# xds0112/5G_based_System_level_Integrated_Sensing_and_Communication_Simulator

Measured on AMD Instinct MI355X. Metric: sensing slots/sec (CDL echo->2D-FFT->2D-CFAR), higher is better.
Workload: dtype f64

## Files before the change

5g_based_system_level_integrated_sensing_and_communication_simulator_amd/_build.py:

```python
from __future__ import annotations

import os
import subprocess
import sys
from concurrent.futures import ThreadPoolExecutor

HERE = os.path.dirname(os.path.abspath(__file__))
CSRC = os.path.join(HERE, "csrc")
OBJ = os.path.join(CSRC, "build")
LIB = os.path.join(HERE, "libisac_hip.so")
SOURCES = ["capi.hip", "fft2d.hip", "tables.hip", "echo.hip", "rdm.hip", "cov.hip", "eigh.hip", "music.hip", "cdl.hip", "cdl_os.hip", "cqi.hip", "los.hip", "doa2d.hip", "doa.hip", "rxfe.hip", "targets.hip", "cfar.hip"]
HEADERS = ["isac_common.hpp", "isac_internal.hpp", "cut_window.hpp", "ofdm_symbol.hpp", "beam_window.hpp", "fft_lds.hpp", "echo_dev.hpp", "eigh_dev.hpp", "eigh_layout.hpp", os.path.join("..", "..", "include", "isac.h"), os.path.join("..", "..", "include", "isac_targets.h"), os.path.join("..", "..", "include", "isac_cfar.h"), os.path.join("..", "..", "include", "isac_cfar_mc.h")]
HIPCC = os.environ.get("HIPCC", "/opt/rocm/bin/hipcc")
FLAGS = ["--offload-arch=gfx950", "-O3", "-std=c++17", "-fPIC", "-fno-gpu-rdc", "-Wall", "-Wno-unused-function",
         "-Wno-unused-variable", "-Wno-unused-value", "-Wno-unused-result", "-ffp-contract=on"]


def _newer(target: str, deps: list[str]) -> bool:
    if not os.path.exists(target):
        return False
    t = os.path.getmtime(target)
    return all(os.path.getmtime(d) <= t for d in deps if os.path.exists(d))


def _compile(src: str, force: bool) -> str:
    obj = os.path.join(OBJ, os.path.splitext(src)[0] + ".o")
    deps = [os.path.join(CSRC, src)] + [os.path.join(CSRC, h) for h in HEADERS] + [os.path.abspath(__file__)]
    if not force and _newer(obj, deps):
        return obj
    cmd = [HIPCC, *FLAGS, "-c", os.path.join(CSRC, src), "-o", obj]
    r = subprocess.run(cmd, capture_output=True, text=True)
    if r.returncode != 0:
        raise RuntimeError(f"hipcc failed for {src}:\n{r.stdout}\n{r.stderr}")
    if r.stderr.strip():
        sys.stderr.write(r.stderr)
    return obj


def build(force: bool = False, verbose: bool = False) -> str:
    os.makedirs(OBJ, exist_ok=True)
    srcs = [s for s in SOURCES if os.path.exists(os.path.join(CSRC, s))]
    with ThreadPoolExecutor(max_workers=min(len(srcs), os.cpu_count() or 4)) as ex:
        objs = list(ex.map(lambda s: _compile(s, force), srcs))
    if force or not _newer(LIB, objs):
        cmd = [HIPCC, "--offload-arch=gfx950", "-shared", "-fPIC", "-o", LIB, *objs,
               "-Wl,-soname,libisac_hip.so", "-Wl,--no-undefined"]
        r = subprocess.run(cmd, capture_output=True, text=True)
        if r.returncode != 0:
            raise RuntimeError(f"link failed:\n{r.stdout}\n{r.stderr}")
    if verbose:
        print(f"built {LIB}")
    return LIB


if __name__ == "__main__":
    build(force="--force" in sys.argv, verbose=True)
```

5g_based_system_level_integrated_sensing_and_communication_simulator_amd/_lib.py:

```python
from __future__ import annotations

import ctypes as C
import os
import sys
import threading

import numpy as np

_HERE = os.path.dirname(os.path.abspath(__file__))
_LIB_PATH = os.path.join(_HERE, "libisac_hip.so")
_lib = None
_lock = threading.Lock()

ISAC_ABI_VERSION = 8
ISAC_MAX_EST = 4096
ISAC_MAX_TARGETS = 1024
NOISE_NONE, NOISE_INJECTED, NOISE_PHILOX, NOISE_PHILOX_SPECTRAL, NOISE_INJECTED_SPECTRAL = 0, 1, 2, 3, 4
CFAR_CA, CFAR_GOCA, CFAR_SOCA, CFAR_OS = 0, 1, 2, 3
CFAR_METHODS = {"CA": CFAR_CA, "GOCA": CFAR_GOCA, "SOCA": CFAR_SOCA, "OS": CFAR_OS}
ISAC_CFAR_MAX_TRAIN = 1024
TARGET_SW0, TARGET_SW1 = 0, 1
TARGET_MODELS = {"swerling0": TARGET_SW0, "swerling1": TARGET_SW1}
ISAC_CFAR_MC_MAX_TRAIN = 128
OPT_MUSIC_ROUTE, OPT_TAIL_FUSION, OPT_WIDE_ORDER, OPT_CDL_SHARE_SPECTRA, OPT_UPA_DOA = 0, 1, 2, 3, 4

STATUS_NAMES = {0: "OK", 1: "INVALID_ARG", 2: "HIP", 3: "NO_LOS", 4: "NO_DETECTION", 5: "CFAR_WINDOW",
                6: "CAPACITY", 7: "UNSUPPORTED", 8: "SHORT_WAVEFORM"}


class IsacError(RuntimeError):

    def __init__(self, code: int, message: str):
        self.code = int(code)
        self.name = STATUS_NAMES.get(int(code), str(code))
        super().__init__(f"isac[{self.name}]: {message}")


class c64(C.Structure):
    _fields_ = [("re", C.c_double), ("im", C.c_double)]


class Carrier(C.Structure):
    _fields_ = [("n_sc", C.c_int32), ("nfft", C.c_int32), ("scs_khz", C.c_int32), ("reserved", C.c_int32)]


class RadarChannelParams(C.Structure):
    _fields_ = [("fc", C.c_double), ("fs", C.c_double), ("n0", C.c_double), ("n_ants", C.c_int32),
                ("n_targets", C.c_int32), ("range", C.POINTER(C.c_double)), ("velocity", C.POINTER(C.c_double)),
                ("large_scale_fading", C.POINTER(C.c_double)), ("rx_steering", C.c_void_p)]


class CfarConfig(C.Structure):
    _fields_ = [("pfa", C.c_double), ("guard", C.c_int32 * 2), ("train", C.c_int32 * 2),
                ("row0", C.c_int32), ("row1", C.c_int32), ("col0", C.c_int32), ("col1", C.c_int32)]


class EstParams(C.Structure):
    _fields_ = [("n_ifft", C.c_int32), ("n_fft", C.c_int32), ("r_res", C.c_double), ("v_res", C.c_double),
                ("array_is_upa", C.c_int32), ("n_ants_x", C.c_int32), ("n_ants_y", C.c_int32),
                ("azimuth_scan_scale", C.c_double), ("azimuth_scan_granularity", C.c_double),
                ("elevation_scan_scale", C.c_double), ("elevation_scan_granularity", C.c_double)]


class Music2dParams(C.Structure):
    _fields_ = [("fc", C.c_double), ("t_sri", C.c_double), ("scs_hz", C.c_double), ("r_max", C.c_double), ("v_max", C.c_double)]


ISAC_MAX_SUBBANDS = 70


class CsiReport(C.Structure):
    _fields_ = [("n_subbands_pmi", C.c_int32), ("n_subbands_cqi", C.c_int32), ("n_cqi", C.c_int32), ("reserved", C.c_int32),
                ("i1", C.c_double * 3), ("i2", C.c_double * ISAC_MAX_SUBBANDS), ("cqi", C.c_double * (ISAC_MAX_SUBBANDS + 1)),
                ("subband_cqi", C.c_double * (ISAC_MAX_SUBBANDS + 1)), ("sinr_per_subband_cw", C.c_double * (ISAC_MAX_SUBBANDS + 1)), ("ri_total_sinr", C.c_double)]


ISAC_MAX_RBS = 275


class SrsReport(C.Structure):
    _fields_ = [("n_subbands", C.c_int32), ("n_tpmi", C.c_int32), ("n_rb", C.c_int32), ("reserved", C.c_int32),
                ("pmi", C.c_double * (ISAC_MAX_SUBBANDS + 1)), ("sinr_subband_pmi", C.c_double * (ISAC_MAX_SUBBANDS + 1)), ("cqi_rb", C.c_double * ISAC_MAX_RBS)]


class CdlJob(C.Structure):
    _fields_ = [("d_x", C.c_void_p), ("d_y", C.c_void_p), ("d_H", C.c_void_p), ("block_start", C.c_void_p), ("n_blocks", C.c_int32), ("reserved", C.c_int32)]


class SensingJob(C.Structure):
    _fields_ = [("d_tx_wave", C.c_void_p), ("d_tx_grid", C.c_void_p), ("d_echo_grid", C.c_void_p), ("rp", C.c_void_p), ("los", C.c_void_p),
                ("d_noise_unit", C.c_void_p), ("seed", C.c_uint64), ("noise_mode", C.c_int32), ("reserved", C.c_int32)]


class RxFrontendJob(C.Structure):
    _fields_ = [("d_y", C.c_void_p), ("d_noise_unit", C.c_void_p), ("path_scale", C.c_double), ("gain_scale", C.c_double), ("noise_power", C.c_double), ("seed", C.c_uint64)]


class PathLossConfig(C.Structure):
    _fields_ = [("building_height", C.c_double), ("street_width", C.c_double), ("environment_height", C.c_double), ("optional_model", C.c_int32), ("reserved", C.c_int32)]


class EstResult(C.Structure):
    _fields_ = [("n_rng", C.c_int32), ("n_vel", C.c_int32), ("n_azi", C.c_int32), ("num_dets", C.c_int32),
                ("total_detections", C.c_int32), ("reserved", C.c_int32),
                ("rng_est", C.c_double * ISAC_MAX_EST), ("vel_est", C.c_double * ISAC_MAX_EST),
                ("azi_est", C.c_double * ISAC_MAX_EST), ("ele_est", C.c_double * ISAC_MAX_EST)]
# ... 29 lines not shown
    "isac_sync": (_INT, (_P,)),
    "isac_dev_alloc": (_INT, (_P, _SZ, _P)),
    "isac_dev_free": (_INT, (_P, _P)),
    "isac_memcpy_h2d": (_INT, (_P, _P, _P, _SZ)),
    "isac_memcpy_d2h": (_INT, (_P, _P, _P, _SZ)),
    "isac_memcpy_d2d": (_INT, (_P, _P, _P, _SZ)),
    "isac_memset_dev": (_INT, (_P, _P, _I32, _SZ)),
    "isac_timer_start": (_INT, (_P,)),
    "isac_timer_stop_ms": (_INT, (_P, _P)),
    "isac_profile_enable": (_INT, (_P, _I32)),
    "isac_profile_last_kernel_ms": (_INT, (_P, _P)),
    "isac_basic_radar_channel_dev": (_INT, (_P, _P, _I64, _ptr(RadarChannelParams), _P, _I32, _P, _U64, _P)),
    "isac_basic_radar_channel": (_INT, (_P, _P, _I64, _ptr(RadarChannelParams), _P, _I32, _P, _U64, _P)),
    "isac_mono_static_sensing_dev": (_INT, (_P, _P, _I64, _I32, _ptr(Carrier), _ptr(RadarChannelParams), _P, _I32, _P, _U64, _P, _P)),
    "isac_mono_static_sensing": (_INT, (_P, _P, _I64, _I32, _ptr(Carrier), _ptr(RadarChannelParams), _P, _I32, _P, _U64, _P, _P)),
    "isac_mono_static_sensing_fused_dev": (_INT, (_P, _P, _I64, _I32, _ptr(Carrier), _ptr(RadarChannelParams), _P, _I32, _P, _U64, _P, _P, _ptr(EstParams), _ptr(CfarConfig), _P)),
    "isac_echo_grid_materialize_dev": (_INT, (_P, _P, _P)),
    "isac_ofdm_symbol_count": (_INT, (_ptr(Carrier), _I64, _P)),
    "isac_ofdm_demodulate_dev": (_INT, (_P, _P, _I64, _I32, _ptr(Carrier), _P, _I32)),
    "isac_ofdm_modulate_dev": (_INT, (_P, _P, _I32, _I32, _ptr(Carrier), _F64, _P, _I64)),
    "isac_ofdm_waveform_length": (_INT, (_ptr(Carrier), _I32, _P)),
    "isac_ofdm_modulate_windowed_dev": (_INT, (_P, _P, _I32, _I32, _ptr(Carrier), _F64, _I32, _I32, _P, _I64)),
    "isac_sentx_append_dev": (_INT, (_P, _ptr(Carrier), _I32, _I32, _I32, _P, _F64, _I32, _P, _I32, _I32, _P, _I64, _I64, _P)),
    "isac_cfar2d_ca": (_INT, (_P, _P, _I32, _I32, _P, _I32, _P, _P, _F64, _P, _I32, _P)),
    "isac_fft2d_dev": (_INT, (_P, _ptr(EstParams), _ptr(CfarConfig), _P, _P, _I32, _I32, _I32, _ptr(EstResult))),
    "isac_fft2d": (_INT, (_P, _ptr(EstParams), _ptr(CfarConfig), _P, _P, _I32, _I32, _I32, _ptr(EstResult))),
    "isac_fft2d_submit_dev": (_INT, (_P, _ptr(EstParams), _ptr(CfarConfig), _P, _P, _I32, _I32, _I32)),
    "isac_fft2d_collect": (_INT, (_P, _ptr(EstResult))),
    "isac_fft2d_submit_cached_dev": (_INT, (_P, _ptr(EstParams), _ptr(CfarConfig), _P, _P, _I32, _I32, _I32)),
    "isac_sensing_submit_n": (_INT, (_P, _I32, _ptr(SensingJob), _I64, _I32, _ptr(Carrier), _ptr(EstParams), _ptr(CfarConfig), _F64, _P)),
    "isac_sensing_collect_n": (_INT, (_P, _I32, _ptr(EstResult), _P)),
    "isac_fft2d_range_stage_dev": (_INT, (_P, _ptr(EstParams), _ptr(CfarConfig), _P, _P, _I32, _I32, _I32)),
    "isac_fft2d_get_detections": (_INT, (_P, _P, _P, _I32, _P, _P)),
    "isac_fft2d_get_power_window": (_INT, (_P, _P, _I64, _P, _P, _P)),
    "isac_fft2d_get_covariance": (_INT, (_P, _P, _I32)),
    "isac_fft2d_get_music_spectrum": (_INT, (_P, _P, _I32, _P)),
    "isac_rdm_plane_dev": (_INT, (_P, _ptr(EstParams), _P, _P, _I32, _I32, _I32, _I32, _P)),
    "isac_covariance_dev": (_INT, (_P, _P, _I64, _I32, _P)),
    "isac_eigh_top": (_INT, (_P, _P, _I32, _I32, _P, _P)),
    "isac_ctx_set_option": (_INT, (_P, _I32, _I32)),
    "isac_ctx_share_streams": (_INT, (_P, _P)),
    "isac_ctx_reserve": (_INT, (_P, _I64, _I32, _ptr(Carrier), _ptr(RadarChannelParams), _ptr(EstParams), _ptr(CfarConfig), _F64, _P)),
    "isac_music_doa": (_INT, (_P, _I32, _ptr(EstParams), _P, _I32, _P, _P, _P, _I32, _P)),
    "isac_beamscan_doa": (_INT, (_P, _I32, _I32, _ptr(EstParams), _P, _I32, _P, _P, _I32, _P)),
    "isac_get_angular_spectrum2d": (_INT, (_P, _P, _I64, _P)),
    "isac_find2d_peaks": (_INT, (_P, _P, _I32, _I32, _I32, _P, _P, _P)),
    "isac_music2d_dev": (_INT, (_P, _ptr(EstParams), _ptr(Music2dParams), _P, _P, _I32, _I32, _I32, _ptr(EstResult))),
    "isac_music2d_get_spectra": (_INT, (_P, _P, _I32, _P, _I32, _P)),
    "isac_eigh": (_INT, (_P, _P, _I32, _P, _P)),
    "isac_cdl_apply_dev": (_INT, (_P, _P, _I64, _I32, _I32, _I32, _P, _I32, _P, _P, _I32, _P, _F64, _P)),
    "isac_cdl_apply_batch_dev": (_INT, (_P, _ptr(CdlJob), _I32, _I64, _I32, _I32, _I32, _P, _I32, _P, _F64)),
    "isac_cdl_path_gains_dev": (_INT, (_P, _P, _P, _I32, _I32, _I32, _I32, _P, _F64, _P, _I32, _P)),
    "isac_prg_precode_dev": (_INT, (_P, _P, _I32, _I32, _I32, _P, _I32, _I32, _I32, _P)),
    "isac_cdl_freq_response_dev": (_INT, (_P, _P, _I32, _I32, _I32, _I32, _P, _P, _I64, _P)),
    "isac_cdl_csi_estimate_batch_dev": (_INT, (_P, _I32, _P, _P, _P, _P, _P, _I32, _I32, _I32, _I32, _I32, _P, _P, _I64, _P)),
    "isac_path_loss_38901": (_INT, (_I32, _F64, _I32, _P, _P, _ptr(PathLossConfig), _P)),
    "isac_path_loss_fspl": (_INT, (_F64, _P, _P, _P)),
    "isac_thermal_noise_power": (_INT, (_F64, _F64, _F64, _P)),
    "isac_dft_channel_matrix": (_INT, (_I32, _I32, _P)),
    "isac_rx_frontend_batch_dev": (_INT, (_P, _ptr(RxFrontendJob), _I32, _I64, _I32, _I32)),
    "isac_rx_frontend_dev": (_INT, (_P, _P, _I64, _I32, _F64, _F64, _F64, _I32, _P, _U64)),
    "isac_precoded_sinr_cqi_dev": (_INT, (_P, _P, _I64, _I32, _I32, _P, _I32, _F64, _P, _I32, _P, _P, _P)),
    "isac_type1sp_codebook": (_INT, (_I32, _I32, _I32, _I32, _I32, _P, _I64, _P)),
    "isac_csi_report_dev": (_INT, (_P, _P, _I64, _I32, _I32, _P, _P, _I32, _I32, _I32, _I32, _I32, _P, _I32, _P, _F64, _P, _I32, _ptr(CsiReport), _P, _P)),
    "isac_csi_report_batch_dev": (_INT, (_P, _I32, _P, _I64, _I32, _I32, _P, _P, _I32, _I32, _I32, _I32, _I32, _P, _I32, _P, _P, _P, _I32, _ptr(CsiReport), _P)),
    "isac_pusch_codebook": (_INT, (_I32, _I32, _P, _I64, _P)),
    "isac_srs_pmi_select_batch_dev": (_INT, (_P, _I32, _P, _I64, _I32, _I32, _P, _I32, _I32, _I32, _P, _P, _I32, _ptr(SrsReport))),
    "isac_los_check_dev": (_INT, (_P, _P, _P, _I64, _P, _P, _P, _P, _I32, _P, _P)),
    "isac_winding_number_dev": (_INT, (_P, _P, _I64, _P, _P, _P, _I32, _P)),
    "isac_synth_qpsk_grid_dev": (_INT, (_P, _P, _I32, _I32, _I32, _U64, _I32)),
}
EXPORTS = list(PROTOTYPES)
PROTOTYPES_ADDED = {
    "isac_fft2d_get_targets": (_INT, (_P, _P, _P, _I32)),
}
PROTOTYPES_CFAR = {
    "isac_cfar_threshold_factor": (_INT, (_I32, _I32, _I32, _F64, _P)),
    "isac_cfar2d": (_INT, (_P, _P, _I32, _I32, _P, _I32, _P, _P, _F64, _ptr(CfarMethod), _P, _I32, _P)),
    "isac_fft2d_redetect": (_INT, (_P, _ptr(CfarMethod), _ptr(EstResult), _P, _P, _I32, _P, _P)),
}
PROTOTYPES_CFAR_MC = {
    "isac_cfar_monte_carlo": (_INT, (_P, _ptr(CfarMethod), _I32, _F64, _I32, _P, _I32, _U64, _U64, _P, _P)),
}


def library_path() -> str:
    return _LIB_PATH


def load():
    global _lib
    with _lock:
        if _lib is not None:
            return _lib
        if not os.path.exists(_LIB_PATH):
            raise RuntimeError(
                f"{_LIB_PATH} is missing: build it with `python -c 'import __graft_entry__ as g; g.build()'` "
                "(hipcc --offload-arch=gfx950).  There is no CPU fallback for the sensing hot path.")
        if "torch" not in sys.modules and os.environ.get("ISAC_NO_TORCH_PRELOAD") != "1":
            try:
                import torch
            except Exception:
                pass
        lib = C.CDLL(_LIB_PATH, mode=C.RTLD_GLOBAL)
        for name, (restype, argtypes) in {**PROTOTYPES, **PROTOTYPES_ADDED, **PROTOTYPES_CFAR, **PROTOTYPES_CFAR_MC}.items():
            fn = getattr(lib, name)
            fn.restype, fn.argtypes = restype, argtypes
        if lib.isac_abi_version() != ISAC_ABI_VERSION:
            raise RuntimeError(f"{_LIB_PATH}: ABI version {lib.isac_abi_version()} but this binding was written for {ISAC_ABI_VERSION}; rebuild the library")
        for which, name, cls in [(i, n, c) for i, (n, c) in enumerate(ABI_STRUCTS)] + list(ABI_STRUCTS_ADDED) + list(ABI_STRUCTS_CFAR):
            if lib.isac_abi_sizeof(which) != C.sizeof(cls):
                raise RuntimeError(f"{_LIB_PATH}: sizeof({name}) = {lib.isac_abi_sizeof(which)} in the library, {C.sizeof(cls)} in the binding")
        _lib = lib
        return lib


def _np_ptr(a: np.ndarray):
    return a.ctypes.data_as(C.c_void_p)


class DeviceArray:

    def __init__(self, ctx: "Context", ptr: int, shape, dtype, owner: bool = True):
        self.ctx, self.ptr, self.shape, self.dtype, self._owner = ctx, int(ptr), tuple(int(s) for s in shape), np.dtype(dtype), owner

    @property
    def _as_parameter_(self):
        return C.c_void_p(self.ptr)

    @property
    def nbytes(self) -> int:
        return int(np.prod(self.shape, dtype=np.int64)) * self.dtype.itemsize

    def numpy(self) -> np.ndarray:
        out = np.empty(self.shape, dtype=self.dtype, order="F")
        self.ctx.check(self.ctx.lib.isac_memcpy_d2h(self.ctx.handle, _np_ptr(out), self, self.nbytes))
        return out

    def free(self):
        if self._owner and self.ptr:
            self.ctx.lib.isac_dev_free(self.ctx.handle, self)
            self.ptr = 0

    def __del__(self):
        try:
            if self.ctx.handle:
                self.free()
        except Exception:
            pass


class Context:

    def __init__(self, device: int | None = None):
        self.lib = load()
        if device is None:
            device = int(os.environ.get("ISAC_DEVICE", os.environ.get("LOCAL_RANK", "0")))
        n = C.c_int(0)
        st = self.lib.isac_device_count(C.byref(n))
        if st != 0 or n.value <= 0:
            raise IsacError(2, "no HIP device visible: the sensing hot path needs an MI355X (no CPU fallback)")
        h = C.c_void_p()
        st = self.lib.isac_ctx_create(device % n.value, C.byref(h))
        if st != 0:
            raise IsacError(st, f"isac_ctx_create(device={device}) failed")
        self.handle = h
        self.device = device % n.value
        self.device_cache = {}

    def close(self):
        if getattr(self, "handle", None):
            for ent in list(self.device_cache.values()):
                for d in (ent if isinstance(ent, tuple) else (ent,)):
                    for dd in (d if isinstance(d, tuple) else (d,)):
                        if isinstance(dd, DeviceArray):
                            dd.free()
            self.device_cache.clear()
            self.lib.isac_ctx_destroy(self.handle)
            self.handle = None

    def __del__(self):
        try:
            self.close()
        except Exception:
            pass

    def check(self, status: int):
        if status != 0:
            raise IsacError(status, (self.lib.isac_last_error(self.handle) or b"").decode())

    def sync(self):
        self.check(self.lib.isac_sync(self.handle))

    def stream(self) -> int:
        s = C.c_void_p()
        self.check(self.lib.isac_ctx_get_stream(self.handle, C.byref(s)))
        return int(s.value or 0)

    def empty(self, shape, dtype=np.complex128) -> DeviceArray:
        dt = np.dtype(dtype)
        nbytes = int(np.prod(shape, dtype=np.int64)) * dt.itemsize
        p = C.c_void_p()
        self.check(self.lib.isac_dev_alloc(self.handle, nbytes, C.byref(p)))
        return DeviceArray(self, p.value, shape, dt)

    def to_device(self, a: np.ndarray) -> DeviceArray:
        a = np.asfortranarray(a)
        d = self.empty(a.shape, a.dtype)
        self.check(self.lib.isac_memcpy_h2d(self.handle, d, _np_ptr(a), a.nbytes))
        return d

    def set_music_route(self, route: int):
        self.check(self.lib.isac_ctx_set_option(self.handle, OPT_MUSIC_ROUTE, int(route)))

    def set_tail_fusion(self, on: bool):
        self.check(self.lib.isac_ctx_set_option(self.handle, OPT_TAIL_FUSION, 1 if on else 0))

    def set_cdl_share_spectra(self, on: bool):
        self.check(self.lib.isac_ctx_set_option(self.handle, OPT_CDL_SHARE_SPECTRA, 1 if on else 0))

    def set_wide_order(self, on: bool):
        self.check(self.lib.isac_ctx_set_option(self.handle, OPT_WIDE_ORDER, 1 if on else 0))

    def set_upa_doa(self, on: bool):
        self.check(self.lib.isac_ctx_set_option(self.handle, OPT_UPA_DOA, 1 if on else 0))

    def angular_spectrum2d(self) -> np.ndarray:
        dims = (C.c_int32 * 2)()
        self.check(self.lib.isac_get_angular_spectrum2d(self.handle, None, 0, dims))
        out = np.zeros((dims[0], dims[1]), dtype=np.float64, order="F")
        self.check(self.lib.isac_get_angular_spectrum2d(self.handle, _np_ptr(out), out.size, dims))
        return out

    def angular_spectrum(self) -> np.ndarray:
        n = C.c_int32(0)
        self.check(self.lib.isac_fft2d_get_music_spectrum(self.handle, None, 0, C.byref(n)))
        out = np.zeros(n.value, dtype=np.float64)
        self.check(self.lib.isac_fft2d_get_music_spectrum(self.handle, _np_ptr(out), out.size, C.byref(n)))
        return out

    def music2d_spectra(self):
        n = (C.c_int32 * 2)()
        self.check(self.lib.isac_music2d_get_spectra(self.handle, None, 0, None, 0, n))
        pr, pv = np.zeros(n[0], dtype=np.float64), np.zeros(n[1], dtype=np.float64)
        self.check(self.lib.isac_music2d_get_spectra(self.handle, _np_ptr(pr), pr.size, _np_ptr(pv), pv.size, n))
        return pr, pv

    def share_streams(self, owner: "Context | None"):
        self.check(self.lib.isac_ctx_share_streams(self.handle, owner.handle if owner is not None else None))
        self._stream_owner = owner

    def eigh_top(self, h, n_top: int):
        h = as_c128_f(h)
        a = h.shape[0]
        w = np.zeros(a)
        u = np.zeros((a, max(int(n_top), 1)), dtype=np.complex128, order="F")
        self.check(self.lib.isac_eigh_top(self.handle, _np_ptr(h), a, int(n_top), _np_ptr(w), _np_ptr(u)))
        return w, u[:, : int(n_top)]

    def timer_start(self):
        self.check(self.lib.isac_timer_start(self.handle))

    def timer_stop_ms(self) -> float:
        ms = C.c_double(0)
        self.check(self.lib.isac_timer_stop_ms(self.handle, C.byref(ms)))
        return ms.value


_default_ctx = None


def default_context() -> Context:
    global _default_ctx
    if _default_ctx is None:
        _default_ctx = Context()
    return _default_ctx


def as_f64(x) -> np.ndarray:
    return np.ascontiguousarray(np.asarray(x, dtype=np.float64).reshape(-1))


def as_c128_f(x) -> np.ndarray:
    return np.asfortranarray(np.asarray(x, dtype=np.complex128))
```

5g_based_system_level_integrated_sensing_and_communication_simulator_amd/csrc/capi.hip:

```cpp
#include <algorithm>
#include <chrono>
#include <map>
#include <mutex>

#include "isac_internal.hpp"

using namespace isac;

extern "C" int isac_abi_version(void) { return ISAC_ABI_VERSION; }
extern "C" int isac_abi_sizeof(int32_t which) {
  switch (which) {
    case ISAC_SIZEOF_EST_RESULT: return (int)sizeof(isac_est_result);
    case ISAC_SIZEOF_EST_PARAMS: return (int)sizeof(isac_est_params);
    case ISAC_SIZEOF_CFAR_CONFIG: return (int)sizeof(isac_cfar_config);
    case ISAC_SIZEOF_RADAR_CHANNEL_PARAMS: return (int)sizeof(isac_radar_channel_params);
    case ISAC_SIZEOF_CARRIER: return (int)sizeof(isac_carrier);
    case ISAC_SIZEOF_MUSIC2D_PARAMS: return (int)sizeof(isac_music2d_params);
    case ISAC_SIZEOF_CSI_REPORT: return (int)sizeof(isac_csi_report);
    case ISAC_SIZEOF_SENSING_JOB: return (int)sizeof(isac_sensing_job);
    case ISAC_SIZEOF_SRS_REPORT: return (int)sizeof(isac_srs_report);
    case ISAC_SIZEOF_RX_FRONTEND_JOB: return (int)sizeof(isac_rx_frontend_job);
    case ISAC_SIZEOF_PATH_LOSS_CONFIG: return (int)sizeof(isac_path_loss_config);
    case ISAC_SIZEOF_TARGET_LIST: return (int)sizeof(isac_target_list);
    case ISAC_SIZEOF_CFAR_METHOD: return (int)sizeof(isac_cfar_method);
// ... 195 lines not shown
extern "C" int isac_profile_enable(isac_ctx* ctx, int on) {
  ISAC_ENTER(ctx);
  ctx->profile = on != 0;
  ctx->profile_cov = on == 2;
  ctx->profile_recorded = false;
  return ISAC_OK;
}
extern "C" int isac_profile_last_kernel_ms(isac_ctx* ctx, double* ms) {
  ISAC_ENTER(ctx);
  if (!ms) return fail(ctx, ISAC_ERR_INVALID_ARG, "NULL argument");
  if (!ctx->profile || !ctx->profile_recorded) return fail(ctx, ISAC_ERR_INVALID_ARG, "no profiled kernel launch on this context");
  ISAC_HIP(hipEventSynchronize(ctx->ev_k1));
  float f = 0.f;
  ISAC_HIP(hipEventElapsedTime(&f, ctx->ev_k0, ctx->ev_k1));
  *ms = (double)f;
  return ISAC_OK;
}

extern "C" int isac_ctx_reserve(isac_ctx* ctx, int64_t T, int32_t tx_dim_l, const isac_carrier* carrier, const isac_radar_channel_params* rp,
                                const isac_est_params* ep, const isac_cfar_config* cfar, double warm_ms, double* elapsed_ms) {
  ISAC_ENTER(ctx);
  if (!carrier || !rp || !ep || !cfar || T <= 0 || tx_dim_l < 0 || rp->n_ants <= 0 || rp->n_targets <= 0) return fail(ctx, ISAC_ERR_INVALID_ARG, "isac_ctx_reserve: NULL / empty argument");
  if (!std::isfinite(warm_ms) || warm_ms < 0.0) return fail(ctx, ISAC_ERR_INVALID_ARG, "isac_ctx_reserve: warm_ms must be finite and >= 0");
  if (warm_ms > 5000.0) warm_ms = 5000.0;
  if (ctx->pending.active) return fail(ctx, ISAC_ERR_INVALID_ARG, "isac_ctx_reserve: a submitted fft2D is pending on this context (the dry run would discard it): collect it first");
  const auto t0 = std::chrono::steady_clock::now();
  auto ms_since = [&]() { return std::chrono::duration<double, std::milli>(std::chrono::steady_clock::now() - t0).count(); };
  int32_t l_whole = 0;
  ISAC_TRY(isac_ofdm_symbol_count(carrier, T, &l_whole));
  const int K = carrier->n_sc, A = rp->n_ants, L = std::max<int>(l_whole, tx_dim_l);
  if (L <= 0) return fail(ctx, ISAC_ERR_SHORT_WAVEFORM, "isac_ctx_reserve: waveform shorter than one OFDM symbol");
  const size_t g_bytes = sizeof(c64) * (size_t)K * L * A, w_bytes = sizeof(c64) * (size_t)T * A;
  DevBuf grid, wave, echo;
  if (ensure(ctx, grid, g_bytes) != ISAC_OK || ensure(ctx, wave, w_bytes) != ISAC_OK || ensure(ctx, echo, g_bytes) != ISAC_OK)
    return fail(ctx, ISAC_ERR_HIP, "isac_ctx_reserve: no device memory for the dry run's grids (T A + 2 K L A elements)");
  void *d_grid = grid.p, *d_wave = wave.p, *d_echo = echo.p;
  std::vector<uint8_t> los((size_t)rp->n_targets, 1);
  int st = isac_synth_qpsk_grid_dev(ctx, (isac_c64*)d_grid, K, L, A, 0x5EEDull, 0);
  if (st == ISAC_OK) st = isac_memset_dev(ctx, d_wave, 0, w_bytes);
  if (st == ISAC_OK && l_whole > 0) st = isac_ofdm_modulate_dev(ctx, (const isac_c64*)d_grid, std::min<int>(l_whole, L), A, carrier, 1.0, (isac_c64*)d_wave, T);
  int n_dry = 0;
  while (st == ISAC_OK) {
    int32_t lo = 0;
    st = isac_mono_static_sensing_fused_dev(ctx, (const isac_c64*)d_wave, T, tx_dim_l, carrier, rp, los.data(), ISAC_NOISE_PHILOX_SPECTRAL, nullptr, 0x5EED0000ull + (uint64_t)n_dry,
                                            (isac_c64*)d_echo, &lo, ep, cfar, (const isac_c64*)d_grid);
    if (st != ISAC_OK) break;
    st = isac_fft2d_submit_cached_dev(ctx, ep, cfar, (const isac_c64*)d_echo, (const isac_c64*)d_grid, K, L, A);
    if (st == ISAC_ERR_INVALID_ARG) st = isac_fft2d_submit_dev(ctx, ep, cfar, (const isac_c64*)d_echo, (const isac_c64*)d_grid, K, L, A);
    if (st != ISAC_OK) break;
    static thread_local isac_est_result res;
    st = isac_fft2d_collect(ctx, &res);
    if (st == ISAC_ERR_NO_DETECTION || st == ISAC_ERR_CFAR_WINDOW) st = ISAC_OK;
    ++n_dry;
    if (ms_since() >= warm_ms) break;
  }
  const std::string keep = ctx->err;
  (void)hipStreamSynchronize(ctx->stream);
  (void)hipStreamSynchronize(ctx->stream2);
  ctx->range_cache.valid = false;
  ctx->last.valid = false;
  ctx->last.spectrum_db.clear();
  ctx->last.range_db.clear(); ctx->last.velocity_db.clear();
  ctx->tgt.drop();
  ctx->profile_recorded = false;
  (void)grid.reset(); (void)wave.reset(); (void)echo.reset();
  if (elapsed_ms) *elapsed_ms = ms_since();
  if (st != ISAC_OK) { ctx->err = keep; return st; }
  return ISAC_OK;
}

extern "C" int isac_ctx_set_option(isac_ctx* ctx, int32_t option, int32_t value) {
  ISAC_ENTER(ctx);
  if (value != 0 && value != 1) return fail(ctx, ISAC_ERR_INVALID_ARG, "option values are 0 or 1");
  switch (option) {
    case ISAC_OPT_MUSIC_ROUTE: ctx->music_route = value; return ISAC_OK;
    case ISAC_OPT_TAIL_FUSION: ctx->tail_fusion = value; return ISAC_OK;
    case ISAC_OPT_WIDE_ORDER: ctx->wide_order = value; return ISAC_OK;
    case ISAC_OPT_CDL_SHARE_SPECTRA: ctx->cdl_share_spectra = value; ctx->os_valid = false; return ISAC_OK;
    case ISAC_OPT_UPA_DOA: ctx->upa_doa = value; return ISAC_OK;
    default: return fail(ctx, ISAC_ERR_INVALID_ARG, "unknown option");
  }
}

extern "C" int isac_ctx_share_streams(isac_ctx* ctx, isac_ctx* owner) {
  ISAC_ENTER(ctx);
  if (owner && owner->device != ctx->device) return fail(ctx, ISAC_ERR_INVALID_ARG, "contexts of different devices cannot share streams");
  ISAC_HIP(hipStreamSynchronize(ctx->stream));
  ISAC_HIP(hipStreamSynchronize(ctx->stream2));
  if (ctx->pending.active) return fail(ctx, ISAC_ERR_INVALID_ARG, "a submitted fft2D is pending on this context: collect it first");
  ctx->stream = (owner && owner != ctx) ? owner->stream : ctx->own_stream;
  ctx->stream2 = (owner && owner != ctx) ? owner->stream2 : ctx->own_stream2;
  return ISAC_OK;
}

extern "C" int isac_basic_radar_channel(isac_ctx* ctx, const isac_c64* tx_wave, int64_t T,
                                        const isac_radar_channel_params* rp, const uint8_t* los, int noise_mode,
                                        const isac_c64* noise_unit, uint64_t seed, isac_c64* rx_wave) {
  ISAC_ENTER(ctx);
  if (!tx_wave || !rp || !rx_wave || T <= 0) return fail(ctx, ISAC_ERR_INVALID_ARG, "bad arguments");
  const size_t bytes = sizeof(c64) * (size_t)T * rp->n_ants;
  DevBuf d_tx, d_nz, d_rx;
  ISAC_TRY(ensure(ctx, d_tx, bytes));
  ISAC_TRY(ensure(ctx, d_rx, bytes));
  if (noise_mode == ISAC_NOISE_INJECTED && noise_unit) {
    if (ensure(ctx, d_nz, bytes) != ISAC_OK || copy_h2d(ctx, d_nz.p, noise_unit, bytes) != ISAC_OK)
      return fail(ctx, ISAC_ERR_HIP, "noise upload failed");
  }
  if (copy_h2d(ctx, d_tx.p, tx_wave, bytes) != ISAC_OK) return fail(ctx, ISAC_ERR_HIP, "upload failed");
  ISAC_TRY(isac_basic_radar_channel_dev(ctx, (const isac_c64*)d_tx.p, T, rp, los, noise_mode, (const isac_c64*)d_nz.p, seed, (isac_c64*)d_rx.p));
  if (copy_d2h(ctx, rx_wave, d_rx.p, bytes) != ISAC_OK) return fail(ctx, ISAC_ERR_HIP, "download failed");
  return ISAC_OK;
}

extern "C" int isac_mono_static_sensing(isac_ctx* ctx, const isac_c64* tx_wave, int64_t T, int32_t tx_dim_l,
                                        const isac_carrier* carrier, const isac_radar_channel_params* rp, const uint8_t* los,
                                        int noise_mode, const isac_c64* noise_unit, uint64_t seed, isac_c64* echo_grid,
                                        int32_t* l_out) {
  ISAC_ENTER(ctx);
  if (!tx_wave || !rp || !carrier || !echo_grid || T <= 0) return fail(ctx, ISAC_ERR_INVALID_ARG, "bad arguments");
  int32_t lw = 0;
  ISAC_TRY(isac_ofdm_symbol_count(carrier, T, &lw));
  const int L_out = lw < tx_dim_l ? tx_dim_l : lw;
  const size_t wbytes = sizeof(c64) * (size_t)T * rp->n_ants;
  const size_t gbytes = sizeof(c64) * (size_t)carrier->n_sc * (size_t)(L_out > 0 ? L_out : 1) * rp->n_ants;
  DevBuf d_tx, d_nz, d_g;
  ISAC_TRY(ensure(ctx, d_tx, wbytes));
  ISAC_TRY(ensure(ctx, d_g, gbytes));
  if ((noise_mode == ISAC_NOISE_INJECTED || noise_mode == ISAC_NOISE_INJECTED_SPECTRAL) && noise_unit) {
    const size_t nbytes = noise_mode == ISAC_NOISE_INJECTED ? wbytes : gbytes;
    if (ensure(ctx, d_nz, nbytes) != ISAC_OK || copy_h2d(ctx, d_nz.p, noise_unit, nbytes) != ISAC_OK)
      return fail(ctx, ISAC_ERR_HIP, "noise upload failed");
  }
  if (copy_h2d(ctx, d_tx.p, tx_wave, wbytes) != ISAC_OK) return fail(ctx, ISAC_ERR_HIP, "upload failed");
  ISAC_TRY(isac_mono_static_sensing_dev(ctx, (const isac_c64*)d_tx.p, T, tx_dim_l, carrier, rp, los, noise_mode,
                                        (const isac_c64*)d_nz.p, seed, (isac_c64*)d_g.p, l_out));
  if (copy_d2h(ctx, echo_grid, d_g.p, gbytes) != ISAC_OK) return fail(ctx, ISAC_ERR_HIP, "download failed");
  return ISAC_OK;
}
```

5g_based_system_level_integrated_sensing_and_communication_simulator_amd/csrc/cov.hip:

```cpp
#include <algorithm>
#include <type_traits>
#include "isac_internal.hpp"
#include "echo_dev.hpp"

namespace isac {

typedef double v4f64 __attribute__((ext_vector_type(4)));


constexpr int kCovSyncSlabs = 8;
template <int NB>
struct CovPlan {
  static constexpr int kTiles = NB * (NB + 1) / 2;
  static constexpr int kGroups = (kTiles + 4) / 5;
  static constexpr int kPerGroup = (kTiles + kGroups - 1) / kGroups;
  static constexpr int kPhases = 4 / kGroups;
  static constexpr int kSamplesPerLane = 4 / kPhases;
  static constexpr int first_tile(int grp) { return grp * kPerGroup; }
  static constexpr int tiles_of(int grp) { return first_tile(grp) + kPerGroup <= kTiles ? kPerGroup : kTiles - first_tile(grp); }
};

constexpr int cov_tile_i(int nb, int t) {
  int i = 0;
  while (t >= nb - i) { t -= nb - i; ++i; }
  return i;
}
constexpr int cov_tile_j(int nb, int t) {
  int i = 0;
  while (t >= nb - i) { t -= nb - i; ++i; }
  return i + t;
}
template <int U, int NT, class F>
__device__ __forceinline__ void static_for(F&& f) {
  if constexpr (U < NT) {
    f(std::integral_constant<int, U>{});
    static_for<U + 1, NT>(f);
  }
}

template <int NB, int T0, int NT, int E, int SPL, class F>
__device__ __forceinline__ void cov_3m_kstep(const c64 (&cur)[NB][SPL], const double (&dm)[NB], const double (&sp)[NB], v4f64 (&re)[NT], v4f64 (&im)[NT],
                                             v4f64 (&s3)[NT], F&& filler) {
  static_for<0, NT>([&](auto uc) {
    constexpr int u = decltype(uc)::value;
    constexpr int I = cov_tile_i(NB, T0 + u), J = cov_tile_j(NB, T0 + u);
    re[u] = __builtin_amdgcn_mfma_f64_16x16x4f64(cur[I][E].re, cur[J][E].re, re[u], 0, 0, 0);
    filler(std::integral_constant<int, u>{});
  });
  static_for<0, NT>([&](auto uc) {
    constexpr int u = decltype(uc)::value;
    constexpr int I = cov_tile_i(NB, T0 + u), J = cov_tile_j(NB, T0 + u);
    if constexpr (I == J) im[u] = __builtin_amdgcn_mfma_f64_16x16x4f64(cur[I][E].re, cur[J][E].im, im[u], 0, 0, 0);
    else                  im[u] = __builtin_amdgcn_mfma_f64_16x16x4f64(cur[I][E].im, cur[J][E].im, im[u], 0, 0, 0);
    filler(std::integral_constant<int, NT + u>{});
  });
  static_for<0, NT>([&](auto uc) {
    constexpr int u = decltype(uc)::value;
    constexpr int I = cov_tile_i(NB, T0 + u), J = cov_tile_j(NB, T0 + u);
    if constexpr (I == J) re[u] = __builtin_amdgcn_mfma_f64_16x16x4f64(cur[I][E].im, cur[J][E].im, re[u], 0, 0, 0);
    else                  s3[u] = __builtin_amdgcn_mfma_f64_16x16x4f64(dm[I], sp[J], s3[u], 0, 0, 0);
    filler(std::integral_constant<int, 2 * NT + u>{});
  });
}

template <bool DIAG>
__device__ __forceinline__ void cov_3m_out(double re, double im, double s3, double& o0, double& o1) {
  if constexpr (!DIAG) {
    o0 = re + im;
    o1 = (s3 - re) + im;
  } else {
    o0 = re;
    o1 = im;
  }
}

template <int NB, int GRP, int NBUF = 3>
__device__ __forceinline__ void cov_group_body(const c64* __restrict__ G, long long N, int A, int n_tiles, int phase, int lane,
                                               long long s0, long long s_step, long long s_cnt, long long s_lim, int part_index,
                                               double* __restrict__ part) {
  using P = CovPlan<NB>;
  constexpr int T0 = P::first_tile(GRP), NT = P::tiles_of(GRP);
  constexpr int SPL = P::kSamplesPerLane;
  const int li = lane & 15, kq = lane >> 4;
  v4f64 re[NT], im[NT], s3[NT];
#pragma unroll
  for (int u = 0; u < NT; ++u) re[u] = im[u] = s3[u] = v4f64{0.0, 0.0, 0.0, 0.0};
// ... 599 lines not shown
    v_half[1] = in && k0 + 512 < K;
    const uint32_t slot = (uint32_t)(((c.sc >> 6) << 9) + ((c.sc & 63) << 3));
    const uint64_t slab = (uint64_t)slot + (uint64_t)kSpectralSlotsPerColumn * (uint64_t)c.l;
#pragma unroll
    for (int j = 0; j < 2; ++j) {
      const uint64_t ctr = slab + colbase[j];
      pc[j][0] = (uint32_t)ctr; pc[j][1] = (uint32_t)(ctr >> 32); pc[j][2] = kSpectralStream; pc[j][3] = 0u;
    }
  }
  template <int R>
  __device__ __forceinline__ void round() {
#pragma unroll
    for (int j = 0; j < 2; ++j) philox4x32_round(pc[j], key0 + (uint32_t)R * 0x9E3779B9u, key1 + (uint32_t)R * 0xBB67AE85u);
  }
  template <int I>
  __device__ __forceinline__ void bm() {
    constexpr int j = I / 2, h = I % 2;
    box_muller32_hw_f32(pc[j][2 * h], pc[j][2 * h + 1], wf[j][h][0], wf[j][h][1]);
  }
  template <int I>
  __device__ __forceinline__ void emit(const c64 (&dv)[QT][2], c64* img) {
    constexpr int j = I / 2, h = I % 2;
    c64 d[QT];
#pragma unroll
    for (int q = 0; q < QT; ++q) d[q] = dv[q][h];
    c64 v = spectral_echo_value<QT, true>(d, st[j], mk((double)wf[j][h][0], (double)wf[j][h][1]), sig);
    const bool ok = v_half[h] && ant_ok[j];
    v = mk(ok ? v.re : 0.0, ok ? v.im : 0.0);
    img[g_lds0 + 2 * j * kCovSlabBlk + 8 * h * kCovPitch] = v;
  }
  __device__ __forceinline__ void loads(c64 (&dv)[QT][2], const Cur& c) {
    const int k0 = k0_of(c);
    const bool in = c.g < s_end;
    const unsigned base = (unsigned)(((long long)K * c.l + k0) * (long long)sizeof(c64));
    const unsigned o0 = (in && k0 < K) ? base : kCovOobOffset, o1 = (in && k0 + 512 < K) ? base + 512u * (unsigned)sizeof(c64) : kCovOobOffset;
#pragma unroll
    for (int q = 0; q < QT; ++q) { dv[q][0] = buffer_load_c64(rsD[q], o0); dv[q][1] = buffer_load_c64(rsD[q], o1); }
  }
  __device__ __forceinline__ void whole(c64 (&dv)[QT][2], c64* img) {
    loads(dv, cg);
    init(cg);
    static_for<0, 10>([&](auto rc) { round<decltype(rc)::value>(); });
    static_for<0, 4>([&](auto ic) { bm<decltype(ic)::value>(); });
    static_for<0, 4>([&](auto ic) { emit<decltype(ic)::value>(dv, img); });
    advance(cg);
  }
  __device__ __forceinline__ void prologue(c64* __restrict__ lds) {
    whole(dl[0], lds);
    whole(dl[1], lds + NB * kCovSlabBlk);
    cd = cg;
    loads(dl[0], cd); advance(cd);
    loads(dl[1], cd); advance(cd);
  }
  __device__ __forceinline__ void begin_step(long long) {}
  template <int PAR, int I>
  __device__ __forceinline__ void piece(c64* dst) {
    if constexpr (I == 0) { init(cg); round<0>(); }
    else if constexpr (I < 10) round<I>();
    else if constexpr (I < 14) bm<I - 10>();
    else if constexpr (I < 18) emit<I - 14>(dl[PAR], dst);
    else { loads(dl[PAR], cd); advance(cg); advance(cd); }
  }
  template <int PAR, int K_>
  __device__ __forceinline__ void gap(c64* dst, long long) {
    static_for<0, kLazyPieces>([&](auto ic) {
      if constexpr (lazy_piece_gap(decltype(ic)::value) == K_) piece<PAR, decltype(ic)::value>(dst);
    });
  }
};

template <int QT>
__global__ __launch_bounds__(256, 2) void cov_lazy_kernel(LazyCovArgs a, long long n_slabs, long long slabs_per_wg, double* __restrict__ part ) {
  extern __shared__ __attribute__((aligned(16))) char smem_raw[];
  c64* lds = reinterpret_cast<c64*>(smem_raw);
  const int wid = __builtin_amdgcn_readfirstlane(threadIdx.x >> 6);
  const int grp = wid >> 1, phase = wid & 1;
  const long long s_begin = (long long)blockIdx.x * slabs_per_wg;
  long long s_end = s_begin + slabs_per_wg;
  if (s_end > n_slabs) s_end = n_slabs;
  if (grp == 0) cov_staged_body<4, 0>(CovLazyGenerator<QT>(a, s_begin, s_end), phase, s_begin, s_end, blockIdx.x, part, lds);
  else cov_staged_body<4, 1>(CovLazyGenerator<QT>(a, s_begin, s_end), phase, s_begin, s_end, blockIdx.x, part, lds);
}

__global__ __launch_bounds__(256, 2) void cov_mfma_block_kernel(const c64* __restrict__ G, long long N, int A, int n_blk,
                                                                int n_pairs, long long slabs_per_wg,
                                                                double* __restrict__ part ) {
  extern __shared__ __attribute__((aligned(16))) char smem_raw[];
  c64* lds = reinterpret_cast<c64*>(smem_raw);
  const int pair = blockIdx.x % n_pairs, chunk = blockIdx.x / n_pairs;
  int BI, BJ;
  cov_pair_blocks(n_blk, pair, BI, BJ);
  if (BI == BJ) cov_block_pair<true>(G, N, A, BI, BJ, pair, chunk, n_pairs, slabs_per_wg, part, lds);
  else cov_block_pair<false>(G, N, A, BI, BJ, pair, chunk, n_pairs, slabs_per_wg, part, lds);
}

__global__ __launch_bounds__(1024) void cov_block_reduce_kernel(const double* __restrict__ part, int n_chunks, int n_blk, int n_pairs,
                                                                int A, double inv_n, c64* __restrict__ Ra) {
  __shared__ double s_sum[2][4][256];
  const int tile = blockIdx.x, pair = blockIdx.y;
  int BI, BJ;
  cov_pair_blocks(n_blk, pair, BI, BJ);
  const int I = tile >> 2, J = tile & 3;
  if (BI == BJ && J < I) return;
  const int e = threadIdx.x, g = threadIdx.y;
  const int per = (n_chunks + 3) / 4;
  const int c0 = g * per, c1 = min(n_chunks, c0 + per);
  double sr = 0.0, si = 0.0;
  for (int c = c0; c < c1; ++c) {
    const double* o = part + ((((long long)c * n_pairs + pair) * 16 + tile) * 2) * 256;
    sr += o[e];
    si += o[256 + e];
  }
  s_sum[0][g][e] = sr; s_sum[1][g][e] = si;
  __syncthreads();
  if (g != 0) return;
  sr = ((s_sum[0][0][e] + s_sum[0][1][e]) + s_sum[0][2][e]) + s_sum[0][3][e];
  si = ((s_sum[1][0][e] + s_sum[1][1][e]) + s_sum[1][2][e]) + s_sum[1][3][e];
  const int r = e >> 6, lane = e & 63;
  if (BI == BJ && I == J) {
    const int row = (lane >> 4) + 4 * r, col = lane & 15;
    const int et = (col >> 2) * 64 + ((col & 3) << 4) + row;
    si -= ((s_sum[1][0][et] + s_sum[1][1][et]) + s_sum[1][2][et]) + s_sum[1][3][et];
  }
  const int a = 64 * BI + 16 * I + (lane >> 4) + 4 * r;
  const int b = 64 * BJ + 16 * J + (lane & 15);
  if (a >= A || b >= A) return;
  c64 v = mk(sr * inv_n, si * inv_n);
  if (a == b) v.im = 0.0;
  if (BI == BJ && I == J && a > b) return;
  Ra[a + (long long)A * b] = v;
  if (a != b) Ra[b + (long long)A * a] = conj(v);
}

__global__ __launch_bounds__(256) void cov_reduce_slice_kernel(const double* __restrict__ part, int n_wg, int n_tiles, int S,
                                                               double* __restrict__ part2 ) {
  const int t = blockIdx.x, sl = blockIdx.y, e = threadIdx.x;
  const int per = (n_wg + S - 1) / S;
  const int w0 = sl * per, w1 = min(n_wg, w0 + per);
  double sr = 0.0, si = 0.0;
#pragma unroll 8
  for (int w = w0; w < w1; ++w) {
    const double* o = part + (((long long)w * n_tiles + t) * 2) * 256;
    sr += o[e];
    si += o[256 + e];
  }
  double* d = part2 + (((long long)sl * n_tiles + t) * 2) * 256;
  d[e] = sr; d[256 + e] = si;
}

__global__ __launch_bounds__(1024) void cov_reduce_kernel(const double* __restrict__ part, int n_wg, int n_tiles, int A,
                                                          double inv_n, c64* __restrict__ Ra ) {
  __shared__ double s_sum[2][4][256];
  const int t = blockIdx.x;
  const int nb = (A + 15) / 16;
  const int I = cov_tile_i(nb, t), J = cov_tile_j(nb, t);
  const int e = threadIdx.x;
  const int g = threadIdx.y;
  const int r = e >> 6, lane = e & 63;
  const int row = (lane >> 4) + 4 * r;
  const int col = lane & 15;
  const int per = (n_wg + 3) / 4;
  const int w0 = g * per, w1 = min(n_wg, w0 + per);
  double sr = 0.0, si = 0.0;
#pragma unroll 8
  for (int w = w0; w < w1; ++w) {
    const double* o = part + (((long long)w * n_tiles + t) * 2) * 256;
// ... 23 lines not shown
      Ra[b + (long long)A * a] = conj(v);
    }
  }
}

}

using namespace isac;

extern "C" int isac_covariance_dev(isac_ctx* ctx, const isac_c64* d_grid, int64_t N, int32_t A, isac_c64* d_Ra) {
  ISAC_ENTER(ctx);
  return isac_covariance_on(ctx, ctx->stream, d_grid, N, A, d_Ra);
}
#define ISAC_PROF_COV0(st) do { if (ctx->profile_cov) ISAC_HIP(hipEventRecord(ctx->ev_k0, st)); } while (0)
#define ISAC_PROF_COV1(st) do { if (ctx->profile_cov) { ISAC_HIP(hipEventRecord(ctx->ev_k1, st)); ctx->profile_recorded = true; } } while (0)
static void cov_staged_grid(long long slabs, long long& gx, long long& per) {
  gx = 512 < slabs ? 512 : slabs;
  per = (slabs + gx - 1) / gx;
  per = (per + 1) & ~1ll;
  gx = (slabs + per - 1) / per;
}

template <class Launch>
static int cov_partials_to_ra(isac_ctx* ctx, hipStream_t st, int n_part, int n_tiles, int A, double inv_n, c64* Ra, Launch&& launch) {
  const int S = 32;
  ISAC_TRY(ensure(ctx, ctx->cov_part, sizeof(double) * ((size_t)n_part + S) * n_tiles * 2 * 256));
  double* part = (double*)ctx->cov_part.p;
  double* part2 = part + (size_t)n_part * n_tiles * 2 * 256;
  ISAC_TRY(launch(part));
  hipLaunchKernelGGL(cov_reduce_slice_kernel, dim3(n_tiles, S), dim3(256), 0, st, (const double*)part, n_part, n_tiles, S, part2);
  ISAC_HIP(hipGetLastError());
  hipLaunchKernelGGL(cov_reduce_kernel, dim3(n_tiles), dim3(256, 4), 0, st, (const double*)part2, S, n_tiles, A, inv_n, Ra);
  ISAC_HIP(hipGetLastError());
  return ISAC_OK;
}

template <int NB>
static int launch_cov_small(isac_ctx* ctx, hipStream_t st, const c64* G, long long N, int A, c64* Ra) {
  using P = CovPlan<NB>;
  const long long total = (N + 15) / 16;
  if (N * 256 >= (1ll << 32)) return fail(ctx, ISAC_ERR_UNSUPPORTED, "covariance: at most 2^24 - 1 samples per antenna");
  const bool staged = (NB >= 3) && N * 256 < (1ll << 31);
  long long gx, per;
  if (staged) {
    cov_staged_grid(total, gx, per);
  } else {
    gx = NB == 4 ? 512 : 768;
    if (gx > total) gx = total;
    per = (total + gx - 1) / gx;
    gx = (total + per - 1) / per;
  }
  const int n_part = (int)gx * (staged ? 1 : P::kPhases);
  return cov_partials_to_ra(ctx, st, n_part, P::kTiles, A, 1.0 / (double)N, Ra, [&](double* part) -> int {
    if constexpr (NB >= 3) {
      if (staged) {
        const size_t lds = sizeof(c64) * kCovLdsBufs * NB * kCovSlabBlk;
        ISAC_TRY(allow_lds(ctx, reinterpret_cast<const void*>(cov_mfma_lds_kernel<NB>), lds));
        ISAC_PROF_COV0(st);
        hipLaunchKernelGGL((cov_mfma_lds_kernel<NB>), dim3((unsigned)gx), dim3(256), lds, st, G, N, A, per, part);
        ISAC_HIP(hipGetLastError());
        ISAC_PROF_COV1(st);
        return ISAC_OK;
      }
    }
    ISAC_PROF_COV0(st);
    hipLaunchKernelGGL((cov_mfma_small_kernel<NB>), dim3((unsigned)gx), dim3(256), 0, st, G, N, A, per, part);
    ISAC_HIP(hipGetLastError());
    ISAC_PROF_COV1(st);
    return ISAC_OK;
  });
}

template <int QT>
static int launch_cov_lazy(isac_ctx* ctx, hipStream_t st, const LazyCovArgs& a, long long n_slabs, long long per, long long gx, double* part) {
  const size_t lds = sizeof(c64) * kCovLdsBufs * 4 * kCovSlabBlk;
  ISAC_TRY(allow_lds(ctx, reinterpret_cast<const void*>(cov_lazy_kernel<QT>), lds));
  ISAC_PROF_COV0(st);
  hipLaunchKernelGGL((cov_lazy_kernel<QT>), dim3((unsigned)gx), dim3(256), lds, st, a, n_slabs, per, part);
  ISAC_HIP(hipGetLastError());
  ISAC_PROF_COV1(st);
  return ISAC_OK;
}

int isac_covariance_lazy_on(isac_ctx* ctx, hipStream_t st, isac_c64* d_Ra) {
  const LazyEcho& lz = ctx->lazy;
  if (!lz.valid || !lz.native || !d_Ra) return fail(ctx, ISAC_ERR_INVALID_ARG, "no native lazy echo grid on this context");
  if (lz.A <= 48 || lz.A > 64 || lz.Q < 1 || lz.Q > 2) return fail(ctx, ISAC_ERR_UNSUPPORTED, "lazy covariance: 49..64 antennas, one or two LoS targets");
  if ((long long)lz.K * lz.L_whole * 16 >= (1ll << 31)) return fail(ctx, ISAC_ERR_UNSUPPORTED, "lazy covariance: per-target grid of 2 GB or more");
  int s_col = 0;
  for (int k0 = 0; k0 < lz.K; k0 += 1024) s_col += (std::min(512, lz.K - k0) + 7) / 8;
  const long long n_slabs = (long long)lz.L_whole * s_col;
  if (n_slabs <= 0 || n_slabs >= (1ll << 31) - 4) return fail(ctx, ISAC_ERR_UNSUPPORTED, "lazy covariance: slab count out of range");
  long long gx, per;
  cov_staged_grid(n_slabs, gx, per);
  LazyCovArgs a{(const c64*)ctx->dgrid.p, (const c64*)ctx->steer.p + (size_t)lz.A * lz.Q, lz.sig, lz.seed, lz.K, lz.L_whole, lz.L_out, lz.A, s_col};
  return cov_partials_to_ra(ctx, st, (int)gx, CovPlan<4>::kTiles, lz.A, 1.0 / ((double)lz.K * (double)lz.L_out), (c64*)d_Ra, [&](double* part) -> int {
    return lz.Q == 1 ? launch_cov_lazy<1>(ctx, st, a, n_slabs, per, gx, part) : launch_cov_lazy<2>(ctx, st, a, n_slabs, per, gx, part);
  });
}

int isac_covariance_on(isac_ctx* ctx, hipStream_t st, const isac_c64* d_grid, int64_t N, int32_t A, isac_c64* d_Ra) {
  if (!d_grid || !d_Ra || N <= 0 || A <= 0) return fail(ctx, ISAC_ERR_INVALID_ARG, "bad arguments");
  const int nb = (A + 15) / 16;
  if (nb <= 4) {
    switch (nb) {
      case 1: return launch_cov_small<1>(ctx, st, (const c64*)d_grid, N, A, (c64*)d_Ra);
      case 2: return launch_cov_small<2>(ctx, st, (const c64*)d_grid, N, A, (c64*)d_Ra);
      case 3: return launch_cov_small<3>(ctx, st, (const c64*)d_grid, N, A, (c64*)d_Ra);
      default: return launch_cov_small<4>(ctx, st, (const c64*)d_grid, N, A, (c64*)d_Ra);
    }
  }
  {
    const int n_blk = (A + 63) / 64;
    const int n_pairs = n_blk * (n_blk + 1) / 2;
    const long long total = (N + 15) / 16;
    long long n_chunks = 1024 / n_pairs;
    if (n_chunks < 1) n_chunks = 1;
    if (n_chunks > total) n_chunks = total;
    if (N * 256 >= (1ll << 31)) return fail(ctx, ISAC_ERR_UNSUPPORTED, "covariance of more than 64 antennas: at most 2^23 - 1 samples per antenna");
    long long per = (total + n_chunks - 1) / n_chunks;
    per = (per + 1) & ~1ll;
    n_chunks = (total + per - 1) / per;
    ISAC_TRY(ensure(ctx, ctx->cov_part, sizeof(double) * (size_t)n_chunks * n_pairs * 16 * 2 * 256));
    ISAC_PROF_COV0(st);
    if (N * 512 < (1ll << 31)) {
      const size_t lds = sizeof(c64) * kCovUImgs * kCovUImg;
      ISAC_TRY(allow_lds(ctx, reinterpret_cast<const void*>(cov_mfma_block_pl_kernel), (size_t)(lds)));
      hipLaunchKernelGGL(cov_mfma_block_pl_kernel, dim3((unsigned)(n_chunks * n_pairs)), dim3(256), lds, st, (const c64*)d_grid, (long long)N, A,
                         n_blk, n_pairs, 2 * per, (double*)ctx->cov_part.p);
    } else {
      const size_t lds = sizeof(c64) * 2 * kCovBufElems;
      ISAC_TRY(allow_lds(ctx, reinterpret_cast<const void*>(cov_mfma_block_kernel), (size_t)(lds)));
      hipLaunchKernelGGL(cov_mfma_block_kernel, dim3((unsigned)(n_chunks * n_pairs)), dim3(256), lds, st, (const c64*)d_grid, (long long)N, A,
                         n_blk, n_pairs, per, (double*)ctx->cov_part.p);
    }
    ISAC_HIP(hipGetLastError());
    ISAC_PROF_COV1(st);
    hipLaunchKernelGGL(cov_block_reduce_kernel, dim3(16, n_pairs), dim3(256, 4), 0, st, (const double*)ctx->cov_part.p, (int)n_chunks,
                       n_blk, n_pairs, A, 1.0 / (double)N, (c64*)d_Ra);
    ISAC_HIP(hipGetLastError());
    return ISAC_OK;
  }
}
```

5g_based_system_level_integrated_sensing_and_communication_simulator_amd/csrc/echo.hip:

```cpp
#include <cstring>
#include <type_traits>

#include "isac_internal.hpp"
#include "fft_lds.hpp"
#include "echo_dev.hpp"
#include "beam_window.hpp"

namespace isac {

template <int QT, int UNROLL>
__device__ __forceinline__ void beam_sample(const c64* __restrict__ p , long long T, int A, const c64* __restrict__ s_steer , c64 (&acc)[QT]) {
#pragma unroll
  for (int q = 0; q < QT; ++q) acc[q] = mk(0.0, 0.0);
  int a = 0;
  for (; a + UNROLL <= A; a += UNROLL) {
    c64 v[UNROLL];
#pragma unroll
    for (int u = 0; u < UNROLL; ++u) v[u] = p[(long long)(a + u) * T];
#pragma unroll
    for (int u = 0; u < UNROLL; ++u)
#pragma unroll
      for (int q = 0; q < QT; ++q) acc[q] = fma(v[u], s_steer[q * A + a + u], acc[q]);
  }
  for (; a < A; ++a) {
    c64 v = p[(long long)a * T];
#pragma unroll
    for (int q = 0; q < QT; ++q) acc[q] = fma(v, s_steer[q * A + a], acc[q]);
  }
}

template <int QT, int UNROLL>
__global__ __launch_bounds__(256) void beamsum_kernel(const c64* __restrict__ tx, long long T, int A,
                                                      const c64* __restrict__ steer ,
                                                      c64* __restrict__ beam ) {
  extern __shared__ __attribute__((aligned(16))) char smem_raw[];
  c64* s_steer = reinterpret_cast<c64*>(smem_raw);
  for (int i = threadIdx.x; i < A * QT; i += blockDim.x) s_steer[i] = steer[i];
  __syncthreads();
  for (long long t0 = (long long)blockIdx.x * 256; t0 < T; t0 += (long long)gridDim.x * 256) {
    const long long t = t0 + threadIdx.x;
    const long long tc = t < T ? t : T - 1;
    c64 acc[QT];
    beam_sample<QT, UNROLL>(tx + tc, T, A, s_steer, acc);
    if (t < T) {
#pragma unroll
      for (int q = 0; q < QT; ++q) beam[(long long)q * T + t] = acc[q];
    }
  }
}

struct TargetDesc {
  double wd;
  double lsf;
  long long shift;
};
constexpr int kMaxTargets = 64;
struct TargetTable {
  TargetDesc t[kMaxTargets];
};

__device__ __forceinline__ c64 rx_phase(double w , double tt) {
  double s, c;
  sincos(w * tt, &s, &c);
  return mk(c, -s);
}

__device__ __forceinline__ c64 coef_value(c64 b, long long t, const TargetDesc& td, double w, double Ts, double tt, c64 prx) {
  double sd, cd, st, ct;
  sincos(td.wd * tt, &sd, &cd);
  sincos(w * ((double)(t - td.shift) * Ts), &st, &ct);
  c64 v = b * mk(ct, st);
  v = v * mk(cd, sd);
  v = v * td.lsf;
  return v * prx;
}

__global__ __launch_bounds__(256) void coef_kernel(const c64* __restrict__ beam, long long T, int Q,
                                                   TargetTable tab, double w , double Ts,
                                                   c64* __restrict__ coef ,
                                                   c64* __restrict__ phase_rx ) {
  long long t = (long long)blockIdx.x * blockDim.x + threadIdx.x;
  if (t >= T) return;
  double tt = (double)t * Ts;
  c64 prx = rx_phase(w, tt);
  phase_rx[t] = prx;
  for (int q = 0; q < Q; ++q) {
    long long d = tab.t[q].shift;
    c64 out = mk(0.0, 0.0);
    if (t >= d) out = coef_value(beam[(long long)q * T + (t - d)], t, tab.t[q], w, Ts, tt, prx);
    coef[(long long)q * T + t] = out;
  }
}

template <int QT>
struct CoefTargets {
  TargetDesc t[QT];
};
constexpr int kSteerArgMax = 128;
struct SteerArg {
  c64 v[kSteerArgMax];
};
template <int QT, int UNROLL>
__global__ __launch_bounds__(256) void beamsum_coef_kernel(const c64* __restrict__ tx, long long T, int A,
                                                           const c64* __restrict__ steer ,
                                                           const SteerArg steer_arg, c64* __restrict__ steer_out ,
                                                           BeamWindow bw, CoefTargets<QT> tab, double w , double Ts,
                                                           c64* __restrict__ coef ) {
  extern __shared__ __attribute__((aligned(16))) char smem_raw[];
  c64* s_steer = reinterpret_cast<c64*>(smem_raw);
  if (steer) {
    for (int i = threadIdx.x; i < A * QT; i += blockDim.x) s_steer[i] = steer[i];
  } else {
    for (int i = threadIdx.x; i < A * QT; i += blockDim.x) {
      const c64 v = steer_arg.v[i];
      s_steer[i] = v;
      if (blockIdx.x == 0) {
        const int q = i / A, a = i - q * A;
        steer_out[i] = v;
        steer_out[A * QT + a * QT + q] = v;
      }
    }
  }
  __syncthreads();
  const int n_units = (int)bw_units(bw);
  for (int k = blockIdx.x; k < n_units; k += gridDim.x) {
    const int l = k / bw.units_per_symbol, j = k - l * bw.units_per_symbol;
    const long long lo = bw_first(bw, l), hi = bw_range_end(bw, l);
    const long long u = bw_sample(bw, l, j, threadIdx.x);
    const bool mine = u >= lo && u < hi;
    if (!__any(mine)) continue;
    long long uc = u < lo ? lo : u < hi ? u : hi - 1;
    uc = uc < 0 ? 0 : uc < T ? uc : T - 1;
    c64 acc[QT];
    beam_sample<QT, UNROLL>(tx + uc, T, A, s_steer, acc);
    if (!mine) continue;
#pragma unroll
    for (int q = 0; q < QT; ++q) {
      const long long t = u + tab.t[q].shift;
      c64* cq = coef + (long long)q * T;
      if (t >= 0 && t < T) {
        const double tt = (double)t * Ts;
        cq[t] = u < 0 ? mk(0.0, 0.0) : coef_value(acc[q], t, tab.t[q], w, Ts, tt, rx_phase(w, tt));
      }
    }
  }
}

__global__ __launch_bounds__(256) void radar_waveform_kernel(long long T, int A, int Q, const c64* __restrict__ coef,
                                                             const c64* __restrict__ steer_rq ,
                                                             const c64* __restrict__ phase_rx, int noise_mode,
                                                             const c64* __restrict__ noise, double n0s, uint64_t seed,
                                                             c64* __restrict__ rx) {
  long long t = (long long)blockIdx.x * blockDim.x + threadIdx.x;
  int r = blockIdx.y;
  if (t >= T) return;
  rx[t + T * r] = rx_sample(t, r, T, Q, coef, steer_rq + (long long)r * Q, phase_rx, noise_mode, noise, n0s, seed);
}

struct OfdmGeom {
  int nfft, n_sc, cp_base, cp_long, sym_per_half;
};

template <class FFT, bool SYNTH, int QT = 0>
__global__ __launch_bounds__(256, 2) void demod_kernel(OfdmGeom g, long long T, int A, int L_whole, int L_out,
                                                       const c64* __restrict__ tw,
                                                       int Q_rt, const c64* __restrict__ coef,
                                                       const c64* __restrict__ steer_rq, const c64* __restrict__ phase_rx,
                                                       int noise_mode, const c64* __restrict__ noise, double n0s,
                                                       uint64_t seed,
                                                       const c64* __restrict__ wave,
                                                       c64* __restrict__ grid, const c64* __restrict__ logtab_g) {
  extern __shared__ __attribute__((aligned(16))) char smem_raw[];
  c64* lds = reinterpret_cast<c64*>(smem_raw);
  const int tid = threadIdx.x;
  FFT fft;
  constexpr bool kTables = SYNTH && QT > 0 && std::is_same<FFT, Fft4096>::value;
  const int Q = QT ? QT : Q_rt;
  {
    const int col = blockIdx.x;
    const int l = col % L_whole, r = col / L_whole;
    const int cp = cp_of_symbol(l, g.cp_base, g.cp_long, g.sym_per_half);
    const int off = cp / 2;
    const long long w0 = symbol_start(l, g.nfft, g.cp_base, g.cp_long, g.sym_per_half) + off;
    const int dshift = cp - off;
    if constexpr (SYNTH) {
      const c64* sr = steer_rq + (long long)r * Q;
      if (noise_mode == ISAC_NOISE_PHILOX) {
        if constexpr (kTables) {
          c64* lt = lds + FFT::LDS_ELEMS;
          if (tid < kLogTabSize) lt[tid] = logtab_g[tid];
          fft.init_table(lds, tw, tid);
          const c64* w256 = lds + FFT::IMG;
          fft.template fill<4>([&](int n) { return rx_sample(w0 + n, r, T, Q, coef, sr, phase_rx, ISAC_NOISE_PHILOX, noise, n0s, seed, w256, lt); }, tid);
          fft.init_twiddles(tw, tid);
        } else {
          fft.template fill<4>([&](int n) { return rx_sample(w0 + n, r, T, Q, coef, sr, phase_rx, ISAC_NOISE_PHILOX, noise, n0s, seed); }, tid);
        }
      } else {
        const int nm = (noise_mode == ISAC_NOISE_INJECTED) ? ISAC_NOISE_INJECTED : ISAC_NOISE_NONE;
        fft.template fill<8>([&](int n) { return rx_sample(w0 + n, r, T, Q, coef, sr, phase_rx, nm, noise, n0s, seed); }, tid);
      }
    } else {
      const c64* src = wave + w0 + T * (long long)r;
      fft.fill([&](int n) { return src[n]; }, tid);
    }
    if (!(kTables && noise_mode == ISAC_NOISE_PHILOX)) fft.init(lds, tw, tid);
    fft.template transform<-1>(lds, tw, tid);
    c64* dst = grid + (long long)g.n_sc * ((long long)l + (long long)L_out * r);
    const int half = g.n_sc / 2;
    fft.drain(
        [&](int k, c64 v) {
          const int kb = (k < g.nfft / 2) ? k : k - g.nfft;
          const int row = kb + half;
          const c64 ph = fft.phase_ramp(lds, tw, kb, dshift);
          if (row >= 0 && row < g.n_sc) {
            const c64 o = v * ph;
            __builtin_nontemporal_store(o.re, &dst[row].re);
            __builtin_nontemporal_store(o.im, &dst[row].im);
          }
        },
        tid);
  }
}

template <int QT, int NZ>
__global__ __launch_bounds__(256) void echo_spectral_kernel(int K, int L_whole, int L_out, int A, int Q_rt, const c64* __restrict__ D,
// ... 3 lines not shown
  const int tid = threadIdx.x;
  int l, r;
  if (!spectral_tile_map(blockIdx.x, L_whole, A, l, r)) return;
  const int Q = QT ? QT : Q_rt;
  const long long colg = (long long)l + (long long)L_out * r;
  c64* dst = grid + (long long)K * colg;
  struct None_ {};
  c64 acc[16];
  spectral_echo_column<QT, NZ, 4, 256>(tid, K, Q, D + (long long)K * l, (long long)K * L_whole, steer_rq + (long long)r * Q, sig, seed, colg,
                                  NZ == 2 ? noise + (long long)K * colg : nullptr, acc, [](int) { return None_{}; },
                                  [&](int, int k, c64 v, None_) {
                                    if (k < K) {
                                      __builtin_nontemporal_store(v.re, &dst[k].re);
                                      __builtin_nontemporal_store(v.im, &dst[k].im);
                                    }
                                    return v;
                                  });
}

constexpr int kEchoRangeWavesPerSimd = 4;
template <int QT, int NZ, int GROUP = (QT <= 1 ? 4 : 2)>
__global__ __launch_bounds__(Fft4096W::NT, kEchoRangeWavesPerSimd) void echo_range_kernel(int K, int L_whole, int L_out, int A, int Q_rt, const c64* __restrict__ D,
                                                            const c64* __restrict__ steer_rq, double sig, uint64_t seed,
                                                            const c64* __restrict__ noise, const c64* __restrict__ tw,
                                                            c64* __restrict__ grid,
                                                            const c64* __restrict__ txg, const double* __restrict__ win_k,
                                                            const double* __restrict__ win_r, double inv_n, double sqrt_n,
                                                            int row_lo, int n_rows, c64* __restrict__ ymid) {
  extern __shared__ __attribute__((aligned(16))) char smem_raw[];
  c64* lds = reinterpret_cast<c64*>(smem_raw);
  using FFT = Fft4096W;
  const int tid = threadIdx.x;
  FFT fft;
  const int Q = QT ? QT : Q_rt;
  int l, r;
  if (!spectral_tile_map(blockIdx.x, L_whole, A, l, r)) return;
  const long long colg = (long long)l + (long long)L_out * r;
  fft.init_table(lds, tw, tid);
  c64* dst = grid + (long long)K * colg;
  const c64* ptx = txg + (long long)K * colg;
#pragma unroll
  for (int j = 0; j < FFT::PER; ++j) fft.x[j] = mk(0.0, 0.0);
  struct TxWin { c64 tx; double w; };
  bool live = false;
  spectral_echo_column<QT, NZ, GROUP, FFT::NT>(
      tid, K, Q, D + (long long)K * l, (long long)K * L_whole, steer_rq + (long long)r * Q, sig, seed, colg,
      NZ == 2 ? noise + (long long)K * colg : nullptr, fft.x,
      [&](int kc) { return TxWin{ptx[kc], win_k[kc]}; },
      [&](int, int k, c64 v, TxWin t) {
        if (k < K) {
          __builtin_nontemporal_store(v.re, &dst[k].re);
          __builtin_nontemporal_store(v.im, &dst[k].im);
        }
        c64 y = mul_conj(v, t.tx) * t.w;
        y = k < K ? y : mk(0.0, 0.0);
        live |= (y.re != 0.0) | (y.im != 0.0);
        return y;
      });
  c64* yd = ymid + (long long)n_rows * colg;
  if (!__syncthreads_or(live)) {
    for (int rr = tid; rr < n_rows; rr += FFT::NT) yd[rr] = mk(0.0, 0.0);
    return;
  }
  fft.init_twiddles_lds(lds, tid);
  const int blk = FFT::block_of_rows(row_lo, n_rows);
  fft.template transform<+1>(lds, tw, tid, blk);
  auto put = [&](int n, c64 v) {
    const int rr = n - row_lo;
    const double wr = win_r[n];
    if (rr >= 0 && rr < n_rows) yd[rr] = ((v * inv_n) * sqrt_n) * wr;
  };
  if (blk >= 0) fft.drain_block(put, tid, blk);
  else fft.drain(put, tid);
}

template <int QT, int NZ, bool STORE = true, int GROUP = (QT <= 1 ? 4 : 2)>
__global__ __launch_bounds__(Fft4096W::NT, kEchoRangeWavesPerSimd) void echo_range_sl_kernel(int K, int L_whole, int L_out, int A, const c64* D,
                                                            const c64* __restrict__ steer_rq, double sig, uint64_t seed,
                                                            const c64* noise, const c64* __restrict__ tw,
                                                            c64* grid,
                                                            const c64* txg, const double* win_k,
                                                            const double* __restrict__ win_r, double inv_n, double sqrt_n,
                                                            int row_lo, int n_rows, c64* __restrict__ ymid) {
  static_assert(QT >= 1 && QT <= 2, "compile-time target count");
  extern __shared__ __attribute__((aligned(16))) char smem_raw[];
  c64* lds = reinterpret_cast<c64*>(smem_raw);
  using FFT = Fft4096W;
  constexpr int NT = FFT::NT, PER = FFT::PER, NG = PER / GROUP;
  const int tid = threadIdx.x;
  FFT fft;
  int l, r;
  if (!spectral_tile_map(blockIdx.x, L_whole, A, l, r)) return;
  const long long colg = (long long)l + (long long)L_out * r;
  const c64* Dl = D + (long long)K * l;
  const long long d_stride = (long long)K * L_whole;
  const c64* ptx = txg + (long long)K * colg;
  const c64* nzc = NZ == 2 ? noise + (long long)K * colg : nullptr;
  const __amdgpu_buffer_rsrc_t rs_dst = buffer_of(grid + (long long)K * colg, (unsigned)K * (unsigned)sizeof(c64));
  c64 s[QT];
#pragma unroll
  for (int q = 0; q < QT; ++q) s[q] = steer_rq[(long long)r * QT + q];
  struct Ld { c64 tx; double w; c64 d[QT]; c64 nz; };
  Ld ld[2][GROUP];
  auto load_group = [&](int g, int b) {
#pragma unroll
    for (int u = 0; u < GROUP; ++u) {
      const int k = tid + NT * (g * GROUP + u);
      const int kc = k < K ? k : K - 1;
      const unsigned o16 = (unsigned)kc * (unsigned)sizeof(c64);
      auto at = [](const auto* base, unsigned off) { return *reinterpret_cast<decltype(base)>(reinterpret_cast<const char*>(base) + off); };
      Ld& e = ld[b][u];
      e.tx = at(ptx, o16);
      e.w = at(win_k, (unsigned)k * (unsigned)sizeof(double));
      if constexpr (NZ == 2) e.nz = at(nzc, o16);
#pragma unroll
      for (int q = 0; q < QT; ++q) e.d[q] = at(Dl + (long long)q * d_stride, o16);
    }
    asm volatile("" ::: "memory");
  };
  fft.init_table(lds, tw, tid);
  load_group(0, 0);
  __builtin_amdgcn_sched_barrier(0);
#pragma unroll
  for (int j = 0; j < PER; ++j) fft.x[j] = mk(0.0, 0.0);
  const int wave_k0 = __builtin_amdgcn_readfirstlane(tid & ~63);
  auto draw = [&](int c) {
    if constexpr (NZ == 1) {
      const int j0 = 2 * c, j1 = j0 + 1;
      if (wave_k0 + NT * j0 < K) {
        const uint64_t ctr = (uint64_t)(tid + NT * c) + (uint64_t)kSpectralSlotsPerColumn * (uint64_t)colg;
        uint32_t o[4];
        philox4x32_10((uint32_t)ctr, (uint32_t)(ctr >> 32), kSpectralStream, 0u, (uint32_t)seed, (uint32_t)(seed >> 32), o);
        fft.x[j0] = box_muller32_hw(o[0], o[1]);
        if (wave_k0 + NT * j1 < K) fft.x[j1] = box_muller32_hw(o[2], o[3]);
      }
    }
  };
  bool live = false;
  auto consume = [&](int g, int b) {
#pragma unroll
    for (int u = 0; u < GROUP; ++u) {
      const int j = g * GROUP + u, k = tid + NT * j;
      const Ld& e = ld[b][u];
      const c64 v = spectral_echo_value<QT, NZ != 0>(e.d, s, NZ == 2 ? e.nz : fft.x[j], sig);
      if constexpr (STORE) buffer_store_c64_nt(rs_dst, (unsigned)k * (unsigned)sizeof(c64), v);
      else asm volatile("" ::"v"(v.re), "v"(v.im) : "memory");
      const c64 y = mul_conj(v, e.tx) * e.w;
      live |= (y.re != 0.0) | (y.im != 0.0);
      fft.x[j] = y;
    }
  };
#pragma unroll
  for (int g = 0; g < NG; ++g) {
#pragma unroll
    for (int c = g * GROUP / 2; c < (g + 1) * GROUP / 2; ++c) draw(c);
    __builtin_amdgcn_sched_barrier(0);
    if (g + 1 < NG) load_group(g + 1, (g + 1) & 1);
    consume(g, g & 1);
    __builtin_amdgcn_sched_barrier(0);
  }
  c64* yd = ymid + (long long)n_rows * colg;
  if (!__syncthreads_or(live)) {
    for (int rr = tid; rr < n_rows; rr += NT) yd[rr] = mk(0.0, 0.0);
    return;
  }
  fft.init_twiddles_lds(lds, tid);
  const int blk = FFT::block_of_rows(row_lo, n_rows);
  fft.template transform<+1>(lds, tw, tid, blk);
  auto put = [&](int n, c64 v) {
    const int rr = n - row_lo;
    const double wr = win_r[n];
    if (rr >= 0 && rr < n_rows) yd[rr] = ((v * inv_n) * sqrt_n) * wr;
  };
  if (blk >= 0) fft.drain_block(put, tid, blk);
  else fft.drain(put, tid);
}

struct ModIo {
  long long wave_rows, t_off;
  int grid_cols, l_off, sym0, n_win;
};

template <class FFT>
__global__ __launch_bounds__(256, 2) void mod_kernel(OfdmGeom g, ModIo io, int A, int L, const c64* __restrict__ tw,
                                                     const c64* __restrict__ grid, double scale ,
                                                     c64* __restrict__ wave, c64* __restrict__ head ,
                                                     const double* __restrict__ rise ) {
  extern __shared__ __attribute__((aligned(16))) char smem_raw[];
  c64* lds = reinterpret_cast<c64*>(smem_raw);
  const int tid = threadIdx.x;
  FFT fft;
  {
    const int col = blockIdx.x;
    const int l = col % L, a = col / L;
    const int cp = cp_of_symbol(io.sym0 + l, g.cp_base, g.cp_long, g.sym_per_half);
    const long long s0 = symbol_start(io.sym0 + l, g.nfft, g.cp_base, g.cp_long, g.sym_per_half) -
                         symbol_start(io.sym0, g.nfft, g.cp_base, g.cp_long, g.sym_per_half);
    const c64* src = grid + (long long)g.n_sc * ((long long)(io.l_off + l) + (long long)io.grid_cols * a);
    const int half = g.n_sc / 2;
    fft.fill(
        [&](int n) {
          int kb = (n < g.nfft / 2) ? n : n - g.nfft;
          int row = kb + half;
          const bool ok = (row >= 0 && row < g.n_sc);
          c64 v = src[ok ? row : 0];
          return ok ? v : mk(0.0, 0.0);
        },
        tid);
    fft.init(lds, tw, tid);
    fft.template transform<+1>(lds, tw, tid);
    c64* dst = wave + io.t_off + s0 + io.wave_rows * (long long)a;
    c64* hd = head ? head + (long long)io.n_win * ((long long)l + (long long)L * a) : nullptr;
    const int h0 = g.nfft - cp - io.n_win;
    fft.drain(
        [&](int m, c64 v) {
          v = v * scale;
          dst[cp + m] = v;
          if (m >= g.nfft - cp) dst[m - (g.nfft - cp)] = v;
          if (hd && m >= h0 && m < h0 + io.n_win) hd[m - h0] = v * rise[m - h0];
        },
        tid);
  }
}

__global__ __launch_bounds__(256) void mod_window_kernel(OfdmGeom g, ModIo io, int A, int L, const c64* __restrict__ head,
                                                         const double* __restrict__ rise, c64* __restrict__ wave) {
  const long long i = (long long)blockIdx.x * blockDim.x + threadIdx.x;
  const long long n = (long long)io.n_win * L * A;
  if (i >= n) return;
  const int w = (int)(i % io.n_win), l = (int)((i / io.n_win) % L), a = (int)(i / ((long long)io.n_win * L));
  const long long e = symbol_start(io.sym0 + l + 1, g.nfft, g.cp_base, g.cp_long, g.sym_per_half) -
                      symbol_start(io.sym0, g.nfft, g.cp_base, g.cp_long, g.sym_per_half);
  c64* p = wave + io.t_off + io.wave_rows * (long long)a + e - io.n_win + w;
  const c64 hv = head[(long long)io.n_win * ((long long)((l + 1) % L) + (long long)L * a) + w];
  *p = *p * rise[io.n_win - 1 - w] + hv;
}

__global__ __launch_bounds__(256) void copy_slot_kernel(const c64* __restrict__ src , c64* __restrict__ dst, int K, int L, int A,
                                                        int grid_cols, int l_off) {
  const long long i = (long long)blockIdx.x * blockDim.x + threadIdx.x;
  const long long n = (long long)K * L * A;
  if (i >= n) return;
  const long long k = i % K, l = (i / K) % L, a = i / ((long long)K * L);
  dst[k + (long long)K * ((l_off + l) + (long long)grid_cols * a)] = src ? src[i] : mk(0.0, 0.0);
}

__global__ __launch_bounds__(256) void synth_qpsk_kernel(c64* __restrict__ grid, int K, int L, int A, uint64_t seed,
                                                         int zero_s_slots) {
  long long i = (long long)blockIdx.x * blockDim.x + threadIdx.x;
  long long n = (long long)K * L * A;
  if (i >= n) return;
  int l = (int)((i / K) % L);
  int slot = l / 14;
  c64 v = mk(0.0, 0.0);
  if (!(zero_s_slots && (slot % 4) == 3)) {
    uint32_t o[4];
    philox4x32_10((uint32_t)i, (uint32_t)((uint64_t)i >> 32), 1u, 0u, (uint32_t)seed, (uint32_t)(seed >> 32), o);
    v = mk((o[0] & 1u) ? kR2 : -kR2, (o[1] & 1u) ? kR2 : -kR2);
  }
  grid[i] = v;
}

}

using namespace isac;

static int check_carrier(isac_ctx* ctx, const isac_carrier* c) {
  if (!c) return fail(ctx, ISAC_ERR_INVALID_ARG, "carrier is NULL");
  if (c->nfft < 128 || c->nfft > 4096 || (c->nfft & (c->nfft - 1)))
    return fail(ctx, ISAC_ERR_UNSUPPORTED, "carrier.nfft must be a power of two in 128..4096: no integral normal cyclic prefix (144 Nfft / 2048 samples) exists below 128");
  if (c->n_sc <= 0 || c->n_sc > c->nfft || (c->n_sc & 1)) return fail(ctx, ISAC_ERR_INVALID_ARG, "carrier.n_sc invalid");
  if (c->scs_khz != 15 && c->scs_khz != 30 && c->scs_khz != 60 && c->scs_khz != 120)
    return fail(ctx, ISAC_ERR_INVALID_ARG, "carrier.scs_khz must be 15/30/60/120");
  return ISAC_OK;
}

static OfdmGeom geom_of(const isac_carrier* c) {
  Numerology n = numerology(c->nfft, c->scs_khz);
  return OfdmGeom{c->nfft, c->n_sc, n.cp_base, n.cp_long, n.sym_per_half};
}

static int whole_symbols(const OfdmGeom& g, long long T) {
  long long lo = 0, hi = T / g.nfft + 1;
  while (lo < hi) {
    long long mid = (lo + hi + 1) / 2;
    if (symbol_start((int)mid, g.nfft, g.cp_base, g.cp_long, g.sym_per_half) <= T) lo = mid; else hi = mid - 1;
  }
  return (int)lo;
}

extern "C" int isac_ofdm_symbol_count(const isac_carrier* carrier, int64_t T, int32_t* n_symbols) {
  if (!carrier || !n_symbols || T < 0) return ISAC_ERR_INVALID_ARG;
  *n_symbols = whole_symbols(geom_of(carrier), T);
  return ISAC_OK;
}

extern "C" int isac_ofdm_waveform_length(const isac_carrier* carrier, int32_t L, int64_t* T) {
  if (!carrier || !T || L < 0) return ISAC_ERR_INVALID_ARG;
  OfdmGeom g = geom_of(carrier);
  *T = symbol_start(L, g.nfft, g.cp_base, g.cp_long, g.sym_per_half);
  return ISAC_OK;
}

static int prepare_echo(isac_ctx* ctx, const c64* d_tx, long long T, const isac_radar_channel_params* rp,
                        const uint8_t* los, int* q_out, const OfdmGeom* coef_only = nullptr) {
  if (!d_tx || !rp || !los) return fail(ctx, ISAC_ERR_INVALID_ARG, "NULL argument");
  if (T <= 0 || rp->n_ants <= 0 || rp->n_targets < 0) return fail(ctx, ISAC_ERR_INVALID_ARG, "bad T / n_ants / n_targets");
  ctx->lazy.valid = false;
  if (!(rp->fs > 0)) return fail(ctx, ISAC_ERR_INVALID_ARG, "fs must be positive");
  const int A = rp->n_ants;
  const double c0 = 299792458.0;
  const double lambda = c0 / rp->fc;
  const double Ts = 1.0 / rp->fs;
  const double two_pi = 2.0 * M_PI;
  TargetTable tab{};
  std::vector<c64> steer_aq;
  int Q = 0;
  for (int i = 0; i < rp->n_targets; ++i) {
    if (los[i] != 1) continue;
    if (Q >= kMaxTargets) return fail(ctx, ISAC_ERR_CAPACITY, "more than 64 LoS targets");
    for (int a = 0; a < A; ++a) {
      const isac_c64 sv = rp->rx_steering[(size_t)a + (size_t)A * i];
      steer_aq.push_back(mk(sv.re, sv.im));
    }
    double path_delay = 2.0 * rp->range[i] / c0;
    tab.t[Q].shift = (long long)std::ceil(path_delay / Ts);
    double fd = 2.0 * rp->velocity[i] / lambda;
    tab.t[Q].wd = two_pi * fd;
    tab.t[Q].lsf = rp->large_scale_fading[i];
    ++Q;
  }
  if (Q == 0) return fail(ctx, ISAC_ERR_NO_LOS, "no LoS target: rxWaveform is empty (basicRadarChannel.m:59,64)");
  std::vector<c64> steer_rq((size_t)A * Q);
  for (int q = 0; q < Q; ++q)
    for (int a = 0; a < A; ++a) steer_rq[(size_t)a * Q + q] = steer_aq[(size_t)q * A + a];
  ISAC_TRY(ensure(ctx, ctx->steer, sizeof(c64) * (size_t)A * Q * 2));
  ISAC_TRY(ensure(ctx, ctx->beam, sizeof(c64) * (size_t)Q * T));
  ISAC_TRY(ensure(ctx, ctx->coef, sizeof(c64) * (size_t)Q * T));
  ISAC_TRY(ensure(ctx, ctx->phase_rx, sizeof(c64) * (size_t)T));
  c64* d_steer_aq = (c64*)ctx->steer.p;
  const bool one_launch = coef_only && Q <= 2;
  const bool steer_by_arg = one_launch && A * Q <= kSteerArgMax;
  if (!steer_by_arg) {
    const size_t bytes = sizeof(c64) * (size_t)A * Q * 2;
    void* hst = nullptr;
    ISAC_TRY(stage_acquire(ctx, bytes, &hst));
    std::memcpy(hst, steer_aq.data(), bytes / 2);
    std::memcpy((char*)hst + bytes / 2, steer_rq.data(), bytes / 2);
    ISAC_TRY(stage_commit(ctx, d_steer_aq, bytes));
  }
  const unsigned gb = cdiv(T, 256);
  const unsigned gbs = (unsigned)std::min<long long>(gb, 1024);
  timeline_mark(ctx, 0, ctx->stream);
  const double w = two_pi * rp->fc;
  if (one_launch) {
    long long d_min = tab.t[0].shift, d_max = d_min;
    for (int q = 1; q < Q; ++q) { d_min = std::min(d_min, tab.t[q].shift); d_max = std::max(d_max, tab.t[q].shift); }
    const OfdmGeom& g = *coef_only;
    constexpr long long kSpan = 1LL << 38;
    if (T >= kSpan || d_max >= kSpan || d_min <= -kSpan) return fail(ctx, ISAC_ERR_CAPACITY, "waveform or target delay beyond the beam-sum's unit count");
    const BeamWindow bw = beam_window(g.nfft, g.cp_base, g.cp_long, g.sym_per_half, whole_symbols(g, T), T, d_min, d_max);
    const unsigned gbu = (unsigned)std::max<long long>(1, std::min<long long>(bw_units(bw), 1024));
    SteerArg sa{};
    if (steer_by_arg) std::memcpy(sa.v, steer_aq.data(), sizeof(c64) * (size_t)A * Q);
    auto launch = [&](auto qc) {
      constexpr int QT = decltype(qc)::value;
      CoefTargets<QT> ct;
      for (int q = 0; q < QT; ++q) ct.t[q] = tab.t[q];
      hipLaunchKernelGGL((beamsum_coef_kernel<QT, 32>), dim3(gbu), dim3(256), sizeof(c64) * A * QT, ctx->stream, d_tx, T, A, steer_by_arg ? nullptr : (const c64*)d_steer_aq, sa,
                         d_steer_aq, bw, ct, w, Ts, (c64*)ctx->coef.p);
    };
    if (Q == 1) launch(std::integral_constant<int, 1>{});
    else launch(std::integral_constant<int, 2>{});
    ISAC_HIP(hipGetLastError());
    timeline_mark(ctx, 1, ctx->stream);
    *q_out = Q;
    return ISAC_OK;
  }
#define ISAC_BEAMSUM(QT) \
  hipLaunchKernelGGL((beamsum_kernel<QT, (QT <= 2 ? 32 : 8)>), dim3(gbs), dim3(256), sizeof(c64) * A * QT, ctx->stream, d_tx, T, A, st, bm)
  for (int q0 = 0; q0 < Q;) {
    int rem = Q - q0;
    const c64* st = d_steer_aq + (size_t)q0 * A;
    c64* bm = (c64*)ctx->beam.p + (size_t)q0 * T;
    if (rem >= 8) { ISAC_BEAMSUM(8); q0 += 8; }
    else if (rem >= 4) { ISAC_BEAMSUM(4); q0 += 4; }
    else if (rem >= 2) { ISAC_BEAMSUM(2); q0 += 2; }
    else { ISAC_BEAMSUM(1); q0 += 1; }
  }
#undef ISAC_BEAMSUM
  timeline_mark(ctx, 1, ctx->stream);
  hipLaunchKernelGGL(coef_kernel, dim3(gb), dim3(256), 0, ctx->stream, (const c64*)ctx->beam.p, T, Q, tab, w, Ts,
                     (c64*)ctx->coef.p, (c64*)ctx->phase_rx.p);
  ISAC_HIP(hipGetLastError());
  *q_out = Q;
  return ISAC_OK;
}

extern "C" int isac_basic_radar_channel_dev(isac_ctx* ctx, const isac_c64* d_tx_wave, int64_t T,
                                            const isac_radar_channel_params* rp, const uint8_t* los, int noise_mode,
                                            const isac_c64* d_noise_unit, uint64_t seed, isac_c64* d_rx_wave) {
  ISAC_ENTER(ctx);
  if (!d_rx_wave) return fail(ctx, ISAC_ERR_INVALID_ARG, "rx_wave is NULL");
  if (noise_mode == ISAC_NOISE_INJECTED && !d_noise_unit) return fail(ctx, ISAC_ERR_INVALID_ARG, "noise buffer missing");
  if (noise_mode < ISAC_NOISE_NONE || noise_mode > ISAC_NOISE_PHILOX)
    return fail(ctx, ISAC_ERR_INVALID_ARG, "basicRadarChannel returns a time-domain waveform: noise modes NONE / INJECTED / PHILOX only");
  int Q = 0;
  ISAC_TRY(prepare_echo(ctx, (const c64*)d_tx_wave, T, rp, los, &Q));
  const int A = rp->n_ants;
  const double n0s = std::sqrt(rp->n0 / 2.0);
  hipLaunchKernelGGL(radar_waveform_kernel, dim3(cdiv(T, 256), A), dim3(256), 0, ctx->stream, (long long)T, A, Q,
                     (const c64*)ctx->coef.p, (const c64*)ctx->steer.p + (size_t)A * Q, (const c64*)ctx->phase_rx.p,
                     noise_mode, (const c64*)d_noise_unit, n0s, seed, (c64*)d_rx_wave);
  ISAC_HIP(hipGetLastError());
  return ISAC_OK;
}

template <int MAXQ, class F>
static int echo_dispatch(int Q, F&& f) {
  if constexpr (MAXQ > 0)
    if (Q != MAXQ) return echo_dispatch<MAXQ - 1>(Q, f);
  return f(std::integral_constant<int, MAXQ>{});
}

static int padded_symbols(int L_whole, int tx_dim_l, int32_t* l_out) {
  const int L_out = L_whole < tx_dim_l ? tx_dim_l : L_whole;
  if (l_out) *l_out = L_out;
  return L_out;
}

template <class FFT, bool SYNTH, int QT = 0>
static int launch_demod(isac_ctx* ctx, const OfdmGeom& g, long long T, int A, int L_whole, int L_out, const c64* tw, int Q,
                        int noise_mode, const c64* noise, double n0s, uint64_t seed, const c64* wave, c64* grid) {
  size_t lds = sizeof(c64) * (FFT::LDS_ELEMS + kLogTabSize);
  const c64* logtab = nullptr;
  ISAC_TRY(isac_get_logtab(ctx, &logtab));
  auto kern = demod_kernel<FFT, SYNTH, QT>;
  ISAC_TRY(allow_lds(ctx, reinterpret_cast<const void*>(kern), lds));
  hipLaunchKernelGGL(kern, dim3((unsigned)(L_whole * A)) , dim3(256), lds, ctx->stream, g, T, A, L_whole, L_out, tw, Q,
                     (const c64*)ctx->coef.p, SYNTH ? (const c64*)ctx->steer.p + (size_t)A * Q : nullptr,
                     (const c64*)ctx->phase_rx.p, noise_mode, noise, n0s, seed, wave, grid, logtab);
  ISAC_HIP(hipGetLastError());
  return ISAC_OK;
}

static int spectral_prepare(isac_ctx* ctx, const c64* d_tx, long long T, const isac_radar_channel_params* rp, const uint8_t* los,
                            const OfdmGeom& g, int* q_out, int* l_whole_out, bool coef_only = false) {
  int Q = 0;
  ISAC_TRY(prepare_echo(ctx, d_tx, T, rp, los, &Q, coef_only ? &g : nullptr));
  const int L_whole = whole_symbols(g, T);
  if (L_whole <= 0) return fail(ctx, ISAC_ERR_SHORT_WAVEFORM, "waveform shorter than one OFDM symbol");
  ISAC_TRY(ensure(ctx, ctx->dgrid, sizeof(c64) * (size_t)g.n_sc * L_whole * Q));
  const c64* tw = nullptr;
  ISAC_TRY(isac_get_twiddles(ctx, g.nfft, &tw));
  ISAC_FFT_DISPATCH(g.nfft, ISAC_TRY((launch_demod<FFT, false>(ctx, g, T, Q, L_whole, L_whole, tw, 0, 0, nullptr, 0.0, 0,
                                                               (const c64*)ctx->coef.p, (c64*)ctx->dgrid.p))));
  *q_out = Q;
  *l_whole_out = L_whole;
  return ISAC_OK;
}

static bool spectral_mode(int noise_mode) { return noise_mode == ISAC_NOISE_PHILOX_SPECTRAL || noise_mode == ISAC_NOISE_INJECTED_SPECTRAL; }

template <int QT>
static int launch_echo_spectral(isac_ctx* ctx, const OfdmGeom& g, int A, int L_whole, int L_out, int Q, int noise_mode,
                                const c64* noise, double sig, uint64_t seed, c64* grid) {
  const dim3 gr((unsigned)spectral_grid_size(L_whole, A)), bl(256);
  const c64* D = (const c64*)ctx->dgrid.p;
  const c64* srq = (const c64*)ctx->steer.p + (size_t)A * Q;
  auto kern = noise_mode == ISAC_NOISE_PHILOX_SPECTRAL ? echo_spectral_kernel<QT, 1> : noise_mode == ISAC_NOISE_INJECTED_SPECTRAL ? echo_spectral_kernel<QT, 2> : echo_spectral_kernel<QT, 0>;
  hipLaunchKernelGGL(kern, gr, bl, 0, ctx->stream, g.n_sc, L_whole, L_out, A, Q, D, srq, sig, seed, noise, grid);
  ISAC_HIP(hipGetLastError());
  return ISAC_OK;
}

template <class Kern, class... Args>
static int launch_echo_range(isac_ctx* ctx, Kern kern, int L_whole, int A, Args... args) {
  const size_t lds = sizeof(c64) * Fft4096W::LDS_ELEMS;
  ISAC_TRY(allow_lds(ctx, reinterpret_cast<const void*>(kern), lds));
  hipLaunchKernelGGL(kern, dim3((unsigned)spectral_grid_size(L_whole, A)), dim3(Fft4096W::NT), lds, ctx->stream, args...);
  ISAC_HIP(hipGetLastError());
  return ISAC_OK;
}

static int mono_static_spectral(isac_ctx* ctx, const c64* d_tx, long long T, int tx_dim_l, const OfdmGeom& g,
                                const isac_radar_channel_params* rp, const uint8_t* los, int noise_mode, const c64* d_noise,
                                uint64_t seed, c64* d_grid, int32_t* l_out) {
  int Q = 0, L_whole = 0;
  ISAC_TRY(spectral_prepare(ctx, d_tx, T, rp, los, g, &Q, &L_whole));
  const int A = rp->n_ants;
  const int L_out = padded_symbols(L_whole, tx_dim_l, l_out);
  if (L_out > L_whole) ISAC_HIP(hipMemsetAsync(d_grid, 0, sizeof(c64) * (size_t)g.n_sc * L_out * A, ctx->stream));
  const double sig = std::sqrt(rp->n0 / 2.0) * std::sqrt((double)g.nfft);
  return echo_dispatch<4>(Q, [&](auto qc) { return launch_echo_spectral<decltype(qc)::value>(ctx, g, A, L_whole, L_out, Q, noise_mode, d_noise, sig, seed, d_grid); });
}

extern "C" int isac_mono_static_sensing_dev(isac_ctx* ctx, const isac_c64* d_tx_wave, int64_t T, int32_t tx_dim_l,
                                            const isac_carrier* carrier, const isac_radar_channel_params* rp,
                                            const uint8_t* los, int noise_mode, const isac_c64* d_noise_unit,
                                            uint64_t seed, isac_c64* d_echo_grid, int32_t* l_out) {
  ISAC_ENTER(ctx);
  ctx->range_cache.valid = false;
  ISAC_TRY(check_carrier(ctx, carrier));
  if (!d_echo_grid) return fail(ctx, ISAC_ERR_INVALID_ARG, "echo_grid is NULL");
  if ((noise_mode == ISAC_NOISE_INJECTED || noise_mode == ISAC_NOISE_INJECTED_SPECTRAL) && !d_noise_unit)
    return fail(ctx, ISAC_ERR_INVALID_ARG, "noise buffer missing");
  if (noise_mode < ISAC_NOISE_NONE || noise_mode > ISAC_NOISE_INJECTED_SPECTRAL) return fail(ctx, ISAC_ERR_INVALID_ARG, "unknown noise mode");
  if (spectral_mode(noise_mode))
    return mono_static_spectral(ctx, (const c64*)d_tx_wave, T, tx_dim_l, geom_of(carrier), rp, los, noise_mode, (const c64*)d_noise_unit,
                                seed, (c64*)d_echo_grid, l_out);
  int Q = 0;
  ISAC_TRY(prepare_echo(ctx, (const c64*)d_tx_wave, T, rp, los, &Q));
  OfdmGeom g = geom_of(carrier);
  const int A = rp->n_ants;
  const int L_whole = whole_symbols(g, T);
  if (L_whole <= 0) return fail(ctx, ISAC_ERR_SHORT_WAVEFORM, "waveform shorter than one OFDM symbol");
  const int L_out = padded_symbols(L_whole, tx_dim_l, l_out);
  if (L_out > L_whole) ISAC_HIP(hipMemsetAsync(d_echo_grid, 0, sizeof(c64) * (size_t)g.n_sc * L_out * A, ctx->stream));
  const c64* tw = nullptr;
  ISAC_TRY(isac_get_twiddles(ctx, g.nfft, &tw));
  const double n0s = std::sqrt(rp->n0 / 2.0);
  if (g.nfft == 4096)
    return echo_dispatch<4>(Q, [&](auto qc) {
      return launch_demod<Fft4096, true, decltype(qc)::value>(ctx, g, T, A, L_whole, L_out, tw, Q, noise_mode, (const c64*)d_noise_unit, n0s, seed, nullptr, (c64*)d_echo_grid);
    });
  ISAC_FFT_DISPATCH(g.nfft, ISAC_TRY((launch_demod<FFT, true>(ctx, g, T, A, L_whole, L_out, tw, Q, noise_mode,
                                                              (const c64*)d_noise_unit, n0s, seed, nullptr,
                                                              (c64*)d_echo_grid))));
  return ISAC_OK;
}

extern "C" int isac_mono_static_sensing_fused_dev(isac_ctx* ctx, const isac_c64* d_tx_wave, int64_t T, int32_t tx_dim_l,
                                                  const isac_carrier* carrier, const isac_radar_channel_params* rp,
                                                  const uint8_t* los, int noise_mode, const isac_c64* d_noise_unit,
                                                  uint64_t seed, isac_c64* d_echo_grid, int32_t* l_out,
                                                  const isac_est_params* ep, const isac_cfar_config* cf,
                                                  const isac_c64* d_tx_grid) {
  ISAC_ENTER(ctx);
  ctx->range_cache.valid = false;
  ctx->lazy.valid = false;
  ISAC_TRY(check_carrier(ctx, carrier));
  if (!ep || !cf || !d_tx_grid || !rp) return fail(ctx, ISAC_ERR_INVALID_ARG, "NULL argument");
  if (noise_mode == ISAC_NOISE_INJECTED && !d_noise_unit) return fail(ctx, ISAC_ERR_INVALID_ARG, "noise buffer missing");
  OfdmGeom g = geom_of(carrier);
  CutRows cr;
  const bool rows_ok = cut_rows_ok(ep, cf, &cr) && cf->row1 >= cf->row0;
  const bool fusable = g.nfft == 4096 && ep->n_ifft == g.nfft && rows_ok;
  const bool lazy = d_echo_grid == nullptr;
  bool lazy_native = false;
  if (lazy) {
    int n_los = 0;
    if (!los) return fail(ctx, ISAC_ERR_INVALID_ARG, "NULL argument");
    for (int i = 0; i < rp->n_targets; ++i) n_los += los[i] == 1;
    lazy_native = fusable && noise_mode == ISAC_NOISE_PHILOX_SPECTRAL && rp->n_ants > 48 && rp->n_ants <= 64 && n_los >= 1 && n_los <= 2;
    if (!lazy_native) {
      int32_t lw = 0;
      ISAC_TRY(isac_ofdm_symbol_count(carrier, T, &lw));
      const int lo_ = padded_symbols(lw, tx_dim_l, nullptr);
      if (lo_ <= 0) return fail(ctx, ISAC_ERR_SHORT_WAVEFORM, "waveform shorter than one OFDM symbol");
      ISAC_TRY(ensure(ctx, ctx->echo_own, sizeof(c64) * (size_t)g.n_sc * lo_ * rp->n_ants));
      d_echo_grid = (isac_c64*)ctx->echo_own.p;
    }
  }
  auto plain_then_range = [&](bool cache_rows) -> int {
    int32_t lo = 0;
    ISAC_TRY(isac_mono_static_sensing_dev(ctx, d_tx_wave, T, tx_dim_l, carrier, rp, los, noise_mode, d_noise_unit, seed, d_echo_grid, &lo));
    if (l_out) *l_out = lo;
    if (lazy) ctx->lazy.set_owned(g.n_sc, lo, rp->n_ants);
    if (!cache_rows) return ISAC_OK;
    return isac_range_stage_into_cache(ctx, ep, cf, (const c64*)d_echo_grid, (const c64*)d_tx_grid, g.n_sc, lo, rp->n_ants);
  };
  if (!fusable) return plain_then_range(rows_ok && ep->n_ifft >= g.n_sc && (ep->n_ifft & (ep->n_ifft - 1)) == 0);
  if (noise_mode < ISAC_NOISE_NONE || noise_mode > ISAC_NOISE_INJECTED_SPECTRAL) return fail(ctx, ISAC_ERR_INVALID_ARG, "unknown noise mode");
  if (noise_mode == ISAC_NOISE_INJECTED_SPECTRAL && !d_noise_unit) return fail(ctx, ISAC_ERR_INVALID_ARG, "noise buffer missing");
  if (!spectral_mode(noise_mode)) return plain_then_range(true);
  int Q = 0, L_whole = 0;
  ISAC_TRY(spectral_prepare(ctx, (const c64*)d_tx_wave, T, rp, los, g, &Q, &L_whole, true));
  const int A = rp->n_ants, row_lo = cr.row_lo, nr = cr.nr;
  const int L_out = padded_symbols(L_whole, tx_dim_l, l_out);
  ctx->tgt.drop();
  ISAC_TRY(ensure(ctx, ctx->ymid, sizeof(c64) * (size_t)nr * L_out * A));
  if (L_out > L_whole) {
    if (!lazy_native) ISAC_HIP(hipMemsetAsync(d_echo_grid, 0, sizeof(c64) * (size_t)g.n_sc * L_out * A, ctx->stream));
    ISAC_HIP(hipMemsetAsync(ctx->ymid.p, 0, sizeof(c64) * (size_t)nr * L_out * A, ctx->stream));
  }
  const c64* tw = nullptr;
  const double *wk = nullptr, *wr = nullptr;
  ISAC_TRY(isac_get_w512_pack(ctx, &tw));
  ISAC_TRY(isac_get_windows(ctx, g.n_sc, ep->n_ifft, &wk, &wr));
  const double sig = std::sqrt(rp->n0 / 2.0) * std::sqrt((double)g.nfft);
  if (!ctx->profile_cov) ISAC_TRY(profile_begin(ctx));
  timeline_mark(ctx, 2, ctx->stream);
  auto launch = [&](auto kern, auto... q_rt) {
    return launch_echo_range(ctx, kern, L_whole, A, g.n_sc, L_whole, L_out, A, q_rt..., (const c64*)ctx->dgrid.p, (const c64*)ctx->steer.p + (size_t)A * Q, sig, seed,
                             (const c64*)d_noise_unit, tw, (c64*)d_echo_grid, (const c64*)d_tx_grid, wk, wr, 1.0 / ep->n_ifft, std::sqrt((double)ep->n_ifft), row_lo, nr,
                             (c64*)ctx->ymid.p);
  };
  const bool philox = noise_mode == ISAC_NOISE_PHILOX_SPECTRAL;
  ISAC_TRY(echo_dispatch<4>(Q, [&](auto qc) {
    constexpr int QT = decltype(qc)::value;
    if constexpr (QT == 1 || QT == 2)
      return launch(lazy_native ? echo_range_sl_kernel<QT, 1, false> : philox ? echo_range_sl_kernel<QT, 1> : echo_range_sl_kernel<QT, 2>);
    else
      return launch(philox ? echo_range_kernel<QT, 1> : echo_range_kernel<QT, 2>, Q);
  }));
  if (!ctx->profile_cov) ISAC_TRY(profile_end(ctx));
  timeline_mark(ctx, 3, ctx->stream);
  ctx->range_cache.set(d_echo_grid, d_tx_grid, g.n_sc, L_out, A, ep->n_ifft, row_lo, nr);
  if (lazy_native) ctx->lazy.set_native(g.n_sc, L_whole, L_out, A, Q, sig, seed);
  else if (lazy) ctx->lazy.set_owned(g.n_sc, L_out, A);
  return ISAC_OK;
}

extern "C" int isac_echo_grid_materialize_dev(isac_ctx* ctx, isac_c64* d_echo_grid, int32_t* dims3) {
  ISAC_ENTER(ctx);
  const LazyEcho& lz = ctx->lazy;
  if (!lz.valid) return fail(ctx, ISAC_ERR_INVALID_ARG, "no lazy echo grid on this context (isac_mono_static_sensing_fused_dev with d_echo_grid == NULL comes first)");
  if (dims3) { dims3[0] = lz.K; dims3[1] = lz.L_out; dims3[2] = lz.A; }
  if (!d_echo_grid) return ISAC_OK;
  const size_t bytes = sizeof(c64) * (size_t)lz.K * lz.L_out * lz.A;
  if (!lz.native) {
    ISAC_HIP(hipMemcpyAsync(d_echo_grid, ctx->echo_own.p, bytes, hipMemcpyDeviceToDevice, ctx->stream));
    return ISAC_OK;
  }
  if (lz.L_out > lz.L_whole) ISAC_HIP(hipMemsetAsync(d_echo_grid, 0, bytes, ctx->stream));
  OfdmGeom g{4096, lz.K, 0, 0, 0};
  return echo_dispatch<1>(lz.Q, [&](auto qc) {
    return launch_echo_spectral<(decltype(qc)::value == 1 ? 1 : 2)>(ctx, g, lz.A, lz.L_whole, lz.L_out, lz.Q, ISAC_NOISE_PHILOX_SPECTRAL, nullptr, lz.sig, lz.seed, (c64*)d_echo_grid);
  });
}

extern "C" int isac_ofdm_demodulate_dev(isac_ctx* ctx, const isac_c64* d_wave, int64_t T, int32_t A,
                                        const isac_carrier* carrier, isac_c64* d_grid, int32_t L) {
  ISAC_ENTER(ctx);
  ISAC_TRY(check_carrier(ctx, carrier));
  if (!d_wave || !d_grid || A <= 0) return fail(ctx, ISAC_ERR_INVALID_ARG, "bad arguments");
  OfdmGeom g = geom_of(carrier);
  const int L_whole = whole_symbols(g, T);
  if (L_whole <= 0) return fail(ctx, ISAC_ERR_SHORT_WAVEFORM, "waveform shorter than one OFDM symbol");
  if (L < L_whole) return fail(ctx, ISAC_ERR_CAPACITY, "grid has fewer symbol columns than the waveform holds");
  ctx->range_cache.touch(d_grid, sizeof(c64) * (size_t)g.n_sc * L * A);
  if (L > L_whole) ISAC_HIP(hipMemsetAsync(d_grid, 0, sizeof(c64) * (size_t)g.n_sc * L * A, ctx->stream));
  const c64* tw = nullptr;
  ISAC_TRY(isac_get_twiddles(ctx, g.nfft, &tw));
  ISAC_FFT_DISPATCH(g.nfft, ISAC_TRY((launch_demod<FFT, false>(ctx, g, T, A, L_whole, L, tw, 0, 0, nullptr, 0.0, 0,
                                                               (const c64*)d_wave, (c64*)d_grid))));
  return ISAC_OK;
}

template <class FFT>
static int launch_mod(isac_ctx* ctx, const OfdmGeom& g, const ModIo& io, int A, int L, const c64* tw, const c64* grid,
                      double scale, c64* wave, c64* head, const double* rise) {
  size_t lds = sizeof(c64) * FFT::LDS_ELEMS;
  auto kern = mod_kernel<FFT>;
  ISAC_TRY(allow_lds(ctx, reinterpret_cast<const void*>(kern), lds));
  hipLaunchKernelGGL(kern, dim3((unsigned)(L * A)) , dim3(256), lds, ctx->stream, g, io, A, L, tw, grid, scale, wave, head, rise);
  ISAC_HIP(hipGetLastError());
  return ISAC_OK;
}

static int modulate_into(isac_ctx* ctx, const isac_carrier* carrier, const c64* d_grid, int grid_cols, int l_off, int L, int A, int sym0,
                         double amplitude, int n_win, c64* d_wave, long long wave_rows, long long t_off) {
  OfdmGeom g = geom_of(carrier);
  if (n_win < 0 || n_win > g.cp_base) return fail(ctx, ISAC_ERR_INVALID_ARG, "windowing must lie in 0..(short cyclic prefix length)");
  const c64* tw = nullptr;
  ISAC_TRY(isac_get_twiddles(ctx, g.nfft, &tw));
  ModIo io{wave_rows, t_off, grid_cols, l_off, sym0, n_win};
  c64* head = nullptr;
  const double* rise = nullptr;
  if (n_win > 0) {
    ISAC_TRY(ensure(ctx, ctx->stage_c, sizeof(c64) * (size_t)n_win * L * A));
    head = (c64*)ctx->stage_c.p;
    ISAC_TRY(isac_get_rise_window(ctx, n_win, &rise));
  }
  ISAC_FFT_DISPATCH(g.nfft, ISAC_TRY((launch_mod<FFT>(ctx, g, io, A, L, tw, d_grid, amplitude / g.nfft, d_wave, head, rise))));
  if (n_win > 0) {
    hipLaunchKernelGGL(mod_window_kernel, dim3(cdiv((long long)n_win * L * A, 256)), dim3(256), 0, ctx->stream, g, io, A, L, (const c64*)head, rise, d_wave);
    ISAC_HIP(hipGetLastError());
  }
  return ISAC_OK;
}

extern "C" int isac_ofdm_modulate_dev(isac_ctx* ctx, const isac_c64* d_grid, int32_t L, int32_t A,
                                      const isac_carrier* carrier, double amplitude, isac_c64* d_wave, int64_t T) {
  return isac_ofdm_modulate_windowed_dev(ctx, d_grid, L, A, carrier, amplitude, 0, 0, d_wave, T);
}

extern "C" int isac_ofdm_modulate_windowed_dev(isac_ctx* ctx, const isac_c64* d_grid, int32_t L, int32_t A, const isac_carrier* carrier,
                                               double amplitude, int32_t n_slot, int32_t windowing, isac_c64* d_wave, int64_t T) {
  ISAC_ENTER(ctx);
  ISAC_TRY(check_carrier(ctx, carrier));
  if (!d_wave || !d_grid || A <= 0 || L <= 0 || n_slot < 0) return fail(ctx, ISAC_ERR_INVALID_ARG, "bad arguments");
// ... 46 lines not shown
```

5g_based_system_level_integrated_sensing_and_communication_simulator_amd/csrc/echo_dev.hpp:

```cpp
#pragma once
#include "isac_common.hpp"

namespace isac {

__device__ __forceinline__ uint32_t xor3(uint32_t a, uint32_t b, uint32_t c) {
#if defined(__HIP_DEVICE_COMPILE__) && __has_builtin(__builtin_amdgcn_bitop3_b32)
  return __builtin_amdgcn_bitop3_b32(a, b, c, 0x96);
#else
  return a ^ b ^ c;
#endif
}

__device__ __forceinline__ void philox4x32_10(uint32_t c0, uint32_t c1, uint32_t c2, uint32_t c3,
                                              uint32_t k0, uint32_t k1, uint32_t (&out)[4]) {
#pragma unroll
  for (int r = 0; r < 10; ++r) {
    uint64_t p0 = (uint64_t)0xD2511F53u * c0;
    uint64_t p1 = (uint64_t)0xCD9E8D57u * c2;
    uint32_t hi0 = (uint32_t)(p0 >> 32), lo0 = (uint32_t)p0;
    uint32_t hi1 = (uint32_t)(p1 >> 32), lo1 = (uint32_t)p1;
    uint32_t n0 = xor3(hi1, c1, k0), n2 = xor3(hi0, c3, k1);
    c0 = n0; c1 = lo1; c2 = n2; c3 = lo0;
    k0 += 0x9E3779B9u;
    k1 += 0xBB67AE85u;
// ... 127 lines not shown
  const int x = wg & 7, s = wg >> 3;
  const int tile = (s / (kTileSyms * kTileAnts)) * 8 + x, within = s % (kTileSyms * kTileAnts);
  const int n_ag = (A + kTileAnts - 1) / kTileAnts;
  const int ag = tile % n_ag, lb = tile / n_ag;
  r = kTileAnts * ag + within / kTileSyms;
  l = kTileSyms * lb + within % kTileSyms;
  return r < A && l < L_whole;
}

template <int QT, int NZ, int GROUP, int NT, class PRE, class E>
__device__ __forceinline__ void spectral_echo_column(int tid, int K, int Q_rt, const c64* __restrict__ Dl ,
                                                     long long d_stride , const c64* __restrict__ sr ,
                                                     double sig, uint64_t seed, long long column, const c64* __restrict__ nz,
                                                     c64 (&acc)[4096 / NT],
                                                     PRE&& pre, E&& emit) {
  constexpr int QM = QT ? QT : 1;
  constexpr int PER = 4096 / NT;
  constexpr int NG = PER / GROUP;
  constexpr int NCALL = PER / 2;
  constexpr int JSTEP = 512 / NT;
  const int Q = QT ? QT : Q_rt;
  const int n_el = (K + NT - 1) / NT;
  const int wave_k0 = __builtin_amdgcn_readfirstlane(tid & ~63);
  using Aux = decltype(pre(0));
  Aux aux[2][GROUP];
  c64 dv[2][GROUP][QM];
  c64 nzv[2][GROUP];
  auto kc_of = [&](int j) { const int k = tid + NT * j; return k < K ? k : K - 1; };
  auto load_group = [&](int g, int b) {
#pragma unroll
    for (int u = 0; u < GROUP; ++u) {
      const int j = g * GROUP + u;
      if (j < n_el) {
        const int kc = kc_of(j);
        aux[b][u] = pre(kc);
        if constexpr (NZ == 2) nzv[b][u] = nz[kc];
        if constexpr (QT > 0) {
#pragma unroll
          for (int q = 0; q < QT; ++q) dv[b][u][q] = Dl[(long long)q * d_stride + kc];
        }
      }
    }
  };
  load_group(0, 0);
  __builtin_amdgcn_sched_barrier(0);
  if constexpr (NZ == 1) {
#pragma unroll
    for (int c = 0; c < NCALL; ++c) {
      const int j0 = (NT == 512) ? 2 * c : 4 * (c / 2) + (c % 2), j1 = j0 + JSTEP;
      if (wave_k0 + NT * j0 < K) {
        const uint64_t ctr = (uint64_t)(tid + NT * c) + (uint64_t)kSpectralSlotsPerColumn * (uint64_t)column;
        uint32_t o[4];
        philox4x32_10((uint32_t)ctr, (uint32_t)(ctr >> 32), kSpectralStream, 0u, (uint32_t)seed, (uint32_t)(seed >> 32), o);
        acc[j0] = box_muller32_hw(o[0], o[1]);
        if (wave_k0 + NT * j1 < K) acc[j1] = box_muller32_hw(o[2], o[3]);
      }
    }
  }
  __builtin_amdgcn_sched_barrier(0);
#pragma unroll
  for (int g = 0; g < NG; ++g) {
    const int b = g & 1;
    if (g + 1 < NG) load_group(g + 1, b ^ 1);
#pragma unroll
    for (int u = 0; u < GROUP; ++u) {
      const int j = g * GROUP + u;
      if (j < n_el) {
        c64 v = mk(0.0, 0.0);
        if constexpr (QT > 0) {
#pragma unroll
          for (int q = 0; q < QT; ++q) v = fma(dv[b][u][q], sr[q], v);
        } else {
          for (int q = 0; q < Q; ++q) v = fma(Dl[(long long)q * d_stride + kc_of(j)], sr[q], v);
        }
        if constexpr (NZ == 1) v = v + acc[j] * sig;
        if constexpr (NZ == 2) v = v + nzv[b][u] * sig;
        acc[j] = emit(j, tid + NT * j, v, aux[b][u]);
      }
    }
    __builtin_amdgcn_sched_barrier(0);
  }
}

__device__ __forceinline__ c64 rx_sample(long long t, int r, long long T, int Q, const c64* __restrict__ coef,
                                         const c64* __restrict__ s_steer_r ,
                                         const c64* __restrict__ phase_rx, int noise_mode,
                                         const c64* __restrict__ noise, double n0s, uint64_t seed,
                                         const c64* __restrict__ w256 = nullptr ,
                                         const c64* __restrict__ logtab = nullptr) {
  c64 v = mk(0.0, 0.0);
  for (int q = 0; q < Q; ++q) v = fma(coef[(long long)q * T + t], s_steer_r[q], v);
  if (noise_mode != ISAC_NOISE_NONE) {
    uint64_t e = (uint64_t)t + (uint64_t)T * (uint64_t)r;
    c64 nz = (noise_mode == ISAC_NOISE_INJECTED) ? noise[e]
             : (w256 ? philox_normal_pair_tab(e, seed, 0u, w256, logtab) : philox_normal_pair(e, seed, 0u));
    v = v + (nz * n0s) * phase_rx[t];
  }
  return v;
}

}
```

5g_based_system_level_integrated_sensing_and_communication_simulator_amd/csrc/isac_common.hpp:

```cpp
#pragma once

#include <hip/hip_runtime.h>

#include <array>
#include <cmath>
#include <cstdint>
#include <cstdio>
#include <cstdlib>
#include <cstring>
#include <map>
#include <string>
#include <type_traits>
#include <utility>
#include <vector>

#include "../../include/isac.h"
#include "cut_window.hpp"
#include "ofdm_symbol.hpp"

namespace isac {

struct __attribute__((aligned(16))) c64 {
  double re, im;
};
// ... 12 lines not shown
  return {a.re * b.re + a.im * b.im, a.im * b.re - a.re * b.im};
}
__host__ __device__ inline c64 mul_i(c64 a) { return {-a.im, a.re}; }
__host__ __device__ inline c64 mul_mi(c64 a) { return {a.im, -a.re}; }
__host__ __device__ inline c64& operator+=(c64& a, c64 b) { a.re += b.re; a.im += b.im; return a; }
__host__ __device__ inline c64 fma(c64 a, c64 b, c64 c) {
  return {::fma(a.re, b.re, ::fma(-a.im, b.im, c.re)), ::fma(a.re, b.im, ::fma(a.im, b.re, c.im))};
}

typedef unsigned int u32x4_t __attribute__((ext_vector_type(4)));
constexpr int kBufferRsrcFlags = 0x00020000;
__device__ __forceinline__ __amdgpu_buffer_rsrc_t buffer_of(const void* base, unsigned bytes) {
  const unsigned long long b = reinterpret_cast<unsigned long long>(base);
  const unsigned lo = __builtin_amdgcn_readfirstlane((unsigned)b), hi = __builtin_amdgcn_readfirstlane((unsigned)(b >> 32));
  void* ub = reinterpret_cast<void*>(((unsigned long long)hi << 32) | lo);
  return __builtin_amdgcn_make_buffer_rsrc(ub, 0, (int)__builtin_amdgcn_readfirstlane(bytes), kBufferRsrcFlags);
}
__device__ __forceinline__ c64 buffer_load_c64(__amdgpu_buffer_rsrc_t rs, unsigned byte_off) {
  return __builtin_bit_cast(c64, __builtin_amdgcn_raw_buffer_load_b128(rs, (int)byte_off, 0, 0));
}
__device__ __forceinline__ void buffer_store_c64_nt(__amdgpu_buffer_rsrc_t rs, unsigned byte_off, c64 v) {
  __builtin_amdgcn_raw_buffer_store_b128(__builtin_bit_cast(u32x4_t, v), rs, (int)byte_off, 0,  2);
}

template <hipError_t (*Free)(void*)>
struct OwnedBuf {
  void* p = nullptr;
  size_t cap = 0;
  OwnedBuf() = default;
  OwnedBuf(OwnedBuf&& o) noexcept : p(o.p), cap(o.cap) { o.p = nullptr; o.cap = 0; }
  OwnedBuf& operator=(OwnedBuf&& o) noexcept { if (this != &o) { (void)reset(); p = o.p; cap = o.cap; o.p = nullptr; o.cap = 0; } return *this; }
  OwnedBuf(const OwnedBuf&) = delete;
  OwnedBuf& operator=(const OwnedBuf&) = delete;
  ~OwnedBuf() { (void)reset(); }
  hipError_t reset() {
    const hipError_t e = p ? Free(p) : hipSuccess;
    p = nullptr;
    cap = 0;
    return e;
  }
};
using DevBuf = OwnedBuf<hipFree>;
using PinnedBuf = OwnedBuf<hipHostFree>;
static_assert(!std::is_copy_constructible<DevBuf>::value && std::is_nothrow_move_constructible<DevBuf>::value, "one owner per allocation");

enum TableKind { kTwiddle, kW512Pack, kLogTab, kKaiser3, kKaiser3Shifted, kRiseWindow, kSind, kDoa2d };
struct TableKey {
  TableKind kind;
  std::array<long long, 4> par{};
  bool operator<(const TableKey& o) const { return kind != o.kind ? kind < o.kind : par < o.par; }
};

struct Fft2dLast {
  bool valid = false;
  std::vector<int32_t> det_rc;
  std::vector<double> det_pow;
  std::vector<int32_t> ant_off;
  std::vector<double> spectrum_db;
  std::vector<double> range_db, velocity_db;
};

struct RangeCache {
  bool valid = false;
  const void* rx = nullptr;
  const void* tx = nullptr;
  int K = 0, L = 0, A = 0, n_ifft = 0, row_lo = 0, nr = 0;
  void set(const void* rx_, const void* tx_, int K_, int L_, int A_, int n_ifft_, int row_lo_, int nr_) {
    *this = RangeCache{true, rx_, tx_, K_, L_, A_, n_ifft_, row_lo_, nr_};
  }
  void touch(const void* p, size_t bytes) {
    if (!valid) return;
    const size_t g = sizeof(double) * 2 * (size_t)K * (size_t)L * (size_t)A;
    const char *b = (const char*)p, *e = b + (bytes ? bytes : 1);
    auto hits = [&](const void* q) { const char* c = (const char*)q; return c && b < c + g && c < e; };
    if (hits(rx) || hits(tx)) valid = false;
  }
};

struct LazyEcho {
  bool valid = false, native = false;
  int K = 0, L_whole = 0, L_out = 0, A = 0, Q = 0;
  double sig = 0.0;
  unsigned long long seed = 0;
  void set_owned(int K_, int L_, int A_) { *this = LazyEcho{true, false, K_, L_, L_, A_, 0, 0.0, 0}; }
  void set_native(int K_, int L_whole_, int L_out_, int A_, int Q_, double sig_, unsigned long long seed_) { *this = LazyEcho{true, true, K_, L_whole_, L_out_, A_, Q_, sig_, seed_}; }
};

struct StageSlot {
  PinnedBuf mem;
  hipEvent_t ev = nullptr;
  bool busy = false;
};
constexpr int kStageSlots = 128;

struct DoaPlan {
  int A = 0, mode = 0;
  bool upa = false, upa2d = false;
  bool sub = false;
  const double* d_sind = nullptr; int n_steps = 0;
  const double* d_tab2d = nullptr;
  int e_steps = 0, a_steps = 0, cap2d = 0, n_ants_x = 0, n_ants_y = 0;
  bool refused() const { return upa && !upa2d; }
};

struct Fft2dCpi {
  enum { kNone = 0, kSubmitted = 1, kCollected = 2 };
  int state = kNone;
  isac_est_params ep{};
  isac_cfar_config cfar{};
  CutWindow win{};
  int A = 0, L = 0, cap = 0;
  const double* d_sind = nullptr; int n_steps = 0;
  void drop() { state = kNone; }
};

struct PackLayout {
  static constexpr int pack_first = 4096;
  size_t off_spec = 0, off_pow = 0, off_cut = 0, first_bytes = 0;
  static PackLayout of(int A, int n_spec) {
    PackLayout p;
    p.off_spec = ((3 + (size_t)A + 1) * sizeof(int) + 15) & ~(size_t)15;
    p.off_pow = p.off_spec + sizeof(double) * (size_t)(n_spec > 0 ? n_spec : 1);
    p.off_cut = p.off_pow + sizeof(double) * (size_t)pack_first; p.first_bytes = p.off_cut + sizeof(int) * (size_t)pack_first;
    return p;
  }
};
struct Fft2dPending {
  bool active = false;
  PackLayout pack;
  int* d_pcut_full = nullptr; double* d_ppow_full = nullptr;
  DoaPlan doa; int first2d = 0;
};

}

struct isac_ctx {
  int device = 0;
  int n_cus = 0;
  hipStream_t stream = nullptr;
  hipStream_t stream2 = nullptr;
  hipStream_t own_stream = nullptr, own_stream2 = nullptr;
  hipEvent_t ev_done = nullptr;
  hipEvent_t ev_fork = nullptr, ev_join = nullptr, ev_cfar = nullptr, ev_t0 = nullptr, ev_t1 = nullptr;
  hipEvent_t tl[8] = {nullptr, nullptr, nullptr, nullptr, nullptr, nullptr, nullptr, nullptr};
  bool tl_on = false;
  hipEvent_t ev_k0 = nullptr, ev_k1 = nullptr;
  bool profile = false, profile_recorded = false;
  bool profile_cov = false;
  int music_route = 0;
  long long eig_epoch = 0;
  bool tail_unjoined = false;
  int wide_order = 0;
  int tail_fusion = 1;
  std::string err;
  std::map<const void*, size_t> lds_allowed;
  std::map<isac::TableKey, isac::DevBuf> tables;
  isac::DevBuf beam, coef, phase_rx, steer, dgrid, ymid, pwin, flags, det_cut, det_pow, det_cnt, cov_part, cov,
      eig_w, eig_v, eig_scratch, spec, misc, stage_a, stage_b, stage_c, cdl_par, seg, cdl_h, rxfe_tab;
  isac::PinnedBuf pinned;
  isac::PinnedBuf bounce; hipEvent_t ev_bounce[2] = {nullptr, nullptr};
  isac::PinnedBuf pinned_csi;
  isac::Fft2dLast last;
  isac::Fft2dPending pending;
  isac::Fft2dCpi tgt;
  isac::DevBuf tgt_scratch;
  isac::DevBuf redet;
  isac::DevBuf cfar_mc;
  isac::RangeCache range_cache;
  isac::LazyEcho lazy;
  isac::DevBuf os_x;
  std::vector<const void*> os_waves;
  long long os_T = 0; int os_nt = 0, os_mpad = 0, os_tb = 0; bool os_valid = false;
  int cdl_share_spectra = 0;
  isac::DevBuf echo_own;
  int upa_doa = 0;
  isac::DevBuf doa2d_p, doa2d_db, doa2d_cand, doa2d_w, doa2d_user;
  int doa2d_rows = 0, doa2d_cols = 0;
  isac::StageSlot stage_ring[isac::kStageSlots];
  int stage_next = 0;
};

namespace isac {

inline int fail(isac_ctx* ctx, int code, const std::string& msg) {
  if (ctx) ctx->err = msg;
  return code;
}

inline int allow_lds(isac_ctx* ctx, const void* kernel, size_t bytes) {
  size_t& have = ctx->lds_allowed[kernel];
  if (have < bytes) {
    hipError_t e = hipFuncSetAttribute(kernel, hipFuncAttributeMaxDynamicSharedMemorySize, (int)bytes);
    if (e != hipSuccess) return fail(ctx, ISAC_ERR_HIP, std::string("hipFuncSetAttribute(MaxDynamicSharedMemorySize): ") + hipGetErrorString(e));
    have = bytes;
  }
  return ISAC_OK;
}

#define ISAC_HIP(call)                                                                     \
  do {                                                                                     \
    hipError_t e__ = (call);                                                               \
    if (e__ != hipSuccess)                                                                 \
      return isac::fail(ctx, ISAC_ERR_HIP, std::string(#call) + ": " + hipGetErrorString(e__)); \
  } while (0)

#define ISAC_ENTER_NOJOIN(ctx)                                                                     \
  do {                                                                                             \
    if (!(ctx)) return ISAC_ERR_INVALID_ARG;                                                       \
    if (hipSetDevice((ctx)->device) != hipSuccess)                                                 \
      return isac::fail((ctx), ISAC_ERR_HIP, "hipSetDevice failed for the context's device");     \
  } while (0)
#define ISAC_ENTER(ctx)                                                                            \
  do {                                                                                             \
    ISAC_ENTER_NOJOIN(ctx);                                                                        \
    if ((ctx)->tail_unjoined) {                                                                    \
                   \
      (ctx)->tail_unjoined = false;                                                                \
      if (hipStreamWaitEvent((ctx)->stream, (ctx)->ev_done, 0) != hipSuccess)                       \
        return isac::fail((ctx), ISAC_ERR_HIP, "hipStreamWaitEvent failed");                       \
    }                                                                                              \
  } while (0)

#define ISAC_TRY(call)              \
  do {                              \
    int s__ = (call);               \
    if (s__ != ISAC_OK) return s__; \
  } while (0)

inline int ensure(isac_ctx* ctx, DevBuf& b, size_t bytes) {
  if (b.cap >= bytes && b.p) return ISAC_OK;
  if (b.p) {
    ISAC_HIP(hipStreamSynchronize(ctx->stream));
    if (const hipError_t e = b.reset()) return fail(ctx, ISAC_ERR_HIP, std::string("hipFree(b.p): ") + hipGetErrorString(e));
  }
  size_t want = bytes < 256 ? 256 : bytes;
  ISAC_HIP(hipMalloc(&b.p, want));
  b.cap = want;
  return ISAC_OK;
}

// ... 130 lines not shown
```

5g_based_system_level_integrated_sensing_and_communication_simulator_amd/csrc/isac_internal.hpp:

```cpp
#pragma once
#include "isac_common.hpp"
#include "eigh_layout.hpp"

template <typename T, typename Build>
int cached_table(isac_ctx* ctx, const isac::TableKey& key, const T** out, Build build) {
  auto it = ctx->tables.find(key);
  if (it == ctx->tables.end()) {
    std::vector<T> v;
    build(v);
    isac::DevBuf b;
    ISAC_TRY(isac::upload(ctx, b, v.data(), sizeof(T) * v.size()));
    it = ctx->tables.emplace(key, std::move(b)).first;
  }
  *out = (const T*)it->second.p;
  return ISAC_OK;
}
int isac_get_twiddles(isac_ctx* ctx, int n, const isac::c64** out);
int isac_get_w512_pack(isac_ctx* ctx, const isac::c64** out);
int isac_get_logtab(isac_ctx* ctx, const isac::c64** out);
int isac_get_rise_window(isac_ctx* ctx, int n_win, const double** out);
int isac_get_windows(isac_ctx* ctx, int K, int n_ifft, const double** win_k, const double** win_r);
int isac_rdm_power_window(isac_ctx* ctx, const isac_est_params* ep, const isac_cfar_config* cf, const isac::c64* d_rx, const isac::c64* d_tx, int K, int L, int A, bool use_cached_range);
int check_rdm_dims(isac_ctx* ctx, const isac_est_params* ep, int K, int L, int A);
int isac_cfar_window(isac_ctx* ctx, const isac_est_params* ep, const isac_cfar_config* cf, int A, int cap);
double cfar_alpha(int n_train, double pfa);
namespace isac { struct CutRows { int row_lo, nr; }; }
bool cut_rows_ok(const isac_est_params* ep, const isac_cfar_config* cf, isac::CutRows* out);
int cut_rows(isac_ctx* ctx, const isac_est_params* ep, const isac_cfar_config* cf, isac::CutRows* out);
int isac_range_stage_into_cache(isac_ctx* ctx, const isac_est_params* ep, const isac_cfar_config* cf, const isac::c64* d_rx, const isac::c64* d_tx, int K, int L, int A);
int fft2d_estimates(isac_ctx* ctx, const isac_est_params* ep, const isac::CutWindow& win, int A, const int* ant_off, const std::vector<int>& cut, const std::vector<double>& pw, int num_dets_dev, std::vector<int32_t>& det_rc, isac_est_result* out);
int isac_covariance_on(isac_ctx* ctx, hipStream_t st, const isac_c64* d_grid, int64_t N, int32_t A, isac_c64* d_Ra);
int isac_covariance_lazy_on(isac_ctx* ctx, hipStream_t st, isac_c64* d_Ra);
int isac_eigh_dev(isac_ctx* ctx, const isac::c64* d_H, int A, hipStream_t st, bool live_replay = true);
int isac_eigh_replay_recover(isac_ctx* ctx, int n, hipStream_t st);
int isac_eigh_ql_dev(isac_ctx* ctx, int n, hipStream_t st, const int* ctl, bool allow_live = true);
int isac_music_tridiag_bisect_dev(isac_ctx* ctx, const isac::c64* d_H, int A, hipStream_t st);
bool isac_music_subspace_ok(isac_ctx* ctx, int A);
int isac_music_subspace_dev(isac_ctx* ctx, int A, const int* d_num_dets, int num_dets_host, hipStream_t st);
const int* isac_music_ctl(isac_ctx* ctx);
int isac_music_scan_dev(isac_ctx* ctx, int A, const int* d_num_dets, int num_dets_host, const double* d_sind, int n_steps, double d_ratio, double* d_spec, hipStream_t st, int mode = 0, const int* ctl = nullptr);
int isac_music2d_plane(isac_ctx* ctx, const isac::c64* d_rx, const isac::c64* d_tx, long long n, isac::c64* d_h);
int isac_music2d_signal_vectors(isac_ctx* ctx, const isac::c64* d_h, int K, int Ls, const int* d_top, int Lsig, isac::c64* d_U);
int isac_music2d_scan(isac_ctx* ctx, const isac::c64* d_U, int N, int ldU, const int* d_cols, int Lsig, int conj_u, double coef, double den, double x0, double dx, int n_steps, double* d_p);
int isac_doa2d_peak_cap(int rows, int cols);
int isac_doa2d_cand_doubles(int cap);
int isac_doa2d_scan_dev(isac_ctx* ctx, int mode, int nV, int nH, int eS, int aS, const double* d_tab, const int* d_num_dets, int num_dets_host, const int* ctl, hipStream_t st);
int isac_doa2d_norm_peaks_dev(isac_ctx* ctx, bool normalise, const double* d_db, int rows, int cols, double* d_cand, int cap, hipStream_t st);
int isac_doa2d_select(isac_ctx* ctx, const double* cand, int count, int cap, int rows, int L, std::vector<int>& ele, std::vector<int>& azi);
int doa_plan(isac_ctx* ctx, const isac_est_params* ep, int A, int mode, isac::DoaPlan* pl);
constexpr const char* kUpaRefused = "UPA DoA: music.m:69 calls tools.find2DPeaks, which the reference does not define";
int doa_eig_first_half(isac_ctx* ctx, const isac::DoaPlan& pl, const isac::c64* d_H, hipStream_t st, bool live_replay);
int doa_enqueue(isac_ctx* ctx, const isac::DoaPlan& pl, const int* d_num_dets, int num_dets_host, hipStream_t st);
int doa_readout(isac_ctx* ctx, const isac::DoaPlan& pl, const isac_est_params* ep, const double* host, int n_first, int L, const char* none_prefix, std::vector<double>& ele, std::vector<double>& azi);
void doa_store(const std::vector<double>& ele, const std::vector<double>& azi, int n, double* ele_est, double* azi_est);
bool cdl_os_ok(long long T, int Nt, int Nr, int n_paths, int n_taps, int max_shift);
bool cdl_os_ul_ok(long long T, int Nt, int Nr, int n_paths, int n_taps, int max_shift);
int cdl_os_apply(isac_ctx* ctx, const isac_cdl_job* jobs, int n_jobs, long long T, int Nt, int Nr, int n_paths, const double* taps, int n_taps, const int32_t* shift, int max_shift, double out_scale);
constexpr uint32_t kRxFrontEndStream = 3u;
constexpr uint32_t kCfarMcStream = 4u;
int isac_rx_frontend_jobs(isac_ctx* ctx, const isac_rx_frontend_job* jobs, int n_jobs, long long T, int Nr, int noise_mode);

inline isac::EighInfo* eig_info(isac_ctx* ctx, int A) { return reinterpret_cast<isac::EighInfo*>((char*)ctx->eig_w.p + sizeof(double) * (size_t)A); }
inline int ensure_eig_out(isac_ctx* ctx, int A) {
  ISAC_TRY(isac::ensure(ctx, ctx->eig_w, sizeof(double) * (size_t)A + sizeof(isac::EighInfo)));
  return isac::ensure(ctx, ctx->eig_v, sizeof(isac::c64) * (size_t)A * A);
}
namespace isac {
hipEvent_t timeline_base(hipStream_t st);
inline void timeline_mark(isac_ctx* ctx, int i, hipStream_t st) {
  static const bool on = std::getenv("ISAC_TIMELINE") != nullptr;
  if (!on) return;
  if (!ctx->tl_on) {
    for (auto& e : ctx->tl) (void)hipEventCreate(&e);
    ctx->tl_on = true;
    (void)timeline_base(st);
  }
  (void)hipEventRecord(ctx->tl[i], st);
}

struct MusicCtl { enum { kRoute = 0, kLsub = 1 }; };
}
```

include/isac.h:

```cpp
#ifndef ISAC_H
#define ISAC_H

#include <stddef.h>
#include <stdint.h>

#ifdef __cplusplus
extern "C" {
#endif

#define ISAC_ABI_VERSION 8
#define ISAC_MAX_EST 4096

typedef struct isac_ctx isac_ctx;

typedef struct { double re, im; } isac_c64;

typedef enum {
  ISAC_OK = 0,
  ISAC_ERR_INVALID_ARG = 1,
  ISAC_ERR_HIP = 2,
  ISAC_ERR_NO_LOS = 3,
  ISAC_ERR_NO_DETECTION = 4,
  ISAC_ERR_CFAR_WINDOW = 5,
  ISAC_ERR_CAPACITY = 6,
// ... 237 lines not shown
  ISAC_PL_UMA = 0, ISAC_PL_UMI = 1, ISAC_PL_RMA = 2, ISAC_PL_INH = 3,
  ISAC_PL_INF_SL = 4, ISAC_PL_INF_DL = 5, ISAC_PL_INF_SH = 6, ISAC_PL_INF_DH = 7, ISAC_PL_INF_HH = 8
} isac_path_loss_scenario;
typedef struct {
  double building_height;
  double street_width;
  double environment_height;
  int32_t optional_model;
  int32_t reserved;
} isac_path_loss_config;
int isac_path_loss_38901(int32_t scenario, double fc_hz, int32_t los, const double bs_pos[3], const double ue_pos[3],
                         const isac_path_loss_config* cfg, double* pl_db);
int isac_path_loss_fspl(double fc_hz, const double bs_pos[3], const double ue_pos[3], double* pl_db);
int isac_thermal_noise_power(double temperature_k, double noise_figure_db, double sample_rate_hz, double* nt_w);
int isac_dft_channel_matrix(int32_t Nt, int32_t Nr, isac_c64* H);

typedef struct {
  isac_c64* d_y;
  const isac_c64* d_noise_unit;
  double path_scale;
  double gain_scale;
  double noise_power;
  uint64_t seed;
} isac_rx_frontend_job;
int isac_rx_frontend_batch_dev(isac_ctx* ctx, const isac_rx_frontend_job* jobs, int32_t n_jobs, int64_t T, int32_t Nr, int32_t noise_mode);
int isac_rx_frontend_dev(isac_ctx* ctx, isac_c64* d_y, int64_t T, int32_t Nr, double path_scale, double gain_scale, double noise_power, int32_t noise_mode,
                         const isac_c64* d_noise_unit, uint64_t seed);

int isac_precoded_sinr_cqi_dev(isac_ctx* ctx, const isac_c64* d_H, int64_t n_re, int32_t Nr, int32_t P,
                               const isac_c64* W, int32_t n_layers, double sigma, const double* sinr_table_db,
                               int32_t n_table, double* d_sinr_per_re, double* mean_sinr, int32_t* cqi);

int isac_type1sp_codebook(int32_t n_ports, int32_t n1, int32_t n2, int32_t codebook_mode, int32_t n_layers, isac_c64* W,
                          int64_t cap_elems, int32_t dims[4]);

#define ISAC_MAX_SUBBANDS 70
typedef struct {
  int32_t n_subbands_pmi, n_subbands_cqi, n_cqi, reserved;
  double i1[3];
  double i2[ISAC_MAX_SUBBANDS];
  double cqi[ISAC_MAX_SUBBANDS + 1];
  double subband_cqi[ISAC_MAX_SUBBANDS + 1];
  double sinr_per_subband_cw[ISAC_MAX_SUBBANDS + 1];
  double ri_total_sinr;
} isac_csi_report;
int isac_csi_report_dev(isac_ctx* ctx, const isac_c64* d_H, int64_t n_re, int32_t Nr, int32_t P, const int32_t* re_k,
                        const int32_t* re_l, int32_t n_size_bwp, int32_t n_start_bwp, int32_t subband_size, int32_t pmi_subband,
                        int32_t cqi_subband, const isac_c64* W, int32_t n_layers, const int32_t dims[4], double nvar,
                        const double* sinr_table_db, int32_t n_table, isac_csi_report* out, double* total_sinr_out,
                        double* d_sinr_per_re_out);
int isac_csi_report_batch_dev(isac_ctx* ctx, int32_t n_ue, const isac_c64* const* d_H_list, int64_t n_re, int32_t Nr, int32_t P, const int32_t* re_k,
                              const int32_t* re_l, int32_t n_size_bwp, int32_t n_start_bwp, int32_t subband_size, int32_t pmi_subband,
                              int32_t cqi_subband, const isac_c64* W, int32_t n_layers, const int32_t dims[4], const double* nvar,
                              const double* sinr_table_db, int32_t n_table, isac_csi_report* out, double* total_sinr_out);

int isac_pusch_codebook(int32_t n_layers, int32_t n_ports, isac_c64* W, int64_t cap_elems, int32_t* n_tpmi);
#define ISAC_MAX_RBS 275
typedef struct {
  int32_t n_subbands, n_tpmi, n_rb, reserved;
  double pmi[ISAC_MAX_SUBBANDS + 1];
  double sinr_subband_pmi[ISAC_MAX_SUBBANDS + 1];
  double cqi_rb[ISAC_MAX_RBS];
} isac_srs_report;
int isac_srs_pmi_select_batch_dev(isac_ctx* ctx, int32_t n_ue, const isac_c64* const* d_H_list, int64_t n_re, int32_t R, int32_t P, const int32_t* re_k, int32_t n_rb,
                                  int32_t band_size, int32_t n_layers, const double* nvar, const double* sinr_table_db, int32_t n_table, isac_srs_report* out);

int isac_los_check_dev(isac_ctx* ctx, const double* d_ue, const double* d_ant, int64_t n_links,
                       const double* d_corners, const int32_t* d_wall_offsets, const double* d_normals,
                       const double* d_norm_dist, int32_t n_walls, uint8_t* d_los, int32_t* d_n_blocking);
int isac_winding_number_dev(isac_ctx* ctx, const double* d_points, int64_t n_points, const double* d_corners,
                            const int32_t* d_wall_offsets, const double* d_normals, int32_t n_walls,
                            double* d_winding);

int isac_synth_qpsk_grid_dev(isac_ctx* ctx, isac_c64* d_grid, int32_t K, int32_t L, int32_t A,
                             uint64_t seed, int32_t zero_s_slots);

#ifdef __cplusplus
}
#endif

#include "isac_targets.h"
#include "isac_cfar.h"
#include "isac_cfar_mc.h"

#endif
```

Before: 22250.

## Add split lazy-covariance route fusing noise covariance with beamforming stream

```diff
diff --git a/5g_based_system_level_integrated_sensing_and_communication_simulator_amd/_build.py b/5g_based_system_level_integrated_sensing_and_communication_simulator_amd/_build.py
--- a/5g_based_system_level_integrated_sensing_and_communication_simulator_amd/_build.py
+++ b/5g_based_system_level_integrated_sensing_and_communication_simulator_amd/_build.py
@@ -10,7 +10,7 @@
 OBJ = os.path.join(CSRC, "build")
 LIB = os.path.join(HERE, "libisac_hip.so")
 SOURCES = ["capi.hip", "fft2d.hip", "tables.hip", "echo.hip", "rdm.hip", "cov.hip", "eigh.hip", "music.hip", "cdl.hip", "cdl_os.hip", "cqi.hip", "los.hip", "doa2d.hip", "doa.hip", "rxfe.hip", "targets.hip", "cfar.hip"]
-HEADERS = ["isac_common.hpp", "isac_internal.hpp", "cut_window.hpp", "ofdm_symbol.hpp", "beam_window.hpp", "fft_lds.hpp", "echo_dev.hpp", "eigh_dev.hpp", "eigh_layout.hpp", os.path.join("..", "..", "include", "isac.h"), os.path.join("..", "..", "include", "isac_targets.h"), os.path.join("..", "..", "include", "isac_cfar.h"), os.path.join("..", "..", "include", "isac_cfar_mc.h")]
+HEADERS = ["isac_common.hpp", "isac_internal.hpp", "cut_window.hpp", "ofdm_symbol.hpp", "beam_window.hpp", "beam_stream.hpp", "echo_range_sl_body.inc", "fft_lds.hpp", "echo_dev.hpp", "eigh_dev.hpp", "eigh_layout.hpp", os.path.join("..", "..", "include", "isac.h"), os.path.join("..", "..", "include", "isac_targets.h"), os.path.join("..", "..", "include", "isac_cfar.h"), os.path.join("..", "..", "include", "isac_cfar_mc.h"), os.path.join("..", "..", "include", "isac_lazy_cov.h")]
 HIPCC = os.environ.get("HIPCC", "/opt/rocm/bin/hipcc")
 FLAGS = ["--offload-arch=gfx950", "-O3", "-std=c++17", "-fPIC", "-fno-gpu-rdc", "-Wall", "-Wno-unused-function",
          "-Wno-unused-variable", "-Wno-unused-value", "-Wno-unused-result", "-ffp-contract=on"]
diff --git a/5g_based_system_level_integrated_sensing_and_communication_simulator_amd/_lib.py b/5g_based_system_level_integrated_sensing_and_communication_simulator_amd/_lib.py
--- a/5g_based_system_level_integrated_sensing_and_communication_simulator_amd/_lib.py
+++ b/5g_based_system_level_integrated_sensing_and_communication_simulator_amd/_lib.py
@@ -22,6 +22,7 @@
 TARGET_SW0, TARGET_SW1 = 0, 1
 TARGET_MODELS = {"swerling0": TARGET_SW0, "swerling1": TARGET_SW1}
 ISAC_CFAR_MC_MAX_TRAIN = 128
+LAZY_COV_SPLIT, LAZY_COV_REGENERATE = 0, 1
 OPT_MUSIC_ROUTE, OPT_TAIL_FUSION, OPT_WIDE_ORDER, OPT_CDL_SHARE_SPECTRA, OPT_UPA_DOA = 0, 1, 2, 3, 4
 
 STATUS_NAMES = {0: "OK", 1: "INVALID_ARG", 2: "HIP", 3: "NO_LOS", 4: "NO_DETECTION", 5: "CFAR_WINDOW",
@@ -217,6 +218,10 @@
 PROTOTYPES_CFAR_MC = {
     "isac_cfar_monte_carlo": (_INT, (_P, _ptr(CfarMethod), _I32, _F64, _I32, _P, _I32, _U64, _U64, _P, _P)),
 }
+PROTOTYPES_LAZY_COV = {
+    "isac_ctx_set_lazy_cov_route": (_INT, (_P, _I32)),
+    "isac_ctx_get_lazy_cov_route_used": (_INT, (_P, _P)),
+}
 
 
 def library_path() -> str:
@@ -238,7 +243,7 @@
             except Exception:
                 pass
         lib = C.CDLL(_LIB_PATH, mode=C.RTLD_GLOBAL)
-        for name, (restype, argtypes) in {**PROTOTYPES, **PROTOTYPES_ADDED, **PROTOTYPES_CFAR, **PROTOTYPES_CFAR_MC}.items():
+        for name, (restype, argtypes) in {**PROTOTYPES, **PROTOTYPES_ADDED, **PROTOTYPES_CFAR, **PROTOTYPES_CFAR_MC, **PROTOTYPES_LAZY_COV}.items():
             fn = getattr(lib, name)
             fn.restype, fn.argtypes = restype, argtypes
         if lib.isac_abi_version() != ISAC_ABI_VERSION:
@@ -348,6 +353,14 @@
     def set_music_route(self, route: int):
         self.check(self.lib.isac_ctx_set_option(self.handle, OPT_MUSIC_ROUTE, int(route)))
 
+    def set_lazy_cov_route(self, route: int):
+        self.check(self.lib.isac_ctx_set_lazy_cov_route(self.handle, int(route)))
+
+    def lazy_cov_route_used(self) -> int:
+        r = C.c_int32(-1)
+        self.check(self.lib.isac_ctx_get_lazy_cov_route_used(self.handle, C.byref(r)))
+        return int(r.value)
+
     def set_tail_fusion(self, on: bool):
         self.check(self.lib.isac_ctx_set_option(self.handle, OPT_TAIL_FUSION, 1 if on else 0))
 
diff --git a/5g_based_system_level_integrated_sensing_and_communication_simulator_amd/csrc/beam_stream.hpp b/5g_based_system_level_integrated_sensing_and_communication_simulator_amd/csrc/beam_stream.hpp
--- /dev/null
+++ b/5g_based_system_level_integrated_sensing_and_communication_simulator_amd/csrc/beam_stream.hpp
@@ -0,0 +1,26 @@
+#pragma once
+
+#include "beam_window.hpp"
+
+namespace isac {
+
+constexpr int kBeamStreamLoads = 6;
+constexpr int kBeamStreamTab = 32;
+
+ISAC_HD inline int bs_steps_per_unit(int A) { return (A + kBeamStreamLoads - 1) / kBeamStreamLoads; }
+ISAC_HD inline int bs_units_of(long long n_units, int n_wg, int wg) { return wg < n_units ? (int)((n_units - wg + n_wg - 1) / n_wg) : 0; }
+ISAC_HD inline long long bs_unit(int n_wg, int wg, int t) { return (long long)wg + (long long)t * n_wg; }
+ISAC_HD inline long long bs_steps_of(long long n_slabs, long long per, int wg) {
+  const long long b = (long long)wg * per;
+  long long e = b + per;
+  if (e > n_slabs) e = n_slabs;
+  return e > b ? ((e - b + 1) & ~1ll) : 0;
+}
+ISAC_HD inline int bs_stream_units(int my_units, long long steps, int steps_per_unit) {
+  long long fit = steps > 0 ? (steps - 1) / steps_per_unit : 0;
+  if (fit > kBeamStreamTab - 1) fit = kBeamStreamTab - 1;
+  return fit < my_units ? (int)fit : my_units;
+}
+ISAC_HD inline int bs_antenna(int i, int j) { return i * kBeamStreamLoads + j; }
+
+}
diff --git a/5g_based_system_level_integrated_sensing_and_communication_simulator_amd/csrc/capi.hip b/5g_based_system_level_integrated_sensing_and_communication_simulator_amd/csrc/capi.hip
--- a/5g_based_system_level_integrated_sensing_and_communication_simulator_amd/csrc/capi.hip
+++ b/5g_based_system_level_integrated_sensing_and_communication_simulator_amd/csrc/capi.hip
@@ -301,6 +301,20 @@
   }
 }
 
+extern "C" int isac_ctx_set_lazy_cov_route(isac_ctx* ctx, int32_t route) {
+  ISAC_ENTER(ctx);
+  if (route != ISAC_LAZY_COV_SPLIT && route != ISAC_LAZY_COV_REGENERATE) return fail(ctx, ISAC_ERR_INVALID_ARG, "lazy covariance route: ISAC_LAZY_COV_SPLIT or ISAC_LAZY_COV_REGENERATE");
+  ctx->lazy_cov_route = route;
+  return ISAC_OK;
+}
+
+extern "C" int isac_ctx_get_lazy_cov_route_used(isac_ctx* ctx, int32_t* route) {
+  ISAC_ENTER_NOJOIN(ctx);
+  if (!route || ctx->lazy_cov_used < 0) return fail(ctx, ISAC_ERR_INVALID_ARG, "no covariance of a native lazy echo grid on this context yet");
+  *route = ctx->lazy_cov_used;
+  return ISAC_OK;
+}
+
 extern "C" int isac_ctx_share_streams(isac_ctx* ctx, isac_ctx* owner) {
   ISAC_ENTER(ctx);
   if (owner && owner->device != ctx->device) return fail(ctx, ISAC_ERR_INVALID_ARG, "contexts of different devices cannot share streams");
diff --git a/5g_based_system_level_integrated_sensing_and_communication_simulator_amd/csrc/cov.hip b/5g_based_system_level_integrated_sensing_and_communication_simulator_amd/csrc/cov.hip
--- a/5g_based_system_level_integrated_sensing_and_communication_simulator_amd/csrc/cov.hip
+++ b/5g_based_system_level_integrated_sensing_and_communication_simulator_amd/csrc/cov.hip
@@ -1,7 +1,9 @@
 #include <algorithm>
+#include <cstring>
 #include <type_traits>
 #include "isac_internal.hpp"
 #include "echo_dev.hpp"
+#include "beam_stream.hpp"
 
 namespace isac {
 
@@ -767,6 +769,370 @@
   else cov_staged_body<4, 1>(CovLazyGenerator<QT>(a, s_begin, s_end), phase, s_begin, s_end, blockIdx.x, part, lds);
 }
 
+struct NoiseBeamArgs {
+  const c64* tx;
+  const c64* steer;
+  c64* steer_out;
+  c64* beam;
+  long long T;
+  unsigned long long seed;
+  int K, L_out, A, s_col;
+  BeamWindow bw;
+};
+constexpr int kBeamSteerPitch = 72;
+struct BeamUnitEntry {
+  unsigned base16;
+  int d_s, d_lo, d_hi, c_lo, c_hi, pad0, pad1;
+};
+static_assert(sizeof(BeamUnitEntry) == 32, "two 16-byte LDS reads");
+__device__ __forceinline__ BeamUnitEntry beam_unit_entry(const BeamWindow& bw, long long k, bool active) {
+  BeamUnitEntry e{kCovOobOffset, 0, 0, 0, 0, 0, 0, 0};
+  if (!active) return e;
+  const int l = (int)(k / bw.units_per_symbol), j = (int)(k - (long long)l * bw.units_per_symbol);
+  const long long s = bw_range_start(bw, l), base = bw_floor_line(s) + (long long)j * kBeamUnit;
+  long long lo = bw_first(bw, l), hi = bw_range_end(bw, l);
+  if (lo < 0) lo = 0;
+  const long long span = (long long)(bw.units_per_symbol + 2) * kBeamUnit;
+  auto rel = [&](long long x) { const long long d = x - base; return (int)(d < -span ? -span : d > span ? span : d); };
+  e.d_s = rel(s);
+  if (hi > lo) {
+    e.base16 = (unsigned)((unsigned long long)base * sizeof(c64));
+    e.d_lo = e.c_lo = rel(lo);
+    e.d_hi = rel(hi);
+    e.c_hi = rel(hi - 1);
+  }
+  return e;
+}
+
+template <int QT>
+struct CovNoiseBeamSource {
+  static constexpr int NB = 4;
+  static constexpr int kGaps = 30;
+  static constexpr int kPieces = 27;
+  struct Cur { int l, sc; long long g; };
+  int gp, ga, K, s_col, g_lds0;
+  uint32_t key0, key1;
+  long long s_end;
+  bool ant_ok[2];
+  uint64_t colbase[2];
+  Cur cg;
+  uint32_t pc[2][4];
+  float wf[2][2][2];
+  bool v_half[2];
+  const c64* tx;
+  long long T;
+  int A, spu, W;
+  __amdgpu_buffer_rsrc_t rs_beam[QT];
+  const c64* s_steer;
+  const BeamUnitEntry* s_tab;
+  int n, i, ip;
+  bool fin;
+  c64 v[kBeamStreamLoads];
+  c64 acc[QT];
+  unsigned voff, soff;
+  __device__ __forceinline__ CovNoiseBeamSource(const NoiseBeamArgs& a, long long s_begin, long long s_end_, const c64* s_steer_, const BeamUnitEntry* s_tab_)
+      : gp(threadIdx.x & 7), ga(threadIdx.x >> 3), K(a.K), s_col(a.s_col), key0((uint32_t)a.seed), key1((uint32_t)(a.seed >> 32)), s_end(s_end_), tx(a.tx), T(a.T), A(a.A),
+        spu(bs_steps_per_unit(a.A)), W(a.bw.units_per_symbol * kBeamUnit), s_steer(s_steer_), s_tab(s_tab_), n(0), i(0), ip(0), fin(false), voff(kCovOobOffset), soff(kCovOobOffset) {
+#pragma unroll
+    for (int j = 0; j < 2; ++j) {
+      const int ant = ga + 32 * j;
+      ant_ok[j] = ant < a.A;
+      colbase[j] = (uint64_t)gp + (uint64_t)kSpectralSlotsPerColumn * ((uint64_t)a.L_out * (uint64_t)ant);
+    }
+    g_lds0 = (ga >> 4) * kCovSlabBlk + gp * kCovPitch + ((ga & 15) ^ kCovSwizzle(gp));
+    Cur c; c.g = s_begin; c.l = (int)((unsigned)s_begin / (unsigned)s_col); c.sc = (int)((unsigned)s_begin - (unsigned)c.l * (unsigned)s_col);
+    cg = c;
+#pragma unroll
+    for (int q = 0; q < QT; ++q) { rs_beam[q] = buffer_of(a.beam + (long long)q * a.T, (unsigned)(a.T * (long long)sizeof(c64))); acc[q] = mk(0.0, 0.0); }
+#pragma unroll
+    for (int j = 0; j < kBeamStreamLoads; ++j) v[j] = mk(0.0, 0.0);
+  }
+  __device__ __forceinline__ void advance(Cur& c) const { ++c.g; if (++c.sc == s_col) { c.sc = 0; ++c.l; } }
+  __device__ __forceinline__ void init(const Cur& c) {
+    const int k0 = ((c.sc >> 6) << 10) + ((c.sc & 63) << 3) + gp;
+    const bool in = c.g < s_end;
+    v_half[0] = in && k0 < K;
+    v_half[1] = in && k0 + 512 < K;
+    const uint32_t slot = (uint32_t)(((c.sc >> 6) << 9) + ((c.sc & 63) << 3));
+    const uint64_t slab = (uint64_t)slot + (uint64_t)kSpectralSlotsPerColumn * (uint64_t)c.l;
+#pragma unroll
+    for (int j = 0; j < 2; ++j) {
+      const uint64_t ctr = slab + colbase[j];
+      pc[j][0] = (uint32_t)ctr; pc[j][1] = (uint32_t)(ctr >> 32); pc[j][2] = kSpectralStream; pc[j][3] = 0u;
+    }
+  }
+  template <int R>
+  __device__ __forceinline__ void round() {
+#pragma unroll
+    for (int j = 0; j < 2; ++j) philox4x32_round(pc[j], key0 + (uint32_t)R * 0x9E3779B9u, key1 + (uint32_t)R * 0xBB67AE85u);
+  }
+  template <int I>
+  __device__ __forceinline__ void bm() {
+    constexpr int j = I / 2, h = I % 2;
+    box_muller32_hw_f32(pc[j][2 * h], pc[j][2 * h + 1], wf[j][h][0], wf[j][h][1]);
+  }
+  template <int I>
+  __device__ __forceinline__ void emit(c64* img) {
+    constexpr int j = I / 2, h = I % 2;
+    const bool ok = v_half[h] && ant_ok[j];
+    const double re = (double)wf[j][h][0], im = (double)wf[j][h][1];
+    img[g_lds0 + 2 * j * kCovSlabBlk + 8 * h * kCovPitch] = mk(ok ? re : 0.0, ok ? im : 0.0);
+  }
+  template <int I>
+  __device__ __forceinline__ void gen(c64* dst) {
+    if constexpr (I == 0) { init(cg); round<0>(); }
+    else if constexpr (I < 10) round<I>();
+    else if constexpr (I < 14) bm<I - 10>();
+    else { emit<I - 14>(dst); if constexpr (I == 17) advance(cg); }
+  }
+  __device__ __forceinline__ void whole(c64* img) {
+    static_for<0, 18>([&](auto ic) { gen<decltype(ic)::value>(img); });
+  }
+  __device__ __forceinline__ void prologue(c64* __restrict__ lds) {
+    whole(lds);
+    whole(lds + NB * kCovSlabBlk);
+  }
+  __device__ __forceinline__ void begin_step(long long) {}
+  template <int J0>
+  __device__ __forceinline__ void fold() {
+    const c64* sp = s_steer + ip * kBeamStreamLoads;
+#pragma unroll
+    for (int j = J0; j < J0 + kBeamStreamLoads / 2; ++j)
+#pragma unroll
+      for (int q = 0; q < QT; ++q) acc[q] = fma(v[j], sp[q * kBeamSteerPitch + j], acc[q]);
+  }
+  __device__ __forceinline__ void finish() {
+    const unsigned so = fin ? soff : kCovOobOffset;
+#pragma unroll
+    for (int q = 0; q < QT; ++q) {
+      __builtin_amdgcn_raw_buffer_store_b128(__builtin_bit_cast(u32x4_t, acc[q]), rs_beam[q], (int)so, 0, 0);
+      acc[q] = mk(fin ? 0.0 : acc[q].re, fin ? 0.0 : acc[q].im);
+    }
+  }
+  __device__ __forceinline__ void offsets() {
+    const uint4 e0 = *reinterpret_cast<const uint4*>(s_tab + n);
+    const uint4 e1 = *(reinterpret_cast<const uint4*>(s_tab + n) + 1);
+    const int tid = threadIdx.x;
+    const int ur = tid + (tid < (int)e0.y ? W : 0);
+    const bool mine = ur >= (int)e0.z && ur < (int)e0.w;
+    int uc = ur < (int)e1.x ? (int)e1.x : ur;
+    uc = uc > (int)e1.y ? (int)e1.y : uc;
+    voff = e0.x + (unsigned)uc * (unsigned)sizeof(c64);
+    soff = mine ? voff : kCovOobOffset;
+  }
+  template <int J>
+  __device__ __forceinline__ void load() {
+    const int a = bs_antenna(i, J), ac = a < A ? a : A - 1;
+    v[J] = buffer_load_c64(buffer_of(tx + (long long)ac * T, (unsigned)(T * (long long)sizeof(c64))), a < A ? voff : kCovOobOffset);
+    if constexpr (J == kBeamStreamLoads - 1) {
+      const bool last = i == spu - 1;
+      ip = i;
+      fin = last;
+      i = last ? 0 : i + 1;
+      n = (last && n < kBeamStreamTab - 1) ? n + 1 : n;
+    }
+  }
+  template <int I>
+  __device__ __forceinline__ void beam() {
+    if constexpr (I == 0) fold<0>();
+    else if constexpr (I == 1) { fold<kBeamStreamLoads / 2>(); finish(); }
+    else if constexpr (I == 2) offsets();
+    else load<I - 3>();
+  }
+  template <int P>
+  __device__ __forceinline__ void piece(c64* dst) {
+    if constexpr (P >= 18) gen<P - 9>(dst);
+    else if constexpr (P % 2 == 0) gen<P / 2>(dst);
+    else beam<P / 2>();
+  }
+  static __host__ __device__ constexpr int piece_gap(int p) { return (p * 30) / kPieces; }
+  template <int PAR, int K_>
+  __device__ __forceinline__ void gap(c64* dst, long long) {
+    static_for<0, kPieces>([&](auto ic) {
+      if constexpr (piece_gap(decltype(ic)::value) == K_) piece<decltype(ic)::value>(dst);
+    });
+  }
+};
+
+template <int QT>
+__global__ __launch_bounds__(256, 2) void cov_noise_beam_kernel(NoiseBeamArgs a, const SteerArg steer_arg, long long n_slabs, long long slabs_per_wg,
+                                                                double* __restrict__ part ) {
+  extern __shared__ __attribute__((aligned(16))) char smem_raw[];
+  c64* lds = reinterpret_cast<c64*>(smem_raw);
+  c64* s_steer = lds + kCovLdsBufs * 4 * kCovSlabBlk;
+  BeamUnitEntry* s_tab = reinterpret_cast<BeamUnitEntry*>(s_steer + QT * kBeamSteerPitch);
+  const int tid = threadIdx.x;
+  const int wid = __builtin_amdgcn_readfirstlane(tid >> 6);
+  const int grp = wid >> 1, phase = wid & 1;
+  const int A = a.A, wg = blockIdx.x, n_wg = gridDim.x;
+  const long long s_begin = (long long)wg * slabs_per_wg;
+  long long s_end = s_begin + slabs_per_wg;
+  if (s_end > n_slabs) s_end = n_slabs;
+  const int my_units = bs_units_of(bw_units(a.bw), n_wg, wg);
+  const int n_stream = bs_stream_units(my_units, bs_steps_of(n_slabs, slabs_per_wg, wg), bs_steps_per_unit(A));
+  for (int i = tid; i < QT * kBeamSteerPitch; i += 256) {
+    const int q = i / kBeamSteerPitch, r = i - q * kBeamSteerPitch;
+    c64 sv = mk(0.0, 0.0);
+    if (r < A) {
+      sv = a.steer ? a.steer[q * A + r] : steer_arg.v[q * A + r];
+      if (!a.steer && wg == 0) {
+        a.steer_out[q * A + r] = sv;
+        a.steer_out[A * QT + r * QT + q] = sv;
+      }
+    }
+    s_steer[i] = sv;
+  }
+  if (tid < kBeamStreamTab) s_tab[tid] = beam_unit_entry(a.bw, bs_unit(n_wg, wg, tid), tid < n_stream);
+  __syncthreads();
+  if (grp == 0) cov_staged_body<4, 0>(CovNoiseBeamSource<QT>(a, s_begin, s_end, s_steer, s_tab), phase, s_begin, s_end, wg, part, lds);
+  else cov_staged_body<4, 1>(CovNoiseBeamSource<QT>(a, s_begin, s_end, s_steer, s_tab), phase, s_begin, s_end, wg, part, lds);
+  for (int t = n_stream; t < my_units; ++t) {
+    const long long k = bs_unit(n_wg, wg, t);
+    const int l = (int)(k / a.bw.units_per_symbol), j = (int)(k - (long long)l * a.bw.units_per_symbol);
+    const long long lo = bw_first(a.bw, l), hi = bw_range_end(a.bw, l);
+    const long long u = bw_sample(a.bw, l, j, tid);
+    const bool mine = u >= lo && u < hi;
+    if (!__any(mine)) continue;
+    long long uc = u < lo ? lo : u < hi ? u : hi - 1;
+    uc = uc < 0 ? 0 : uc < a.T ? uc : a.T - 1;
+    const c64* p = a.tx + uc;
+    c64 acc[QT];
+#pragma unroll
+    for (int q = 0; q < QT; ++q) acc[q] = mk(0.0, 0.0);
+    constexpr int UN = 16;
+    int r = 0;
+    for (; r + UN <= A; r += UN) {
+      c64 vv[UN];
+#pragma unroll
+      for (int x = 0; x < UN; ++x) vv[x] = p[(long long)(r + x) * a.T];
+#pragma unroll
+      for (int x = 0; x < UN; ++x)
+#pragma unroll
+        for (int q = 0; q < QT; ++q) acc[q] = fma(vv[x], s_steer[q * kBeamSteerPitch + r + x], acc[q]);
+    }
+    for (; r < A; ++r) {
+      const c64 vv = p[(long long)r * a.T];
+#pragma unroll
+      for (int q = 0; q < QT; ++q) acc[q] = fma(vv, s_steer[q * kBeamSteerPitch + r], acc[q]);
+    }
+    if (mine && u >= 0) {
+#pragma unroll
+      for (int q = 0; q < QT; ++q) a.beam[(long long)q * a.T + u] = acc[q];
+    }
+  }
+}
+
+template <int QT>
+__global__ __launch_bounds__(256) void cov_cross_kernel(const c64* __restrict__ D , int K, int L, int L_out, int A, unsigned long long seed,
+                                                        c64* __restrict__ xc ) {
+  __shared__ c64 s_sum[QT][256];
+  const int l = blockIdx.x % L, r = blockIdx.x / L, tid = threadIdx.x;
+  const unsigned long long colg = (unsigned long long)l + (unsigned long long)L_out * (unsigned long long)r;
+  c64 acc[QT];
+#pragma unroll
+  for (int q = 0; q < QT; ++q) acc[q] = mk(0.0, 0.0);
+  for (int s = tid; s < kSpectralSlotsPerColumn; s += 256) {
+    const int k0 = (s & 511) + ((s >> 9) << 10);
+    if (k0 >= K) break;
+    const uint64_t ctr = (uint64_t)s + (uint64_t)kSpectralSlotsPerColumn * colg;
+    uint32_t o[4];
+    philox4x32_10((uint32_t)ctr, (uint32_t)(ctr >> 32), kSpectralStream, 0u, (uint32_t)seed, (uint32_t)(seed >> 32), o);
+    const c64 w0 = box_muller32_hw(o[0], o[1]);
+#pragma unroll
+    for (int q = 0; q < QT; ++q) acc[q] = fma(w0, conj(D[(long long)K * ((long long)l + (long long)L * q) + k0]), acc[q]);
+    if (k0 + 512 < K) {
+      const c64 w1 = box_muller32_hw(o[2], o[3]);
+#pragma unroll
+      for (int q = 0; q < QT; ++q) acc[q] = fma(w1, conj(D[(long long)K * ((long long)l + (long long)L * q) + k0 + 512]), acc[q]);
+    }
+  }
+#pragma unroll
+  for (int q = 0; q < QT; ++q) s_sum[q][tid] = acc[q];
+  __syncthreads();
+  for (int w = 128; w > 0; w >>= 1) {
+    if (tid < w) {
+#pragma unroll
+      for (int q = 0; q < QT; ++q) s_sum[q][tid] += s_sum[q][tid + w];
+    }
+    __syncthreads();
+  }
+  if (tid < QT) xc[((long long)l * A + r) * QT + tid] = s_sum[tid][0];
+}
+
+template <int QT>
+__global__ __launch_bounds__(256) void cov_dgram_kernel(const c64* __restrict__ D , int K, int L, c64* __restrict__ H ) {
+  __shared__ c64 s_sum[256];
+  const int l = blockIdx.x, tid = threadIdx.x;
+#pragma unroll
+  for (int p = 0; p < QT; ++p)
+#pragma unroll
+    for (int q = 0; q < QT; ++q) {
+      const c64 *dp = D + (long long)K * ((long long)l + (long long)L * p), *dq = D + (long long)K * ((long long)l + (long long)L * q);
+      c64 s = mk(0.0, 0.0);
+      for (int k = tid; k < K; k += 256) s = fma(conj(dp[k]), dq[k], s);
+      __syncthreads();
+      s_sum[tid] = s;
+      __syncthreads();
+      for (int w = 128; w > 0; w >>= 1) {
+        if (tid < w) s_sum[tid] += s_sum[tid + w];
+        __syncthreads();
+      }
+      if (tid == 0) H[((long long)l * QT + p) * QT + q] = s_sum[0];
+    }
+}
+
+template <int QT>
+__global__ __launch_bounds__(256) void cov_assemble_kernel(const c64* __restrict__ Mn , const c64* __restrict__ xc ,
+                                                           const c64* __restrict__ H , const c64* __restrict__ steer_rq ,
+                                                           int A, int L, double sig, double inv_n, c64* __restrict__ Ra) {
+  __shared__ c64 s_c[64 * QT], s_a[64 * QT], s_h[QT * QT], s_p[256];
+  const int tid = threadIdx.x;
+  constexpr int kParts = 256 / (64 * QT);
+  {
+    const int i = tid % (64 * QT), p = tid / (64 * QT);
+    c64 s = mk(0.0, 0.0);
+    if (i < A * QT) {
+#pragma unroll 8
+      for (int l = p; l < L; l += kParts) s += xc[(long long)l * A * QT + i];
+    }
+    s_p[tid] = s;
+  }
+  __syncthreads();
+  for (int i = tid; i < A * QT; i += 256) {
+    c64 s = s_p[i];
+#pragma unroll
+    for (int p = 1; p < kParts; ++p) s += s_p[p * 64 * QT + i];
+    s_c[i] = s;
+    s_a[i] = steer_rq[i];
+  }
+  if (tid >= 128 && tid < 128 + QT * QT) {
+    c64 s = mk(0.0, 0.0);
+#pragma unroll 8
+    for (int l = 0; l < L; ++l) s += H[(long long)l * QT * QT + (tid - 128)];
+    s_h[tid - 128] = s;
+  }
+  __syncthreads();
+  for (int e = tid; e < A * A; e += 256) {
+    const int a = e % A, b = e / A;
+    if (a > b) continue;
+    c64 x = mk(0.0, 0.0), h = mk(0.0, 0.0);
+#pragma unroll
+    for (int q = 0; q < QT; ++q) {
+      x = fma(conj(s_a[a * QT + q]), s_c[b * QT + q], x);
+      x = fma(conj(s_c[a * QT + q]), s_a[b * QT + q], x);
+      c64 hq = mk(0.0, 0.0);
+#pragma unroll
+      for (int p = 0; p < QT; ++p) hq = fma(conj(s_a[a * QT + p]), s_h[p * QT + q], hq);
+      h = fma(hq, s_a[b * QT + q], h);
+    }
+    const c64 m = Mn[a + (long long)A * b];
+    c64 v = mk(::fma(sig * sig, m.re, (sig * x.re + h.re) * inv_n), ::fma(sig * sig, m.im, (sig * x.im + h.im) * inv_n));
+    if (a == b) v.im = 0.0;
+    Ra[a + (long long)A * b] = v;
+    if (a != b) Ra[b + (long long)A * a] = conj(v);
+  }
+}
+
 __global__ __launch_bounds__(256, 2) void cov_mfma_block_kernel(const c64* __restrict__ G, long long N, int A, int n_blk,
                                                                 int n_pairs, long long slabs_per_wg,
                                                                 double* __restrict__ part ) {
@@ -956,14 +1322,84 @@
   return ISAC_OK;
 }
 
+static long long lazy_slabs(int K, int L_whole, int* s_col_out) {
+  int s_col = 0;
+  for (int k0 = 0; k0 < K; k0 += 1024) s_col += (std::min(512, K - k0) + 7) / 8;
+  *s_col_out = s_col;
+  return (long long)L_whole * s_col;
+}
+
+bool isac_lazy_split_ok(long long T, int K, int L_whole) {
+  int s_col = 0;
+  const long long n_slabs = lazy_slabs(K, L_whole, &s_col);
+  return T > 0 && T * (long long)sizeof(c64) < (1ll << 31) && n_slabs > 0 && n_slabs < (1ll << 31) - 4;
+}
+
+int isac_cov_noise_beam_on(isac_ctx* ctx, hipStream_t st, const LazySplitFront& f) {
+  if (!isac_lazy_split_ok(f.T, f.K, f.L_whole) || f.A <= 48 || f.A > 64 || f.Q < 1 || f.Q > 2) return fail(ctx, ISAC_ERR_UNSUPPORTED, "split lazy covariance: shape outside the route (49..64 antennas, one or two LoS targets)");
+  int s_col = 0;
+  const long long n_slabs = lazy_slabs(f.K, f.L_whole, &s_col);
+  long long gx, per;
+  cov_staged_grid(n_slabs, gx, per);
+  const int S = 32, n_tiles = CovPlan<4>::kTiles;
+  ISAC_TRY(ensure(ctx, ctx->cov_noise, sizeof(double) * ((size_t)gx + S) * n_tiles * 2 * 256));
+  NoiseBeamArgs a{f.d_tx, f.steer_host ? nullptr : (const c64*)ctx->steer.p, (c64*)ctx->steer.p, (c64*)ctx->beam.p, f.T, f.seed, f.K, f.L_out, f.A, s_col, f.bw};
+  SteerArg sa{};
+  if (f.steer_host) std::memcpy(sa.v, f.steer_host, sizeof(c64) * (size_t)f.A * f.Q);
+  auto launch = [&](auto qc) -> int {
+    constexpr int QT = decltype(qc)::value;
+    const size_t lds = sizeof(c64) * (kCovLdsBufs * 4 * kCovSlabBlk + QT * kBeamSteerPitch) + sizeof(BeamUnitEntry) * kBeamStreamTab;
+    ISAC_TRY(allow_lds(ctx, reinterpret_cast<const void*>(cov_noise_beam_kernel<QT>), lds));
+    ISAC_PROF_COV0(st);
+    hipLaunchKernelGGL((cov_noise_beam_kernel<QT>), dim3((unsigned)gx), dim3(256), lds, st, a, sa, n_slabs, per, (double*)ctx->cov_noise.p);
+    ISAC_HIP(hipGetLastError());
+    ISAC_PROF_COV1(st);
+    return ISAC_OK;
+  };
+  ISAC_TRY(f.Q == 1 ? launch(std::integral_constant<int, 1>{}) : launch(std::integral_constant<int, 2>{}));
+  ctx->split_wg = (int)gx;
+  return ISAC_OK;
+}
+
+static int covariance_lazy_split(isac_ctx* ctx, hipStream_t st, c64* Ra) {
+  const LazyEcho& lz = ctx->lazy;
+  const int S = 32, n_tiles = CovPlan<4>::kTiles, n_part = ctx->split_wg;
+  const double inv_n = 1.0 / ((double)lz.K * (double)lz.L_out);
+  double* part = (double*)ctx->cov_noise.p;
+  double* part2 = part + (size_t)n_part * n_tiles * 2 * 256;
+  c64* xc = (c64*)ctx->cov_xc.p;
+  c64* H = xc + lazy_xc_elems(lz.L_whole, lz.A, lz.Q);
+  c64* Mn = H + (size_t)lz.L_whole * lz.Q * lz.Q;
+  hipLaunchKernelGGL(cov_reduce_slice_kernel, dim3(n_tiles, S), dim3(256), 0, st, (const double*)part, n_part, n_tiles, S, part2);
+  ISAC_HIP(hipGetLastError());
+  hipLaunchKernelGGL(cov_reduce_kernel, dim3(n_tiles), dim3(256, 4), 0, st, (const double*)part2, S, n_tiles, lz.A, inv_n, Mn);
+  ISAC_HIP(hipGetLastError());
+  const c64* srq = (const c64*)ctx->steer.p + (size_t)lz.A * lz.Q;
+  auto tail = [&](auto qc) -> int {
+    constexpr int QT = decltype(qc)::value;
+    if constexpr (QT > 1) {
+      hipLaunchKernelGGL((cov_cross_kernel<QT>), dim3((unsigned)(lz.L_whole * lz.A)), dim3(256), 0, st, (const c64*)ctx->dgrid.p, lz.K, lz.L_whole, lz.L_out, lz.A, lz.seed, xc);
+      ISAC_HIP(hipGetLastError());
+    }
+    hipLaunchKernelGGL((cov_dgram_kernel<QT>), dim3((unsigned)lz.L_whole), dim3(256), 0, st, (const c64*)ctx->dgrid.p, lz.K, lz.L_whole, H);
+    ISAC_HIP(hipGetLastError());
+    hipLaunchKernelGGL((cov_assemble_kernel<QT>), dim3(1), dim3(256), 0, st, (const c64*)Mn, (const c64*)xc, (const c64*)H, srq, lz.A, lz.L_whole, lz.sig, inv_n, Ra);
+    ISAC_HIP(hipGetLastError());
+    return ISAC_OK;
+  };
+  ISAC_TRY(lz.Q == 1 ? tail(std::integral_constant<int, 1>{}) : tail(std::integral_constant<int, 2>{}));
+  return ISAC_OK;
+}
+
 int isac_covariance_lazy_on(isac_ctx* ctx, hipStream_t st, isac_c64* d_Ra) {
   const LazyEcho& lz = ctx->lazy;
   if (!lz.valid || !lz.native || !d_Ra) return fail(ctx, ISAC_ERR_INVALID_ARG, "no native lazy echo grid on this context");
   if (lz.A <= 48 || lz.A > 64 || lz.Q < 1 || lz.Q > 2) return fail(ctx, ISAC_ERR_UNSUPPORTED, "lazy covariance: 49..64 antennas, one or two LoS targets");
+  ctx->lazy_cov_used = lz.split ? ISAC_LAZY_COV_SPLIT : ISAC_LAZY_COV_REGENERATE;
+  if (lz.split) return covariance_lazy_split(ctx, st, (c64*)d_Ra);
   if ((long long)lz.K * lz.L_whole * 16 >= (1ll << 31)) return fail(ctx, ISAC_ERR_UNSUPPORTED, "lazy covariance: per-target grid of 2 GB or more");
   int s_col = 0;
-  for (int k0 = 0; k0 < lz.K; k0 += 1024) s_col += (std::min(512, lz.K - k0) + 7) / 8;
-  const long long n_slabs = (long long)lz.L_whole * s_col;
+  const long long n_slabs = lazy_slabs(lz.K, lz.L_whole, &s_col);
   if (n_slabs <= 0 || n_slabs >= (1ll << 31) - 4) return fail(ctx, ISAC_ERR_UNSUPPORTED, "lazy covariance: slab count out of range");
   long long gx, per;
   cov_staged_grid(n_slabs, gx, per);
diff --git a/5g_based_system_level_integrated_sensing_and_communication_simulator_amd/csrc/echo.hip b/5g_based_system_level_integrated_sensing_and_communication_simulator_amd/csrc/echo.hip
--- a/5g_based_system_level_integrated_sensing_and_communication_simulator_amd/csrc/echo.hip
+++ b/5g_based_system_level_integrated_sensing_and_communication_simulator_amd/csrc/echo.hip
@@ -95,10 +95,6 @@
 template <int QT>
 struct CoefTargets {
   TargetDesc t[QT];
-};
-constexpr int kSteerArgMax = 128;
-struct SteerArg {
-  c64 v[kSteerArgMax];
 };
 template <int QT, int UNROLL>
 __global__ __launch_bounds__(256) void beamsum_coef_kernel(const c64* __restrict__ tx, long long T, int A,
@@ -142,6 +138,24 @@
         const double tt = (double)t * Ts;
         cq[t] = u < 0 ? mk(0.0, 0.0) : coef_value(acc[q], t, tab.t[q], w, Ts, tt, rx_phase(w, tt));
       }
+    }
+  }
+}
+
+template <int QT>
+__global__ __launch_bounds__(256) void coef_window_kernel(const c64* __restrict__ beam , long long T, BeamWindow bw, CoefTargets<QT> tab, double w, double Ts,
+                                                          c64* __restrict__ coef ) {
+  const int k = blockIdx.x;
+  const int l = k / bw.units_per_symbol, j = k - l * bw.units_per_symbol;
+  const long long lo = bw_first(bw, l), hi = bw_range_end(bw, l);
+  const long long u = bw_sample(bw, l, j, threadIdx.x);
+  if (!(u >= lo && u < hi)) return;
+#pragma unroll
+  for (int q = 0; q < QT; ++q) {
+    const long long t = u + tab.t[q].shift;
+    if (t >= 0 && t < T) {
+      const double tt = (double)t * Ts;
+      coef[(long long)q * T + t] = u < 0 ? mk(0.0, 0.0) : coef_value(beam[(long long)q * T + u], t, tab.t[q], w, Ts, tt, rx_phase(w, tt));
     }
   }
 }
@@ -311,98 +325,24 @@
                                                             const c64* txg, const double* win_k,
                                                             const double* __restrict__ win_r, double inv_n, double sqrt_n,
                                                             int row_lo, int n_rows, c64* __restrict__ ymid) {
-  static_assert(QT >= 1 && QT <= 2, "compile-time target count");
-  extern __shared__ __attribute__((aligned(16))) char smem_raw[];
-  c64* lds = reinterpret_cast<c64*>(smem_raw);
-  using FFT = Fft4096W;
-  constexpr int NT = FFT::NT, PER = FFT::PER, NG = PER / GROUP;
-  const int tid = threadIdx.x;
-  FFT fft;
-  int l, r;
-  if (!spectral_tile_map(blockIdx.x, L_whole, A, l, r)) return;
-  const long long colg = (long long)l + (long long)L_out * r;
-  const c64* Dl = D + (long long)K * l;
-  const long long d_stride = (long long)K * L_whole;
-  const c64* ptx = txg + (long long)K * colg;
-  const c64* nzc = NZ == 2 ? noise + (long long)K * colg : nullptr;
-  const __amdgpu_buffer_rsrc_t rs_dst = buffer_of(grid + (long long)K * colg, (unsigned)K * (unsigned)sizeof(c64));
-  c64 s[QT];
-#pragma unroll
-  for (int q = 0; q < QT; ++q) s[q] = steer_rq[(long long)r * QT + q];
-  struct Ld { c64 tx; double w; c64 d[QT]; c64 nz; };
-  Ld ld[2][GROUP];
-  auto load_group = [&](int g, int b) {
-#pragma unroll
-    for (int u = 0; u < GROUP; ++u) {
-      const int k = tid + NT * (g * GROUP + u);
-      const int kc = k < K ? k : K - 1;
-      const unsigned o16 = (unsigned)kc * (unsigned)sizeof(c64);
-      auto at = [](const auto* base, unsigned off) { return *reinterpret_cast<decltype(base)>(reinterpret_cast<const char*>(base) + off); };
-      Ld& e = ld[b][u];
-      e.tx = at(ptx, o16);
-      e.w = at(win_k, (unsigned)k * (unsigned)sizeof(double));
-      if constexpr (NZ == 2) e.nz = at(nzc, o16);
-#pragma unroll
-      for (int q = 0; q < QT; ++q) e.d[q] = at(Dl + (long long)q * d_stride, o16);
-    }
-    asm volatile("" ::: "memory");
-  };
-  fft.init_table(lds, tw, tid);
-  load_group(0, 0);
-  __builtin_amdgcn_sched_barrier(0);
-#pragma unroll
-  for (int j = 0; j < PER; ++j) fft.x[j] = mk(0.0, 0.0);
-  const int wave_k0 = __builtin_amdgcn_readfirstlane(tid & ~63);
-  auto draw = [&](int c) {
-    if constexpr (NZ == 1) {
-      const int j0 = 2 * c, j1 = j0 + 1;
-      if (wave_k0 + NT * j0 < K) {
-        const uint64_t ctr = (uint64_t)(tid + NT * c) + (uint64_t)kSpectralSlotsPerColumn * (uint64_t)colg;
-        uint32_t o[4];
-        philox4x32_10((uint32_t)ctr, (uint32_t)(ctr >> 32), kSpectralStream, 0u, (uint32_t)seed, (uint32_t)(seed >> 32), o);
-        fft.x[j0] = box_muller32_hw(o[0], o[1]);
-        if (wave_k0 + NT * j1 < K) fft.x[j1] = box_muller32_hw(o[2], o[3]);
-      }
-    }
-  };
-  bool live = false;
-  auto consume = [&](int g, int b) {
-#pragma unroll
-    for (int u = 0; u < GROUP; ++u) {
-      const int j = g * GROUP + u, k = tid + NT * j;
-      const Ld& e = ld[b][u];
-      const c64 v = spectral_echo_value<QT, NZ != 0>(e.d, s, NZ == 2 ? e.nz : fft.x[j], sig);
-      if constexpr (STORE) buffer_store_c64_nt(rs_dst, (unsigned)k * (unsigned)sizeof(c64), v);
-      else asm volatile("" ::"v"(v.re), "v"(v.im) : "memory");
-      const c64 y = mul_conj(v, e.tx) * e.w;
-      live |= (y.re != 0.0) | (y.im != 0.0);
-      fft.x[j] = y;
-    }
-  };
-#pragma unroll
-  for (int g = 0; g < NG; ++g) {
-#pragma unroll
-    for (int c = g * GROUP / 2; c < (g + 1) * GROUP / 2; ++c) draw(c);
-    __builtin_amdgcn_sched_barrier(0);
-    if (g + 1 < NG) load_group(g + 1, (g + 1) & 1);
-    consume(g, g & 1);
-    __builtin_amdgcn_sched_barrier(0);
-  }
-  c64* yd = ymid + (long long)n_rows * colg;
-  if (!__syncthreads_or(live)) {
-    for (int rr = tid; rr < n_rows; rr += NT) yd[rr] = mk(0.0, 0.0);
-    return;
-  }
-  fft.init_twiddles_lds(lds, tid);
-  const int blk = FFT::block_of_rows(row_lo, n_rows);
-  fft.template transform<+1>(lds, tw, tid, blk);
-  auto put = [&](int n, c64 v) {
-    const int rr = n - row_lo;
-    const double wr = win_r[n];
-    if (rr >= 0 && rr < n_rows) yd[rr] = ((v * inv_n) * sqrt_n) * wr;
-  };
-  if (blk >= 0) fft.drain_block(put, tid, blk);
-  else fft.drain(put, tid);
+  constexpr bool XC = false;
+  c64* const xc = nullptr;
+#include "echo_range_sl_body.inc"
+}
+
+constexpr int kEchoXcLds = 16;
+template <int QT>
+__global__ __launch_bounds__(Fft4096W::NT, kEchoRangeWavesPerSimd) void echo_range_xc_kernel(int K, int L_whole, int L_out, int A, const c64* D,
+                                                            const c64* __restrict__ steer_rq, double sig, uint64_t seed,
+                                                            const c64* noise, const c64* __restrict__ tw,
+                                                            c64* grid,
+                                                            const c64* txg, const double* win_k,
+                                                            const double* __restrict__ win_r, double inv_n, double sqrt_n,
+                                                            int row_lo, int n_rows, c64* __restrict__ ymid, c64* __restrict__ xc) {
+  static_assert(QT == 1, "one LoS target (see above)");
+  constexpr int NZ = 1, GROUP = 4;
+  constexpr bool STORE = false, XC = true;
+#include "echo_range_sl_body.inc"
 }
 
 struct ModIo {
@@ -531,8 +471,9 @@
   return ISAC_OK;
 }
 
+struct SplitReq { int L_out; unsigned long long seed; };
 static int prepare_echo(isac_ctx* ctx, const c64* d_tx, long long T, const isac_radar_channel_params* rp,
-                        const uint8_t* los, int* q_out, const OfdmGeom* coef_only = nullptr) {
+                        const uint8_t* los, int* q_out, const OfdmGeom* coef_only = nullptr, const SplitReq* split = nullptr) {
   if (!d_tx || !rp || !los) return fail(ctx, ISAC_ERR_INVALID_ARG, "NULL argument");
   if (T <= 0 || rp->n_ants <= 0 || rp->n_targets < 0) return fail(ctx, ISAC_ERR_INVALID_ARG, "bad T / n_ants / n_targets");
   ctx->lazy.valid = false;
@@ -590,6 +531,22 @@
     if (T >= kSpan || d_max >= kSpan || d_min <= -kSpan) return fail(ctx, ISAC_ERR_CAPACITY, "waveform or target delay beyond the beam-sum's unit count");
     const BeamWindow bw = beam_window(g.nfft, g.cp_base, g.cp_long, g.sym_per_half, whole_symbols(g, T), T, d_min, d_max);
     const unsigned gbu = (unsigned)std::max<long long>(1, std::min<long long>(bw_units(bw), 1024));
+    if (split) {
+      const LazySplitFront f{d_tx, T, A, Q, steer_by_arg ? steer_aq.data() : nullptr, bw, g.n_sc, whole_symbols(g, T), split->L_out, split->seed};
+      ISAC_TRY(isac_cov_noise_beam_on(ctx, ctx->stream, f));
+      timeline_mark(ctx, 1, ctx->stream);
+      auto coefs = [&](auto qc) {
+        constexpr int QT = decltype(qc)::value;
+        CoefTargets<QT> ct;
+        for (int q = 0; q < QT; ++q) ct.t[q] = tab.t[q];
+        hipLaunchKernelGGL((coef_window_kernel<QT>), dim3((unsigned)bw_units(bw)), dim3(256), 0, ctx->stream, (const c64*)ctx->beam.p, T, bw, ct, w, Ts, (c64*)ctx->coef.p);
+      };
+      if (Q == 1) coefs(std::integral_constant<int, 1>{});
+      else coefs(std::integral_constant<int, 2>{});
+      ISAC_HIP(hipGetLastError());
+      *q_out = Q;
+      return ISAC_OK;
+    }
     SteerArg sa{};
     if (steer_by_arg) std::memcpy(sa.v, steer_aq.data(), sizeof(c64) * (size_t)A * Q);
     auto launch = [&](auto qc) {
@@ -674,9 +631,9 @@
 }
 
 static int spectral_prepare(isac_ctx* ctx, const c64* d_tx, long long T, const isac_radar_channel_params* rp, const uint8_t* los,
-                            const OfdmGeom& g, int* q_out, int* l_whole_out, bool coef_only = false) {
+                            const OfdmGeom& g, int* q_out, int* l_whole_out, bool coef_only = false, const SplitReq* split = nullptr) {
   int Q = 0;
-  ISAC_TRY(prepare_echo(ctx, d_tx, T, rp, los, &Q, coef_only ? &g : nullptr));
+  ISAC_TRY(prepare_echo(ctx, d_tx, T, rp, los, &Q, coef_only ? &g : nullptr, split));
   const int L_whole = whole_symbols(g, T);
   if (L_whole <= 0) return fail(ctx, ISAC_ERR_SHORT_WAVEFORM, "waveform shorter than one OFDM symbol");
   ISAC_TRY(ensure(ctx, ctx->dgrid, sizeof(c64) * (size_t)g.n_sc * L_whole * Q));
@@ -704,8 +661,8 @@
 }
 
 template <class Kern, class... Args>
-static int launch_echo_range(isac_ctx* ctx, Kern kern, int L_whole, int A, Args... args) {
-  const size_t lds = sizeof(c64) * Fft4096W::LDS_ELEMS;
+static int launch_echo_range(isac_ctx* ctx, Kern kern, int L_whole, int A, size_t lds_extra, Args... args) {
+  const size_t lds = sizeof(c64) * Fft4096W::LDS_ELEMS + lds_extra;
   ISAC_TRY(allow_lds(ctx, reinterpret_cast<const void*>(kern), lds));
   hipLaunchKernelGGL(kern, dim3((unsigned)spectral_grid_size(L_whole, A)), dim3(Fft4096W::NT), lds, ctx->stream, args...);
   ISAC_HIP(hipGetLastError());
@@ -804,9 +761,13 @@
   if (noise_mode == ISAC_NOISE_INJECTED_SPECTRAL && !d_noise_unit) return fail(ctx, ISAC_ERR_INVALID_ARG, "noise buffer missing");
   if (!spectral_mode(noise_mode)) return plain_then_range(true);
   int Q = 0, L_whole = 0;
-  ISAC_TRY(spectral_prepare(ctx, (const c64*)d_tx_wave, T, rp, los, g, &Q, &L_whole, true));
+  const int lw_pre = whole_symbols(g, T);
+  const SplitReq sreq{padded_symbols(lw_pre, tx_dim_l, nullptr), seed};
+  const bool split = lazy_native && ctx->lazy_cov_route == 0 && lw_pre > 0 && isac_lazy_split_ok(T, g.n_sc, lw_pre);
+  ISAC_TRY(spectral_prepare(ctx, (const c64*)d_tx_wave, T, rp, los, g, &Q, &L_whole, true, split ? &sreq : nullptr));
   const int A = rp->n_ants, row_lo = cr.row_lo, nr = cr.nr;
   const int L_out = padded_symbols(L_whole, tx_dim_l, l_out);
+  if (split) ISAC_TRY(ensure(ctx, ctx->cov_xc, sizeof(c64) * lazy_xc_total(L_whole, A, Q)));
   ctx->tgt.drop();
   ISAC_TRY(ensure(ctx, ctx->ymid, sizeof(c64) * (size_t)nr * L_out * A));
   if (L_out > L_whole) {
@@ -821,22 +782,27 @@
   if (!ctx->profile_cov) ISAC_TRY(profile_begin(ctx));
   timeline_mark(ctx, 2, ctx->stream);
   auto launch = [&](auto kern, auto... q_rt) {
-    return launch_echo_range(ctx, kern, L_whole, A, g.n_sc, L_whole, L_out, A, q_rt..., (const c64*)ctx->dgrid.p, (const c64*)ctx->steer.p + (size_t)A * Q, sig, seed,
+    return launch_echo_range(ctx, kern, L_whole, A, (size_t)0, g.n_sc, L_whole, L_out, A, q_rt..., (const c64*)ctx->dgrid.p, (const c64*)ctx->steer.p + (size_t)A * Q, sig, seed,
                              (const c64*)d_noise_unit, tw, (c64*)d_echo_grid, (const c64*)d_tx_grid, wk, wr, 1.0 / ep->n_ifft, std::sqrt((double)ep->n_ifft), row_lo, nr,
                              (c64*)ctx->ymid.p);
   };
   const bool philox = noise_mode == ISAC_NOISE_PHILOX_SPECTRAL;
   ISAC_TRY(echo_dispatch<4>(Q, [&](auto qc) {
     constexpr int QT = decltype(qc)::value;
-    if constexpr (QT == 1 || QT == 2)
+    if constexpr (QT == 1 || QT == 2) {
+      if constexpr (QT == 1)
+        if (split)
+          return launch_echo_range(ctx, echo_range_xc_kernel<QT>, L_whole, A, sizeof(c64) * kEchoXcLds, g.n_sc, L_whole, L_out, A, (const c64*)ctx->dgrid.p, (const c64*)ctx->steer.p + (size_t)A * Q, sig, seed,
+                                 (const c64*)d_noise_unit, tw, (c64*)d_echo_grid, (const c64*)d_tx_grid, wk, wr, 1.0 / ep->n_ifft, std::sqrt((double)ep->n_ifft), row_lo, nr,
+                                 (c64*)ctx->ymid.p, (c64*)ctx->cov_xc.p);
       return launch(lazy_native ? echo_range_sl_kernel<QT, 1, false> : philox ? echo_range_sl_kernel<QT, 1> : echo_range_sl_kernel<QT, 2>);
-    else
+    } else
       return launch(philox ? echo_range_kernel<QT, 1> : echo_range_kernel<QT, 2>, Q);
   }));
   if (!ctx->profile_cov) ISAC_TRY(profile_end(ctx));
   timeline_mark(ctx, 3, ctx->stream);
   ctx->range_cache.set(d_echo_grid, d_tx_grid, g.n_sc, L_out, A, ep->n_ifft, row_lo, nr);
-  if (lazy_native) ctx->lazy.set_native(g.n_sc, L_whole, L_out, A, Q, sig, seed);
+  if (lazy_native) { ctx->lazy.set_native(g.n_sc, L_whole, L_out, A, Q, sig, seed); ctx->lazy.split = split; }
   else if (lazy) ctx->lazy.set_owned(g.n_sc, L_out, A);
   return ISAC_OK;
 }
diff --git a/5g_based_system_level_integrated_sensing_and_communication_simulator_amd/csrc/echo_dev.hpp b/5g_based_system_level_integrated_sensing_and_communication_simulator_amd/csrc/echo_dev.hpp
--- a/5g_based_system_level_integrated_sensing_and_communication_simulator_amd/csrc/echo_dev.hpp
+++ b/5g_based_system_level_integrated_sensing_and_communication_simulator_amd/csrc/echo_dev.hpp
@@ -233,6 +233,11 @@
   }
 }
 
+constexpr int kSteerArgMax = 128;
+struct SteerArg {
+  c64 v[kSteerArgMax];
+};
+
 __device__ __forceinline__ c64 rx_sample(long long t, int r, long long T, int Q, const c64* __restrict__ coef,
                                          const c64* __restrict__ s_steer_r ,
                                          const c64* __restrict__ phase_rx, int noise_mode,
diff --git a/5g_based_system_level_integrated_sensing_and_communication_simulator_amd/csrc/echo_range_sl_body.inc b/5g_based_system_level_integrated_sensing_and_communication_simulator_amd/csrc/echo_range_sl_body.inc
--- /dev/null
+++ b/5g_based_system_level_integrated_sensing_and_communication_simulator_amd/csrc/echo_range_sl_body.inc
@@ -0,0 +1,133 @@
+  static_assert(QT >= 1 && QT <= 2, "compile-time target count");
+  static_assert(!XC || NZ == 1, "the cross term is of the Philox field");
+  extern __shared__ __attribute__((aligned(16))) char smem_raw[];
+  c64* lds = reinterpret_cast<c64*>(smem_raw);
+  using FFT = Fft4096W;
+  constexpr int NT = FFT::NT, PER = FFT::PER, NG = PER / GROUP;
+  const int tid = threadIdx.x;
+  FFT fft;
+  int l, r;
+  if (!spectral_tile_map(blockIdx.x, L_whole, A, l, r)) return;
+  const long long colg = (long long)l + (long long)L_out * r;
+  const c64* Dl = D + (long long)K * l;
+  const long long d_stride = (long long)K * L_whole;
+  const c64* ptx = txg + (long long)K * colg;
+  const c64* nzc = NZ == 2 ? noise + (long long)K * colg : nullptr;
+  const __amdgpu_buffer_rsrc_t rs_dst = buffer_of(grid + (long long)K * colg, (unsigned)K * (unsigned)sizeof(c64));
+  c64 s[QT];
+#pragma unroll
+  for (int q = 0; q < QT; ++q) s[q] = steer_rq[(long long)r * QT + q];
+  struct Ld { c64 tx; double w; c64 d[QT]; c64 nz; };
+  Ld ld[2][GROUP];
+  auto load_group = [&](int g, int b) {
+#pragma unroll
+    for (int u = 0; u < GROUP; ++u) {
+      const int k = tid + NT * (g * GROUP + u);
+      const int kc = k < K ? k : K - 1;
+      const unsigned o16 = (unsigned)kc * (unsigned)sizeof(c64);
+      auto at = [](const auto* base, unsigned off) { return *reinterpret_cast<decltype(base)>(reinterpret_cast<const char*>(base) + off); };
+      Ld& e = ld[b][u];
+      e.tx = at(ptx, o16);
+      e.w = at(win_k, (unsigned)k * (unsigned)sizeof(double));
+      if constexpr (NZ == 2) e.nz = at(nzc, o16);
+#pragma unroll
+      for (int q = 0; q < QT; ++q) e.d[q] = at(Dl + (long long)q * d_stride, o16);
+    }
+    asm volatile("" ::: "memory");
+  };
+  fft.init_table(lds, tw, tid);
+  load_group(0, 0);
+  __builtin_amdgcn_sched_barrier(0);
+#pragma unroll
+  for (int j = 0; j < PER; ++j) fft.x[j] = mk(0.0, 0.0);
+  const int wave_k0 = __builtin_amdgcn_readfirstlane(tid & ~63);
+  auto draw = [&](int c) {
+    if constexpr (NZ == 1) {
+      const int j0 = 2 * c, j1 = j0 + 1;
+      if (wave_k0 + NT * j0 < K) {
+        const uint64_t ctr = (uint64_t)(tid + NT * c) + (uint64_t)kSpectralSlotsPerColumn * (uint64_t)colg;
+        uint32_t o[4];
+        philox4x32_10((uint32_t)ctr, (uint32_t)(ctr >> 32), kSpectralStream, 0u, (uint32_t)seed, (uint32_t)(seed >> 32), o);
+        fft.x[j0] = box_muller32_hw(o[0], o[1]);
+        if (wave_k0 + NT * j1 < K) fft.x[j1] = box_muller32_hw(o[2], o[3]);
+        if constexpr (XC) {
+          if (!(tid + NT * j0 < K)) fft.x[j0] = mk(0.0, 0.0);
+          if (!(tid + NT * j1 < K)) fft.x[j1] = mk(0.0, 0.0);
+        }
+      }
+    }
+  };
+  bool live = false;
+  auto consume = [&](int g, int b) {
+    c64 xg[QT];
+#pragma unroll
+    for (int q = 0; q < QT; ++q) xg[q] = mk(0.0, 0.0);
+#pragma unroll
+    for (int u = 0; u < GROUP; ++u) {
+      const int j = g * GROUP + u, k = tid + NT * j;
+      const Ld& e = ld[b][u];
+      if constexpr (XC) {
+#pragma unroll
+        for (int q = 0; q < QT; ++q) {
+          xg[q] = fma(fft.x[j], conj(e.d[q]), xg[q]);
+          asm volatile("" : "+v"(xg[q].re), "+v"(xg[q].im));
+        }
+      }
+      const c64 v = spectral_echo_value<QT, NZ != 0>(e.d, s, NZ == 2 ? e.nz : fft.x[j], sig);
+      if constexpr (STORE) buffer_store_c64_nt(rs_dst, (unsigned)k * (unsigned)sizeof(c64), v);
+      else asm volatile("" ::"v"(v.re), "v"(v.im) : "memory");
+      const c64 y = mul_conj(v, e.tx) * e.w;
+      live |= (y.re != 0.0) | (y.im != 0.0);
+      fft.x[j] = y;
+    }
+    if constexpr (XC) {
+#pragma unroll
+      for (int q = 0; q < QT; ++q) lds[(g * QT + q) * NT + tid] = xg[q];
+    }
+  };
+#pragma unroll
+  for (int g = 0; g < NG; ++g) {
+#pragma unroll
+    for (int c = g * GROUP / 2; c < (g + 1) * GROUP / 2; ++c) draw(c);
+    __builtin_amdgcn_sched_barrier(0);
+    if (g + 1 < NG) load_group(g + 1, (g + 1) & 1);
+    consume(g, g & 1);
+    __builtin_amdgcn_sched_barrier(0);
+  }
+  c64* yd = ymid + (long long)n_rows * colg;
+  c64* xs = lds + FFT::LDS_ELEMS;
+  if constexpr (XC) {
+    static_assert(NG * QT * NT <= FFT::IMG, "the group sums fit the data image");
+    c64 xacc[QT];
+#pragma unroll
+    for (int q = 0; q < QT; ++q) {
+      xacc[q] = lds[q * NT + tid];
+#pragma unroll
+      for (int g = 1; g < NG; ++g) xacc[q] += lds[(g * QT + q) * NT + tid];
+#pragma unroll
+      for (int m = 32; m > 0; m >>= 1) { xacc[q].re += __shfl_xor(xacc[q].re, m); xacc[q].im += __shfl_xor(xacc[q].im, m); }
+      if ((tid & 63) == 0) xs[(tid >> 6) * QT + q] = xacc[q];
+    }
+  }
+  const bool any_live = __syncthreads_or(live);
+  if constexpr (XC) {
+    if (tid < QT) {
+      c64 sum = xs[tid];
+      for (int w = 1; w < NT / 64; ++w) sum += xs[w * QT + tid];
+      xc[((long long)l * A + r) * QT + tid] = sum;
+    }
+  }
+  if (!any_live) {
+    for (int rr = tid; rr < n_rows; rr += NT) yd[rr] = mk(0.0, 0.0);
+    return;
+  }
+  fft.init_twiddles_lds(lds, tid);
+  const int blk = FFT::block_of_rows(row_lo, n_rows);
+  fft.template transform<+1>(lds, tw, tid, blk);
+  auto put = [&](int n, c64 v) {
+    const int rr = n - row_lo;
+    const double wr = win_r[n];
+    if (rr >= 0 && rr < n_rows) yd[rr] = ((v * inv_n) * sqrt_n) * wr;
+  };
+  if (blk >= 0) fft.drain_block(put, tid, blk);
+  else fft.drain(put, tid);
diff --git a/5g_based_system_level_integrated_sensing_and_communication_simulator_amd/csrc/isac_common.hpp b/5g_based_system_level_integrated_sensing_and_communication_simulator_amd/csrc/isac_common.hpp
--- a/5g_based_system_level_integrated_sensing_and_communication_simulator_amd/csrc/isac_common.hpp
+++ b/5g_based_system_level_integrated_sensing_and_communication_simulator_amd/csrc/isac_common.hpp
@@ -118,6 +118,7 @@
   int K = 0, L_whole = 0, L_out = 0, A = 0, Q = 0;
   double sig = 0.0;
   unsigned long long seed = 0;
+  bool split = false;
   void set_owned(int K_, int L_, int A_) { *this = LazyEcho{true, false, K_, L_, L_, A_, 0, 0.0, 0}; }
   void set_native(int K_, int L_whole_, int L_out_, int A_, int Q_, double sig_, unsigned long long seed_) { *this = LazyEcho{true, true, K_, L_whole_, L_out_, A_, Q_, sig_, seed_}; }
 };
@@ -183,6 +184,9 @@
   hipEvent_t ev_k0 = nullptr, ev_k1 = nullptr;
   bool profile = false, profile_recorded = false;
   bool profile_cov = false;
+  int lazy_cov_route = 0;
+  int lazy_cov_used = -1;
+  int split_wg = 0;
   int music_route = 0;
   long long eig_epoch = 0;
   bool tail_unjoined = false;
@@ -191,7 +195,7 @@
   std::string err;
   std::map<const void*, size_t> lds_allowed;
   std::map<isac::TableKey, isac::DevBuf> tables;
-  isac::DevBuf beam, coef, phase_rx, steer, dgrid, ymid, pwin, flags, det_cut, det_pow, det_cnt, cov_part, cov,
+  isac::DevBuf beam, coef, phase_rx, steer, dgrid, ymid, pwin, flags, det_cut, det_pow, det_cnt, cov_part, cov, cov_noise, cov_xc,
       eig_w, eig_v, eig_scratch, spec, misc, stage_a, stage_b, stage_c, cdl_par, seg, cdl_h, rxfe_tab;
   isac::PinnedBuf pinned;
   isac::PinnedBuf bounce; hipEvent_t ev_bounce[2] = {nullptr, nullptr};
diff --git a/5g_based_system_level_integrated_sensing_and_communication_simulator_amd/csrc/isac_internal.hpp b/5g_based_system_level_integrated_sensing_and_communication_simulator_amd/csrc/isac_internal.hpp
--- a/5g_based_system_level_integrated_sensing_and_communication_simulator_amd/csrc/isac_internal.hpp
+++ b/5g_based_system_level_integrated_sensing_and_communication_simulator_amd/csrc/isac_internal.hpp
@@ -1,6 +1,7 @@
 #pragma once
 #include "isac_common.hpp"
 #include "eigh_layout.hpp"
+#include "beam_window.hpp"
 
 template <typename T, typename Build>
 int cached_table(isac_ctx* ctx, const isac::TableKey& key, const T** out, Build build) {
@@ -31,6 +32,16 @@
 int fft2d_estimates(isac_ctx* ctx, const isac_est_params* ep, const isac::CutWindow& win, int A, const int* ant_off, const std::vector<int>& cut, const std::vector<double>& pw, int num_dets_dev, std::vector<int32_t>& det_rc, isac_est_result* out);
 int isac_covariance_on(isac_ctx* ctx, hipStream_t st, const isac_c64* d_grid, int64_t N, int32_t A, isac_c64* d_Ra);
 int isac_covariance_lazy_on(isac_ctx* ctx, hipStream_t st, isac_c64* d_Ra);
+struct LazySplitFront {
+  const isac::c64* d_tx; long long T; int A, Q;
+  const isac::c64* steer_host;
+  isac::BeamWindow bw;
+  int K, L_whole, L_out; unsigned long long seed;
+};
+bool isac_lazy_split_ok(long long T, int K, int L_whole);
+int isac_cov_noise_beam_on(isac_ctx* ctx, hipStream_t st, const LazySplitFront& f);
+inline size_t lazy_xc_elems(int L_whole, int A, int Q) { return (size_t)L_whole * A * Q; }
+inline size_t lazy_xc_total(int L_whole, int A, int Q) { return lazy_xc_elems(L_whole, A, Q) + (size_t)L_whole * Q * Q + (size_t)A * A; }
 int isac_eigh_dev(isac_ctx* ctx, const isac::c64* d_H, int A, hipStream_t st, bool live_replay = true);
 int isac_eigh_replay_recover(isac_ctx* ctx, int n, hipStream_t st);
 int isac_eigh_ql_dev(isac_ctx* ctx, int n, hipStream_t st, const int* ctl, bool allow_live = true);
diff --git a/include/isac.h b/include/isac.h
--- a/include/isac.h
+++ b/include/isac.h
@@ -343,5 +343,6 @@
 #include "isac_targets.h"
 #include "isac_cfar.h"
 #include "isac_cfar_mc.h"
+#include "isac_lazy_cov.h"
 
 #endif
diff --git a/include/isac_lazy_cov.h b/include/isac_lazy_cov.h
--- /dev/null
+++ b/include/isac_lazy_cov.h
@@ -0,0 +1,18 @@
+#ifndef ISAC_LAZY_COV_H
+#define ISAC_LAZY_COV_H
+
+#include "isac.h"
+
+#ifdef __cplusplus
+extern "C" {
+#endif
+
+enum { ISAC_LAZY_COV_SPLIT = 0, ISAC_LAZY_COV_REGENERATE = 1 };
+int isac_ctx_set_lazy_cov_route(isac_ctx* ctx, int32_t route);
+int isac_ctx_get_lazy_cov_route_used(isac_ctx* ctx, int32_t* route);
+
+#ifdef __cplusplus
+}
+#endif
+
+#endif
```

After: 23710 (median of 6 runs). +6.6%, better.
